# zju3dv/LoG

Hardware: NVIDIA H100
Metric: gaussians_per_s_fwd_bwd (higher is better)
Workload: dtype f32

## Files before the change

include/log_b200_raster.h:

```cpp
#ifndef LOG_B200_RASTER_H
#define LOG_B200_RASTER_H

#include <stdint.h>

#ifdef __cplusplus
extern "C" {
#endif

#define LGR_ABI_VERSION 19
#define LGR_TILE 16

#define LGR_FILTER_ADD 0
#define LGR_FILTER_MAX 1
#define LGR_FILTER_NONE 2

#define LGR_E_BADARG (-1)
#define LGR_E_CAPACITY (-2)
#define LGR_E_UNSUPPORTED (-3)

typedef struct lgr_view {
  int32_t image_height, image_width;
  float tanfovx, tanfovy;
  float scale_modifier;
  int32_t sh_degree;
  int32_t sh_coeffs;
  int32_t filter_mode;
  int32_t want_aux;
  int32_t tile_row_begin, tile_row_end;
  int32_t num_owners;
  int32_t raw_params;
  int32_t* band_ids_d;
  int32_t* band_blk_d;
  int32_t* band_count_d;
  int32_t* band_rows_d;
  float* band_dsplat_d;
  int32_t* tile_rank_d;
  const int64_t* gather_index_d;
  const int32_t* pid_map_d;
  int32_t* contrib_id_d;
  uint32_t* contrib_entry_d;
  int32_t* contrib_count_d;
  const int32_t* last_contrib_d;
  const int32_t* region_count_d;
  int64_t region_cap;
  int32_t num_regions;
  int32_t num_channels;
  int32_t log_depth;
  float* splat_ext_d;
  const float* cov3D_precomp_d;
  float* dcov3D_d;
  const float* viewmatrix_d;
  const float* projmatrix_d;
  const float* campos_d;
  const float* bg_d;
} lgr_view;

#define LGR_SPLAT_FLOATS 12
#define LGR_GRAD_FLOATS 12
#define LGR_TILE_SCRATCH_INTS 33
#define LGR_CONTRIB_MAX_LIST (1 << 24)
#define LGR_META_INTS 8

int lgr_abi_version(void);

int lgr_compute_radius(int64_t n, const float* means3D_d, const float* scales_d, const float* rotations_d,
                       const float* projmatrix_d, const float* viewmatrix_d, float focal_x, float focal_y,
                       float tan_fovx, float tan_fovy, float* radii_d, void* stream);

int lgr_mark_visible(int64_t n, const float* means3D_d, const float* viewmatrix_d, uint8_t* visible_d, void* stream);

int lgr_forward_project(const lgr_view* view, int64_t n, const float* means3D_d, const float* opacities_d,
                        const float* scales_d, const float* rotations_d, const float* colors_precomp_d,
                        const float* shs_d, float* splat_d, int32_t* radii_d, uint8_t* clamped_d,
                        int32_t* tile_start_d, int32_t* tile_cursor_d, int32_t* meta_d, void* stream);

int lgr_forward_render(const lgr_view* view, int64_t n, int64_t num_instances, int32_t max_tile_len,
                       int32_t num_long_tiles, const float* splat_d, const int32_t* radii_d, const int32_t* tile_start_d,
                       int32_t* tile_cursor_d, uint32_t* inst_key_d, uint32_t* inst_val_d, uint32_t* inst_tmp_d,
                       int32_t* sorted_ids_d, float* image_d, float* final_T_d, int32_t* n_contrib_d,
                       int32_t* point_id_pixel_d, float* point_weight_pixel_d, float* point_weight_d,
                       int32_t* point_count_d, void* stream);
int32_t lgr_sort_smem_capacity(void);

int lgr_forward_render_device_sized(const lgr_view* view, int64_t n, int64_t instance_capacity, int32_t* meta_d,
                                    const float* splat_d, const int32_t* radii_d, int32_t* tile_start_d,
                                    int32_t* tile_cursor_d, uint32_t* inst_key_d, uint32_t* inst_val_d,
                                    int32_t* sorted_ids_d, float* image_d, float* final_T_d, int32_t* n_contrib_d,
                                    int32_t* point_id_pixel_d, float* point_weight_pixel_d, float* point_weight_d,
                                    int32_t* point_count_d, void* stream);

int lgr_backward(const lgr_view* view, int64_t n, int64_t num_instances, const float* means3D_d,
                 const float* opacities_d, const float* scales_d, const float* rotations_d,
                 const float* colors_precomp_d, const float* shs_d, const float* splat_d, const int32_t* radii_d,
                 const uint8_t* clamped_d, const int32_t* tile_start_d, const int32_t* sorted_ids_d,
                 const float* image_d, const float* dL_dimage_d, float* dsplat_d,
                 float* dmeans3D_d, float* dmeans2D_d, float* dopacities_d, float* dscales_d, float* drotations_d,
                 float* dcolors_d, float* dshs_d, float* grad_rows_d, void* const* peer_stage_d, int32_t my_rank,
                 int64_t num_rows, void* stream);

#define LGR_STAGE_HEADER_FLOATS 64
#define LGR_ROW_FLOATS 20
#define LGR_OWNER_CHUNK(n, r) ((((n) + (r) - 1) / (r) + 255) / 256 * 256)
int lgr_grad_scatter_add(int64_t num_rows, const float* rows_d, int64_t lo, int64_t hi, float* shard_d, void* stream);
int lgr_grad_scatter_add_staged(const float* stage_d, int32_t num_sources, int64_t owner_chunk, int64_t lo, int64_t hi,
                                float* shard_d, void* stream);

typedef struct lgr_shard_layout {
  int32_t num_ranks, my_rank;
  int64_t cap;
  int64_t off_count, off_splat, off_radii, off_gid, off_dsplat, off_weight, off_pcount;
} lgr_shard_layout;
#define LGR_SHARD_MAX_RANKS 32
#define LGR_SHARD_SEND_INTS(n_local, r) (2 * (int64_t)(r) * ((((n_local) > 0 ? (n_local) : 1) + 255) / 256) + (r))

int lgr_shard_send(const lgr_view* view, const lgr_shard_layout* layout, int64_t n_local, int64_t gid_base,
                   const float* splat_d, const int32_t* radii_d, int32_t* send_scratch_d, void* const* peer_base_d,
                   void* stream);

int lgr_shard_recv_bin(const lgr_view* view, const lgr_shard_layout* layout, float* exchange_d, float* dsplat_d,
                       int32_t* tile_start_d, int32_t* tile_cursor_d, int32_t* meta_d, void* stream);

int lgr_blend_backward(const lgr_view* view, int64_t n, int64_t num_instances, const float* splat_d,
                       const int32_t* tile_start_d, const int32_t* sorted_ids_d, const float* image_d,
                       const float* dL_dimage_d, float* dsplat_d, void* stream);

int lgr_shard_return_rows(const lgr_shard_layout* layout, const float* exchange_d, int64_t total_rows, const void* rows_d,
                          int32_t row_floats, int64_t dst_offset_floats, void* const* peer_base_d, void* stream);

int lgr_shard_gather(const lgr_view* view, const lgr_shard_layout* layout, int64_t n_local, const float* splat_d,
                     const int32_t* radii_d, const int32_t* send_scratch_d, const float* exchange_d,
                     float* dsplat_local_d, float* point_weight_d, int32_t* point_count_d, void* stream);

int lgr_shard_recv_bin_aux(const lgr_view* view, const lgr_shard_layout* layout, float* exchange_d, float* dsplat_d,
                           int32_t* tile_start_d, int32_t* tile_cursor_d, int32_t* meta_d, float* point_weight_rows_d,
                           int32_t* point_count_rows_d, void* stream);
int lgr_shard_return_packed(const lgr_shard_layout* layout, const float* exchange_d, const float* dsplat_rows_d,
                            const float* point_weight_rows_d, const int32_t* point_count_rows_d, void* const* peer_base_d,
                            void* stream);
int lgr_shard_gather_packed(const lgr_view* view, const lgr_shard_layout* layout, int64_t n_local, const float* splat_d,
                            const int32_t* radii_d, const int32_t* send_scratch_d, const float* exchange_d,
                            float* dsplat_local_d, float* point_weight_d, int32_t* point_count_d, void* stream);

typedef struct lgr_tree {
  int64_t num_points, num_nodes;
  int32_t max_child, max_level;
  const int32_t* node_index_d;
  const int32_t* tree_d;
} lgr_tree;
#define LGR_TREE_SCRATCH_INTS(p, s) (8 + 2 * (int64_t)(p) + (int64_t)(s) + 2 * (((int64_t)(s) + 255) / 256) + 2 + ((int64_t)(s) + 3) / 4)
int lgr_tree_traverse(const lgr_tree* tree, const float* xyz_d, const float* scaling_raw_d, const float* rotation_raw_d,
                      const float* projmatrix_d, const float* viewmatrix_d, float focal_x, float focal_y, float tan_fovx,
                      float tan_fovy, const int64_t* root_index_d, int64_t num_roots, float min_resolution_pixel,
                      int32_t max_depth, int32_t* scratch_d, int64_t* index_out_d, int64_t* count_out_d, void* stream);

int lgr_point_compact(int64_t n, const int32_t* point_count_d, int32_t* scratch_d, int32_t* ids_out_d,
                      int32_t* counts_out_d, int32_t* num_out_d, void* stream);

int lgr_sparse_adam(int64_t rows, int32_t row_floats, const int64_t* index_d, const float* grad_d, float* param_d,
                    float* exp_avg_d, float* exp_avg_sq_d, float* max_exp_avg_sq_d, int64_t step, double lr, double beta1,
                    double beta2, double eps, void* stream);

#define LGR_PROFILE_KERNELS 12
int lgr_profile_enable(int on);
int lgr_profile_collect(double* ms_out, int32_t* launches_out, int32_t capacity);
const char* lgr_profile_kernel_name(int kernel_id);


#ifdef __cplusplus
}
#endif
#endif
```

log_b200/_capi.py:

```python
import ctypes
import os

from .build import LIB_PATH

_i32, _i64, _f32, _vp = ctypes.c_int32, ctypes.c_int64, ctypes.c_float, ctypes.c_void_p

LGR_FILTER_ADD, LGR_FILTER_MAX, LGR_FILTER_NONE = 0, 1, 2
LGR_SPLAT_FLOATS = 12
LGR_GRAD_FLOATS = 12
LGR_META_INTS = 8
LGR_TILE_SCRATCH_INTS = 33
LGR_ABI_VERSION = 19
LGR_CONTRIB_MAX_LIST = 1 << 24
LGR_STAGE_HEADER_FLOATS = 64
LGR_ROW_FLOATS = 20

EXPORTS = ('lgr_abi_version', 'lgr_sort_smem_capacity', 'lgr_compute_radius', 'lgr_forward_project',
           'lgr_forward_render', 'lgr_forward_render_device_sized', 'lgr_backward', 'lgr_grad_scatter_add', 'lgr_grad_scatter_add_staged', 'lgr_point_compact', 'lgr_sparse_adam', 'lgr_profile_enable', 'lgr_profile_collect',
           'lgr_profile_kernel_name', 'lgr_shard_send', 'lgr_shard_recv_bin', 'lgr_blend_backward', 'lgr_shard_return_rows',
           'lgr_shard_gather', 'lgr_shard_recv_bin_aux', 'lgr_shard_return_packed', 'lgr_shard_gather_packed', 'lgr_tree_traverse', 'lgr_mark_visible')
LGR_SHARD_MAX_RANKS = 32
LGR_PROFILE_KERNELS = 12


class LgrView(ctypes.Structure):
    _fields_ = [('image_height', _i32), ('image_width', _i32), ('tanfovx', _f32), ('tanfovy', _f32),
                ('scale_modifier', _f32), ('sh_degree', _i32), ('sh_coeffs', _i32), ('filter_mode', _i32),
                ('want_aux', _i32), ('tile_row_begin', _i32), ('tile_row_end', _i32),
                ('num_owners', _i32), ('raw_params', _i32), ('band_ids_d', _vp), ('band_blk_d', _vp), ('band_count_d', _vp), ('band_rows_d', _vp), ('band_dsplat_d', _vp), ('tile_rank_d', _vp), ('gather_index_d', _vp), ('pid_map_d', _vp), ('contrib_id_d', _vp), ('contrib_entry_d', _vp), ('contrib_count_d', _vp), ('last_contrib_d', _vp),
                ('region_count_d', _vp), ('region_cap', _i64), ('num_regions', _i32), ('num_channels', _i32), ('log_depth', _i32), ('splat_ext_d', _vp), ('cov3D_precomp_d', _vp), ('dcov3D_d', _vp),
                ('viewmatrix_d', _vp), ('projmatrix_d', _vp), ('campos_d', _vp), ('bg_d', _vp)]


class LgrShardLayout(ctypes.Structure):
    _fields_ = [('num_ranks', _i32), ('my_rank', _i32), ('cap', _i64), ('off_count', _i64), ('off_splat', _i64),
                ('off_radii', _i64), ('off_gid', _i64), ('off_dsplat', _i64), ('off_weight', _i64), ('off_pcount', _i64)]


class LgrTree(ctypes.Structure):
    _fields_ = [('num_points', _i64), ('num_nodes', _i64), ('max_child', _i32), ('max_level', _i32),
                ('node_index_d', _vp), ('tree_d', _vp)]


def tree_scratch_ints(num_points, slots):
    return 8 + 2 * num_points + slots + 2 * ((slots + 255) // 256) + 2 + (slots + 3) // 4


def shard_send_ints(n_local, r):
    return 2 * r * ((max(n_local, 1) + 255) // 256) + r


class LgrError(RuntimeError):
    pass


_lib = None


def bind(lib):
    lib.lgr_abi_version.restype = ctypes.c_int
    lib.lgr_sort_smem_capacity.restype = _i32
    lib.lgr_mark_visible.restype = ctypes.c_int
    lib.lgr_mark_visible.argtypes = [_i64, _vp, _vp, _vp, _vp]
    lib.lgr_compute_radius.restype = ctypes.c_int
    lib.lgr_compute_radius.argtypes = [_i64, _vp, _vp, _vp, _vp, _vp, _f32, _f32, _f32, _f32, _vp, _vp]
    lib.lgr_forward_project.restype = ctypes.c_int
    lib.lgr_forward_project.argtypes = [ctypes.POINTER(LgrView), _i64] + [_vp] * 13
    lib.lgr_forward_render.restype = ctypes.c_int
    lib.lgr_forward_render.argtypes = [ctypes.POINTER(LgrView), _i64, _i64, _i32, _i32] + [_vp] * 16
    lib.lgr_forward_render_device_sized.restype = ctypes.c_int
    lib.lgr_forward_render_device_sized.argtypes = [ctypes.POINTER(LgrView), _i64, _i64] + [_vp] * 16
    lib.lgr_sparse_adam.restype = ctypes.c_int
    lib.lgr_sparse_adam.argtypes = [_i64, _i32, _vp, _vp, _vp, _vp, _vp, _vp, _i64, ctypes.c_double, ctypes.c_double,
                                    ctypes.c_double, ctypes.c_double, _vp]
    lib.lgr_point_compact.restype = ctypes.c_int
    lib.lgr_point_compact.argtypes = [_i64, _vp, _vp, _vp, _vp, _vp, _vp]
    lib.lgr_backward.restype = ctypes.c_int
    lib.lgr_backward.argtypes = [ctypes.POINTER(LgrView), _i64, _i64] + [_vp] * 23 + [_i32, _i64, _vp]
    lib.lgr_grad_scatter_add_staged.restype = ctypes.c_int
    lib.lgr_grad_scatter_add_staged.argtypes = [_vp, _i32, _i64, _i64, _i64, _vp, _vp]
    lib.lgr_grad_scatter_add.restype = ctypes.c_int
    lib.lgr_grad_scatter_add.argtypes = [_i64, _vp, _i64, _i64, _vp, _vp]
    lay = ctypes.POINTER(LgrShardLayout)
    lib.lgr_shard_send.restype = ctypes.c_int
    lib.lgr_shard_send.argtypes = [ctypes.POINTER(LgrView), lay, _i64, _i64, _vp, _vp, _vp, _vp, _vp]
    lib.lgr_shard_recv_bin.restype = ctypes.c_int
    lib.lgr_shard_recv_bin.argtypes = [ctypes.POINTER(LgrView), lay, _vp, _vp, _vp, _vp, _vp, _vp]
    lib.lgr_blend_backward.restype = ctypes.c_int
    lib.lgr_blend_backward.argtypes = [ctypes.POINTER(LgrView), _i64, _i64, _vp, _vp, _vp, _vp, _vp, _vp, _vp]
    lib.lgr_shard_return_rows.restype = ctypes.c_int
    lib.lgr_shard_return_rows.argtypes = [lay, _vp, _i64, _vp, _i32, _i64, _vp, _vp]
    lib.lgr_shard_gather.restype = ctypes.c_int
    lib.lgr_shard_gather.argtypes = [ctypes.POINTER(LgrView), lay, _i64, _vp, _vp, _vp, _vp, _vp, _vp, _vp, _vp]
    lib.lgr_shard_recv_bin_aux.restype = ctypes.c_int
    lib.lgr_shard_recv_bin_aux.argtypes = [ctypes.POINTER(LgrView), lay, _vp, _vp, _vp, _vp, _vp, _vp, _vp, _vp]
    lib.lgr_shard_return_packed.restype = ctypes.c_int
    lib.lgr_shard_return_packed.argtypes = [lay, _vp, _vp, _vp, _vp, _vp, _vp]
    lib.lgr_shard_gather_packed.restype = ctypes.c_int
    lib.lgr_shard_gather_packed.argtypes = [ctypes.POINTER(LgrView), lay, _i64, _vp, _vp, _vp, _vp, _vp, _vp, _vp, _vp]
    lib.lgr_tree_traverse.restype = ctypes.c_int
    lib.lgr_tree_traverse.argtypes = [ctypes.POINTER(LgrTree), _vp, _vp, _vp, _vp, _vp, _f32, _f32, _f32, _f32, _vp, _i64, _f32,
                                      _i32, _vp, _vp, _vp, _vp]
    lib.lgr_profile_enable.restype = ctypes.c_int
    lib.lgr_profile_enable.argtypes = [ctypes.c_int]
    lib.lgr_profile_collect.restype = ctypes.c_int
    lib.lgr_profile_collect.argtypes = [_vp, _vp, _i32]
    lib.lgr_profile_kernel_name.restype = ctypes.c_char_p
    lib.lgr_profile_kernel_name.argtypes = [ctypes.c_int]
    return lib


def load():
    global _lib
    if _lib is not None:
        return _lib
    if not os.path.exists(LIB_PATH):
        raise LgrError(f'{LIB_PATH} not found: run `python -m log_b200.build` (or __graft_entry__.build()). '
                       'log_b200 has no CPU fallback.')
    lib = bind(ctypes.CDLL(LIB_PATH))
    if lib.lgr_abi_version() != LGR_ABI_VERSION:
        raise LgrError('liblog_b200_raster.so ABI version mismatch: rebuild with `python -m log_b200.build --force`')
    _lib = lib
    return lib


def current_stream(device=None):
    import torch
    return ctypes.c_void_p(torch.cuda.current_stream(device).cuda_stream)


def require_cuda(t, name):
    if not t.is_cuda:
        raise LgrError(f'{name} is on {t.device}: log_b200 rasterises on CUDA only (no CPU fallback)')


def check(rc, what):
    if rc == 0:
        return
    if rc > 0:
        raise LgrError(f'{what}: CUDA error {rc}')
    names = {-1: 'bad argument', -2: 'instance buffer capacity', -3: 'unsupported'}
    raise LgrError(f'{what}: {names.get(rc, rc)}')


def profile_enable(on=True):
    check(load().lgr_profile_enable(1 if on else 0), 'lgr_profile_enable')


def profile_collect():
    lib = load()
    ms = (ctypes.c_double * LGR_PROFILE_KERNELS)()
    cnt = (_i32 * LGR_PROFILE_KERNELS)()
    check(lib.lgr_profile_collect(ms, cnt, LGR_PROFILE_KERNELS), 'lgr_profile_collect')
    return {lib.lgr_profile_kernel_name(k).decode(): (ms[k], cnt[k]) for k in range(LGR_PROFILE_KERNELS)}


def owner_chunk(n, r):
    return ((n + r - 1) // r + 255) // 256 * 256
```

log_b200/csrc/lgr_bin.cu:

```cuda
#include "lgr_common.cuh"
#include "lgr_prof.cuh"

namespace lgr {

constexpr int SCAN_THREADS = 1024;
constexpr int SORT_CAP_SMALL_FWD = 4096;

__global__ void __launch_bounds__(SCAN_THREADS)
tile_scan_kernel(int ntiles, int32_t* __restrict__ tile_start ,
                 int32_t* __restrict__ cursor ,
                 int32_t* __restrict__ meta, int small_cap, int ranked) {
  __shared__ int warp_sum[SCAN_THREADS / 32];
  __shared__ int carry_s, maxl_s, nbig_s;
  const int tid = threadIdx.x, lane = tid & 31, wid = tid >> 5;
  if (tid == 0) { carry_s = 0; maxl_s = 0; nbig_s = 0; }
  __syncthreads();
  int local_max = 0;
  for (int base = 0; base < ntiles; base += SCAN_THREADS) {
    const int i = base + tid;
    const int c = (i < ntiles) ? cursor[i * CSTRIDE] + cursor[i * CSTRIDE + 1] : 0;
    local_max = max(local_max, c);
    int x = c;
#pragma unroll
    for (int o = 1; o < 32; o <<= 1) { const int y = __shfl_up_sync(0xffffffffu, x, o); if (lane >= o) x += y; }
    if (lane == 31) warp_sum[wid] = x;
    __syncthreads();
    if (wid == 0) {
      int w = warp_sum[lane];
#pragma unroll
      for (int o = 1; o < 32; o <<= 1) { const int y = __shfl_up_sync(0xffffffffu, w, o); if (lane >= o) w += y; }
      warp_sum[lane] = w;
    }
    __syncthreads();
    const int carry = carry_s;
    const int excl = carry + (wid ? warp_sum[wid - 1] : 0) + x - c;
    if (i < ntiles) {
      tile_start[i] = excl; cursor[i * CSTRIDE + ranked] = 0;
      if (c > small_cap) cursor[CSTRIDE * ntiles + atomicAdd(&nbig_s, 1)] = i;
    }
    __syncthreads();
    if (tid == SCAN_THREADS - 1) carry_s = carry + warp_sum[31];
    __syncthreads();
  }
#pragma unroll
  for (int o = 16; o > 0; o >>= 1) local_max = max(local_max, __shfl_xor_sync(0xffffffffu, local_max, o));
  if (lane == 0) atomicMax(&maxl_s, local_max);
  __syncthreads();
  if (tid == 0) { tile_start[ntiles] = carry_s; meta[0] = carry_s; meta[1] = maxl_s; meta[5] = nbig_s; }
}

constexpr int SCATTER_THREADS = 256;

__global__ void __launch_bounds__(SCATTER_THREADS)
bin_scatter_kernel(View v, int64_t n, const float* __restrict__ splat, const int32_t* __restrict__ radii,
                   const int32_t* __restrict__ tile_start, int32_t* __restrict__ cursor, uint32_t* __restrict__ inst_key,
                   uint32_t* __restrict__ inst_val, int64_t capacity ) {
  __shared__ int64_t s_first[LGR_SHARD_MAX_RANKS + 1];
  const int64_t total = v.region_count ? region_setup(v, s_first) : n;
  for (int64_t base = (int64_t)blockIdx.x * SCATTER_THREADS; base < total; base += (int64_t)gridDim.x * SCATTER_THREADS) {
  int64_t i = base + threadIdx.x;
  bool live = i < total;
  if (live && v.region_count) i = region_row(v, s_first, i);
  if (live && v.num_owners > 0) {
    const int b = (int)(i / 256), sl = (int)(i % 256);
    if (sl >= v.band_blk[b]) live = false;
    else {
      const int id = v.band_ids[i];
      v.band_rows[v.band_blk[v.band_blocks + b] + sl] = id;
      if (v.band_dsplat) {
        float4* z = reinterpret_cast<float4*>(v.band_dsplat + (int64_t)id * LGR_GRAD_FLOATS);
        z[0] = z[1] = z[2] = make_float4(0.f, 0.f, 0.f, 0.f);
      }
      i = id;
    }
  }
  int rad = 0;
  float4 r0 = make_float4(0.f, 0.f, 0.f, 0.f), r1 = r0;
  float depth = 0.f;
  int4 rk = make_int4(-1, -1, -1, -1);
  if (live) {
    rad = radii[i];
    r0 = ldg4(splat + i * LGR_SPLAT_FLOATS);
    r1 = ldg4(splat + i * LGR_SPLAT_FLOATS + 4);
    depth = __ldg(splat + i * LGR_SPLAT_FLOATS + 11);
    if (v.tile_rank) rk = __ldg(reinterpret_cast<const int4*>(v.tile_rank + 4 * i));
    live = rad > 0;
  }
  if (live && v.num_owners == 0 && v.band_dsplat) {
    float4* z = reinterpret_cast<float4*>(v.band_dsplat + i * LGR_GRAD_FLOATS);
    z[0] = z[1] = z[2] = make_float4(0.f, 0.f, 0.f, 0.f);
  }
  int x0 = 0, y0 = 0, x1 = 0, y1 = 0;
  uint32_t key = 0;
  if (live) {
    live = r1.z > 0.f;
    if (live) {
      key = __float_as_uint(depth);
      tile_rect_tight(r0.x, r0.y, rad, r1.z, r1.w, v.gx, v.gy, v.row0, v.row1, x0, y0, x1, y1);
    }
  }
  const int w = x1 - x0, cnt = live ? w * (y1 - y0) : 0;
  if (cnt > 0 && cnt <= 4) {
    int t[4], slot[4];
#pragma unroll
    for (int k = 0; k < 4; k++) {
      const int ty = y0 + k / max(w, 1), tx = x0 + k % max(w, 1);
      t[k] = k < cnt ? (ty - v.row0) * v.gx + tx : -1;
    }
    if (v.tile_rank) {
      slot[0] = rk.x; slot[1] = rk.y; slot[2] = rk.z; slot[3] = rk.w;
    } else {
#pragma unroll
      for (int k = 0; k < 4; k++) slot[k] = t[k] >= 0 ? atomicAdd(cursor + t[k] * CSTRIDE, 1) : 0;
    }
#pragma unroll
    for (int k = 0; k < 4; k++)
      if (t[k] >= 0) {
        const int pos = __ldg(tile_start + t[k]) + slot[k];
        if (pos < capacity) { inst_key[pos] = key; inst_val[pos] = (uint32_t)i; }
      }
  }
  const int lane = threadIdx.x & 31, big = v.tile_rank ? 1 : 0;
  unsigned todo = __ballot_sync(0xffffffffu, cnt > 4);
  while (todo) {
    const int src = __ffs(todo) - 1;
    todo &= todo - 1;
    const int bx0 = __shfl_sync(0xffffffffu, x0, src), by0 = __shfl_sync(0xffffffffu, y0, src);
    const int bw = __shfl_sync(0xffffffffu, w, src), bcnt = __shfl_sync(0xffffffffu, cnt, src);
    const uint32_t bkey = __shfl_sync(0xffffffffu, key, src);
    const uint32_t bid = (uint32_t)__shfl_sync(0xffffffffu, (int)i, src);
    for (int k = lane; k < bcnt; k += 32) {
      const int t = (by0 + k / bw - v.row0) * v.gx + bx0 + k % bw;
      const int pos = tile_start[t] + (big ? cursor[t * CSTRIDE] : 0) + atomicAdd(cursor + t * CSTRIDE + big, 1);
      if (pos < capacity) { inst_key[pos] = bkey; inst_val[pos] = bid; }
    }
  }
  }
}

constexpr int SORT_THREADS = 256;
constexpr int SORT_WARPS = SORT_THREADS / 32;
constexpr int RADIX_BITS = 8;
constexpr int RADIX = 1 << RADIX_BITS;
constexpr int SORT_CAP_SMALL = SORT_CAP_SMALL_FWD;
constexpr int SORT_CAP_LARGE = 13312;

__device__ __forceinline__ bool radix_pass(const uint32_t* __restrict__ kin, const uint32_t* __restrict__ vin,
                                           uint32_t* __restrict__ kout, uint32_t* __restrict__ vout, int len, int shift,
                                           bool on_val, int* __restrict__ whist) {
  const int tid = threadIdx.x, lane = tid & 31, wid = tid >> 5;
  const int seg = ((len + SORT_WARPS * 32 - 1) / (SORT_WARPS * 32)) * 32;
  const int beg = min(len, wid * seg), end = min(len, beg + seg);
  for (int j = tid; j < SORT_WARPS * RADIX; j += SORT_THREADS) whist[j] = 0;
  __syncthreads();
  int* myh = whist + wid * RADIX;
  for (int i = beg + lane; i < end; i += 32) {
    const uint32_t d = ((on_val ? vin[i] : kin[i]) >> shift) & (RADIX - 1);
    atomicAdd(myh + d, 1);
  }
  __syncthreads();
  {
    const int d = tid;
    int tot = 0;
#pragma unroll
    for (int w = 0; w < SORT_WARPS; w++) tot += whist[w * RADIX + d];
    int x = tot;
#pragma unroll
    for (int o = 1; o < 32; o <<= 1) { const int y = __shfl_up_sync(0xffffffffu, x, o); if (lane >= o) x += y; }
    __shared__ int wsum[SORT_WARPS];
    if (lane == 31) wsum[wid] = x;
    __syncthreads();
    int base = x - tot;
#pragma unroll
    for (int w = 0; w < SORT_WARPS; w++) if (w < wid) base += wsum[w];
#pragma unroll
    for (int w = 0; w < SORT_WARPS; w++) { const int c = whist[w * RADIX + d]; whist[w * RADIX + d] = base; base += c; }
    if (__syncthreads_or(tot == len)) return true;
  }
  for (int i0 = beg; i0 < end; i0 += 32) {
    const int i = i0 + lane;
    const bool ok = i < end;
    uint32_t k = 0, val = 0;
    if (ok) { k = kin[i]; val = vin[i]; }
    const uint32_t d = ok ? (((on_val ? val : k) >> shift) & (RADIX - 1)) : (RADIX + lane);
    const uint32_t peers = __match_any_sync(0xffffffffu, d);
    const int rank = __popc(peers & ((1u << lane) - 1u));
    int base = 0;
    if (ok) base = myh[d];
    __syncwarp();
    if (ok && rank == 0) myh[d] = base + __popc(peers);
    __syncwarp();
    if (ok) { kout[base + rank] = k; vout[base + rank] = val; }
  }
  __syncthreads();
  return false;
}

__device__ __forceinline__ void sort_tile(uint32_t* kA, uint32_t* vA, uint32_t* kB, uint32_t* vB, int len, int id_bits,
                                          int* whist) {
  uint32_t *ki = kA, *vi = vA, *ko = kB, *vo = vB;
  auto run = [&](int shift, bool on_val) {
    const bool ident = radix_pass(ki, vi, ko, vo, len, shift, on_val, whist);
    if (!ident) { uint32_t* t = ki; ki = ko; ko = t; t = vi; vi = vo; vo = t; }
  };
  for (int s = 0; s < 32; s += RADIX_BITS) run(s, false);
  int my_tie = 0;
  for (int i = threadIdx.x + 1; i < len; i += SORT_THREADS) if (ki[i] == ki[i - 1]) my_tie = 1;
  if (__syncthreads_or(my_tie)) {
    for (int s = 0; s < id_bits; s += RADIX_BITS) run(s, true);
    for (int s = 0; s < 32; s += RADIX_BITS) run(s, false);
  }
  if (ki != kA) {
    for (int i = threadIdx.x; i < len; i += SORT_THREADS) { kA[i] = ki[i]; vA[i] = vi[i]; }
    __syncthreads();
  }
}

constexpr int MSD_SMALL = 96;
constexpr int MSD_STACK = 512;

struct MsdShared {
  int hist[RADIX];
  int bstart[RADIX + 1];
  alignas(16) int wsum[SORT_WARPS];
  unsigned long long wmin[SORT_WARPS], wmax[SORT_WARPS];
  int stack_beg[MSD_STACK], stack_len[MSD_STACK];
  int top, shift, overflow;
};

__device__ __forceinline__ unsigned long long composite(uint32_t k, uint32_t v) { return ((unsigned long long)k << 32) | v; }

__device__ __forceinline__ bool sort_tile_msd(uint32_t* kA, uint32_t* vA, uint32_t* kB, uint32_t* vB, int len, MsdShared& sh) {
  const int tid = threadIdx.x, lane = tid & 31, wid = tid >> 5;
  if (tid == 0) { sh.stack_beg[0] = 0; sh.stack_len[0] = len; sh.top = 1; sh.overflow = 0; }
  __syncthreads();
  while (true) {
    const int top = sh.top;
    if (top == 0 || sh.overflow) break;
    const int beg = sh.stack_beg[top - 1], n = sh.stack_len[top - 1];
    __syncthreads();
    if (tid == 0) sh.top = top - 1;
    unsigned long long mn = ~0ull, mx = 0ull;
    for (int i = tid; i < n; i += SORT_THREADS) {
      const unsigned long long c = composite(kA[beg + i], vA[beg + i]);
      mn = min(mn, c); mx = max(mx, c);
    }
#pragma unroll
    for (int o = 16; o > 0; o >>= 1) {
      mn = min(mn, __shfl_xor_sync(0xffffffffu, mn, o));
      mx = max(mx, __shfl_xor_sync(0xffffffffu, mx, o));
    }
    if (lane == 0) { sh.wmin[wid] = mn; sh.wmax[wid] = mx; }
    sh.hist[tid] = 0;
    __syncthreads();
    if (tid == 0) {
      unsigned long long a = sh.wmin[0], b = sh.wmax[0];
#pragma unroll
      for (int w = 1; w < SORT_WARPS; w++) { a = min(a, sh.wmin[w]); b = max(b, sh.wmax[w]); }
      const int hb = 63 - __clzll((long long)(a ^ b));
      sh.shift = max(0, hb - (RADIX_BITS - 1));
    }
    __syncthreads();
    const int shift = sh.shift;
    for (int i = tid; i < n; i += SORT_THREADS)
      atomicAdd(&sh.hist[(int)((composite(kA[beg + i], vA[beg + i]) >> shift) & (RADIX - 1))], 1);
    __syncthreads();
    {
      const int c = sh.hist[tid];
      int x = c;
#pragma unroll
      for (int o = 1; o < 32; o <<= 1) { const int y = __shfl_up_sync(0xffffffffu, x, o); if (lane >= o) x += y; }
      if (lane == 31) sh.wsum[wid] = x;
      __syncthreads();
      int base = x - c;
#pragma unroll
      for (int w = 0; w < SORT_WARPS; w++) if (w < wid) base += sh.wsum[w];
      sh.bstart[tid] = base;
      sh.hist[tid] = base;
      if (tid == RADIX - 1) sh.bstart[RADIX] = base + c;
    }
    __syncthreads();
    for (int i = tid; i < n; i += SORT_THREADS) {
      const uint32_t k = kA[beg + i], v = vA[beg + i];
      const int slot = atomicAdd(&sh.hist[(int)((composite(k, v) >> shift) & (RADIX - 1))], 1);
      kB[beg + slot] = k; vB[beg + slot] = v;
    }
    __syncthreads();
    for (int i = tid; i < n; i += SORT_THREADS) {
      const uint32_t k = kB[beg + i], v = vB[beg + i];
      const int d = (int)((composite(k, v) >> shift) & (RADIX - 1));
      const int b0 = sh.bstart[d], bn = sh.bstart[d + 1] - b0;
      int dst = i;
      if (bn <= MSD_SMALL) {
        const uint32_t* kb = kB + beg + b0;
        const uint32_t* vb = vB + beg + b0;
        int rank = 0, eq = 0;
#pragma unroll 8
        for (int j = 0; j < bn; j++) {
          const uint32_t kj = kb[j];
          rank += (kj < k) ? 1 : 0;
          eq += (kj == k) ? 1 : 0;
        }
        if (eq > 1)
          for (int j = 0; j < bn; j++) rank += (kb[j] == k && vb[j] < v) ? 1 : 0;
        dst = b0 + rank;
      }
      kA[beg + dst] = k; vA[beg + dst] = v;
    }
    {
      const int b0 = sh.bstart[tid], bn = sh.bstart[tid + 1] - b0;
      if (bn > MSD_SMALL) {
        const int slot = atomicAdd(&sh.top, 1);
        if (slot < MSD_STACK) { sh.stack_beg[slot] = beg + b0; sh.stack_len[slot] = bn; }
        else sh.overflow = 1;
      }
    }
    __syncthreads();
  }
  const bool ok = sh.overflow == 0;
  __syncthreads();
  return ok;
}

template <int MODE>
__global__ void __launch_bounds__(SORT_THREADS)
tile_sort_kernel(const int32_t* __restrict__ tile_list ,
                 const int32_t* __restrict__ tile_start, uint32_t* __restrict__ inst_key,
                 uint32_t* __restrict__ inst_val, uint32_t* __restrict__ tmp, int32_t* __restrict__ sorted_ids, int lo,
                 int cap, int id_bits, const int32_t* __restrict__ count_ptr, int32_t* __restrict__ flags) {
  extern __shared__ uint32_t smem_u32[];
  __shared__ int whist[MODE == 1 ? SORT_WARPS * RADIX : 1];
  __shared__ MsdShared msd;
  const int count = count_ptr ? *count_ptr : (int)gridDim.x;
  for (int b = blockIdx.x; b < count; b += gridDim.x) {
    const int t = tile_list ? tile_list[b] : b;
    const int beg = tile_start[t], len = tile_start[t + 1] - beg;
    if (len <= lo) continue;
    if (MODE == 0 && len > cap) {
      if (flags && lo > 0 && threadIdx.x == 0) atomicOr(flags, 2);
      continue;
    }
    if (MODE == 0) {
      uint32_t* kA = smem_u32; uint32_t* vA = kA + cap; uint32_t* kB = vA + cap; uint32_t* vB = kB + cap;
      for (int i = threadIdx.x; i < len; i += SORT_THREADS) { kA[i] = inst_key[beg + i]; vA[i] = inst_val[beg + i]; }
      __syncthreads();
      if (len > 1 && !sort_tile_msd(kA, vA, kB, vB, len, msd)) __trap();
      for (int i = threadIdx.x; i < len; i += SORT_THREADS) sorted_ids[beg + i] = (int32_t)vA[i];
    } else {
      uint32_t* kA = inst_key + beg; uint32_t* vA = inst_val + beg;
      uint32_t* kB = tmp + 2 * (int64_t)beg; uint32_t* vB = kB + len;
      __syncthreads();
      if (!sort_tile_msd(kA, vA, kB, vB, len, msd)) sort_tile(kA, vA, kB, vB, len, id_bits, whist);
      for (int i = threadIdx.x; i < len; i += SORT_THREADS) sorted_ids[beg + i] = (int32_t)vA[i];
    }
    __syncthreads();
  }
}

__global__ void __launch_bounds__(256)
clamp_lists_kernel(int ntiles, int64_t capacity, int32_t* __restrict__ tile_start, int32_t* __restrict__ meta) {
  if ((int64_t)meta[0] <= capacity) return;
  for (int i = blockIdx.x * 256 + threadIdx.x; i <= ntiles; i += gridDim.x * 256) tile_start[i] = 0;
  if (blockIdx.x == 0 && threadIdx.x == 0) atomicOr(meta + 6, 1);
}


int sort_smem_capacity() { return SORT_CAP_LARGE; }

constexpr int PC_THREADS = 1024;

__global__ void __launch_bounds__(PC_THREADS)
pc_block_count_kernel(int64_t n, const int32_t* __restrict__ count, int32_t* __restrict__ blk) {
  const int64_t i = (int64_t)blockIdx.x * PC_THREADS + threadIdx.x;
  const int c = __syncthreads_count(i < n && count[i] > 0);
  if (threadIdx.x == 0) blk[blockIdx.x] = c;
}

__global__ void __launch_bounds__(1024)
pc_scan_kernel(int nb, int32_t* __restrict__ blk , int32_t* __restrict__ num_out) {
  __shared__ int warp_sum[32];
  __shared__ int carry_s;
  const int tid = threadIdx.x, lane = tid & 31, wid = tid >> 5;
  if (tid == 0) carry_s = 0;
  __syncthreads();
  for (int base = 0; base < nb; base += 1024) {
    const int b = base + tid;
    const int c = b < nb ? blk[b] : 0;
    int x = c;
#pragma unroll
    for (int o = 1; o < 32; o <<= 1) { const int y = __shfl_up_sync(0xffffffffu, x, o); if (lane >= o) x += y; }
    if (lane == 31) warp_sum[wid] = x;
    __syncthreads();
    if (wid == 0) {
      int w = warp_sum[lane];
#pragma unroll
      for (int o = 1; o < 32; o <<= 1) { const int y = __shfl_up_sync(0xffffffffu, w, o); if (lane >= o) w += y; }
      warp_sum[lane] = w;
    }
    __syncthreads();
    const int carry = carry_s;
    if (b < nb) blk[nb + b] = carry + (wid ? warp_sum[wid - 1] : 0) + x - c;
    __syncthreads();
    if (tid == 1023) carry_s = carry + warp_sum[31];
    __syncthreads();
  }
  if (tid == 0) { blk[2 * nb] = carry_s; *num_out = carry_s; }
}

__global__ void __launch_bounds__(PC_THREADS)
pc_compact_kernel(int64_t n, const int32_t* __restrict__ count, const int32_t* __restrict__ blk, int nb,
                  int32_t* __restrict__ ids_out, int32_t* __restrict__ counts_out) {
  __shared__ int wsum[PC_THREADS / 32];
  const int64_t i = (int64_t)blockIdx.x * PC_THREADS + threadIdx.x;
  const int lane = threadIdx.x & 31, wid = threadIdx.x >> 5;
  const int c = i < n ? count[i] : 0;
  const unsigned bal = __ballot_sync(0xffffffffu, c > 0);
  if (lane == 0) wsum[wid] = __popc(bal);
  __syncthreads();
  int base = blk[nb + blockIdx.x];
  for (int w = 0; w < wid; w++) base += wsum[w];
  if (c > 0) {
    const int pos = base + __popc(bal & ((1u << lane) - 1u));
    ids_out[pos] = (int32_t)i;
    counts_out[pos] = c;
  }
}

int launch_point_compact(int64_t n, const int32_t* count, int32_t* blk, int32_t* ids_out, int32_t* counts_out, int32_t* num_out,
                         cudaStream_t st) {
  const int nb = (int)((n + PC_THREADS - 1) / PC_THREADS);
  if (nb == 0) {
    cudaError_t e = cudaMemsetAsync(num_out, 0, sizeof(int32_t), st);
    return e == cudaSuccess ? 0 : (int)e;
  }
  pc_block_count_kernel<<<nb, PC_THREADS, 0, st>>>(n, count, blk);
  LGR_CHECK_LAUNCH();
  pc_scan_kernel<<<1, 1024, 0, st>>>(nb, blk, num_out);
  LGR_CHECK_LAUNCH();
  pc_compact_kernel<<<nb, PC_THREADS, 0, st>>>(n, count, blk, nb, ids_out, counts_out);
  LGR_CHECK_LAUNCH();
  return 0;
}

int launch_tile_scan(int ntiles, int32_t* tile_start, int32_t* cursor, int32_t* meta, bool ranked, cudaStream_t st) {
  ProfScope ps(K_TILE_SCAN, st);
  tile_scan_kernel<<<1, SCAN_THREADS, 0, st>>>(ntiles, tile_start, cursor, meta, SORT_CAP_SMALL_FWD, ranked ? 1 : 0);
  LGR_CHECK_LAUNCH();
  return 0;
}

constexpr int LONG_SORT_GRID = 132;

int launch_bin_and_sort(const View& v, int64_t n, int64_t num_inst, int max_len, int num_long, const float* splat,
                        const int32_t* radii, int32_t* tile_start, int32_t* cursor, uint32_t* inst_key,
                        uint32_t* inst_val, uint32_t* inst_tmp, int32_t* sorted_ids, int32_t* meta_dev, cudaStream_t st) {
  if (n == 0) return 0;
  if (meta_dev) {
    const int nt = v.gx * (v.row1 - v.row0);
    clamp_lists_kernel<<<(nt + 256) / 256, 256, 0, st>>>(nt, num_inst, tile_start, meta_dev);
    LGR_CHECK_LAUNCH();
  }
  if (num_inst == 0 && v.num_owners == 0 && v.band_dsplat == nullptr) return 0;
  const int ntiles = v.gx * (v.row1 - v.row0);
  unsigned blocks = (unsigned)((n + SCATTER_THREADS - 1) / SCATTER_THREADS);
  if (v.region_count && blocks > (unsigned)LGR_REGION_GRID) blocks = (unsigned)LGR_REGION_GRID;
  {
    ProfScope ps(K_BIN_SCATTER, st);
    bin_scatter_kernel<<<blocks, SCATTER_THREADS, 0, st>>>(v, n, splat, radii, tile_start, cursor, inst_key, inst_val,
                                                           meta_dev ? num_inst : (int64_t)0x7fffffffffffffffLL);
  }
  LGR_CHECK_LAUNCH();
  if (num_inst == 0) return 0;
  int id_bits = 8;
  while (id_bits < 32 && (n - 1) >> id_bits) id_bits += 8;
  {
    cudaError_t e = cudaFuncSetAttribute(tile_sort_kernel<0>, cudaFuncAttributeMaxDynamicSharedMemorySize, 16 * SORT_CAP_LARGE);
    if (e != cudaSuccess) return (int)e;
  }
  if (meta_dev) {
    ProfScope ps(K_TILE_SORT, st, 2);
    tile_sort_kernel<0><<<ntiles, SORT_THREADS, 16 * SORT_CAP_SMALL, st>>>(nullptr, tile_start, inst_key, inst_val, inst_tmp, sorted_ids, 0, SORT_CAP_SMALL, id_bits, nullptr, nullptr);
    LGR_CHECK_LAUNCH();
    const int32_t* long_list = cursor + CSTRIDE * ntiles;
    tile_sort_kernel<0><<<LONG_SORT_GRID, SORT_THREADS, 16 * SORT_CAP_LARGE, st>>>(long_list, tile_start, inst_key, inst_val, inst_tmp, sorted_ids, SORT_CAP_SMALL, SORT_CAP_LARGE, id_bits, meta_dev + 5, meta_dev + 6);
    LGR_CHECK_LAUNCH();
    return 0;
  }
  ProfScope ps(K_TILE_SORT, st, 1 + (num_long > 0) + (max_len > SORT_CAP_LARGE));
  const int cap_main = max(256, min(max_len, SORT_CAP_SMALL));
  tile_sort_kernel<0><<<ntiles, SORT_THREADS, 16 * cap_main, st>>>(nullptr, tile_start, inst_key, inst_val, inst_tmp, sorted_ids, 0, cap_main, id_bits, nullptr, nullptr);
  LGR_CHECK_LAUNCH();
  if (num_long > 0) {
    const int32_t* long_list = cursor + CSTRIDE * ntiles;
    const int cap = min(max_len, SORT_CAP_LARGE);
    tile_sort_kernel<0><<<num_long, SORT_THREADS, 16 * cap, st>>>(long_list, tile_start, inst_key, inst_val, inst_tmp, sorted_ids, SORT_CAP_SMALL, cap, id_bits, nullptr, nullptr);
    LGR_CHECK_LAUNCH();
    if (max_len > SORT_CAP_LARGE) {
      if (!inst_tmp) return LGR_E_CAPACITY;
      tile_sort_kernel<1><<<num_long, SORT_THREADS, 0, st>>>(long_list, tile_start, inst_key, inst_val, inst_tmp, sorted_ids, SORT_CAP_LARGE, 0, id_bits, nullptr, nullptr);
      LGR_CHECK_LAUNCH();
    }
  }
  return 0;
}

}
```

log_b200/csrc/lgr_capi.cu:

```cuda
#include "lgr_common.cuh"
#include "lgr_prof.cuh"
#include <math.h>

namespace lgr {
int launch_mark_visible(int64_t, const float*, const float*, uint8_t*, cudaStream_t);
int launch_compute_radius(int64_t, const float*, const float*, const float*, const float*, const float*, float, float,
                          float, float, float*, cudaStream_t);
int launch_project_fwd(const View&, int64_t, const float*, const float*, const float*, const float*, const float*,
                       const float*, float*, int32_t*, uint8_t*, int32_t*, int32_t*, cudaStream_t);
int launch_project_bwd(const View&, int64_t, const float*, const float*, const float*, const float*, const float*, bool,
                       const int32_t*, const uint8_t*, const float*, float*, float*, float*, float*, float*, float*,
                       float*, float*, void* const*, int, cudaStream_t);
int launch_grad_scatter_add(int64_t, const float*, int64_t, int64_t, float*, cudaStream_t);
int launch_grad_scatter_add_staged(const float*, int, int64_t, int64_t, int64_t, float*, cudaStream_t);
int launch_band_scan(const View&, cudaStream_t);
int launch_tile_scan(int, int32_t*, int32_t*, int32_t*, bool, cudaStream_t);
int launch_bin_and_sort(const View&, int64_t, int64_t, int, int, const float*, const int32_t*, int32_t*, int32_t*,
                        uint32_t*, uint32_t*, uint32_t*, int32_t*, int32_t*, cudaStream_t);
int sort_smem_capacity();
int launch_blend_fwd(const View&, const int32_t*, const int32_t*, const float*, float*, float*, int32_t*, int32_t*,
                     float*, float*, int32_t*, cudaStream_t);
int launch_sparse_adam(int64_t, int, const int64_t*, const float*, float*, float*, float*, float*, float, float, float, float,
                       float, float, float, cudaStream_t);
int launch_point_compact(int64_t, const int32_t*, int32_t*, int32_t*, int32_t*, int32_t*, cudaStream_t);
int launch_blend_bwd(const View&, const int32_t*, const int32_t*, const float*, const float*, const float*, float*,
                     cudaStream_t);
int launch_shard_send(const View&, const ShardLayout&, int64_t, int64_t, const float*, const int32_t*, int32_t*, void* const*,
                      cudaStream_t);
int launch_shard_recv_count(const View&, const ShardLayout&, float*, float*, int32_t*, int32_t*, float*, int32_t*, cudaStream_t);
int launch_shard_return_packed(const ShardLayout&, const float*, const float*, const float*, const int32_t*, void* const*, cudaStream_t);
int launch_shard_return(const ShardLayout&, const float*, int64_t, const void*, int, int64_t, void* const*, cudaStream_t);
int launch_shard_gather(const View&, const ShardLayout&, int64_t, const float*, const int32_t*, const int32_t*, const float*,
                        float*, float*, int32_t*, int, cudaStream_t);
int launch_tree_traverse(const TreeArgs&, int64_t, int64_t, const int64_t*, int64_t, int, int32_t*, int64_t*, int64_t*, cudaStream_t);
}

using namespace lgr;

static bool view_ok(const lgr_view* v) {
  if (!v || v->image_height <= 0 || v->image_width <= 0) return false;
  if (!v->viewmatrix_d || !v->projmatrix_d || !v->bg_d) return false;
  if (v->filter_mode < 0 || v->filter_mode > 2) return false;
  if (v->tile_row_begin < 0 || v->tile_row_end < v->tile_row_begin) return false;
  const int gy = (v->image_height + TILE - 1) / TILE;
  if (v->tile_row_end > gy) return false;
  if (v->num_owners < 0 || (v->num_owners > 0 && (!v->band_ids_d || !v->band_count_d || !v->band_blk_d || !v->band_rows_d))) return false;
  if (v->gather_index_d && v->num_owners > 0) return false;
  if (v->region_count_d && (v->num_regions <= 0 || v->num_regions > LGR_SHARD_MAX_RANKS || v->region_cap <= 0 || v->num_owners > 0 ||
                            v->gather_index_d))
    return false;
  const int lists = (v->contrib_id_d != nullptr) + (v->contrib_entry_d != nullptr) + (v->contrib_count_d != nullptr);
  if (lists != 0 && lists != 3) return false;
  if (v->num_channels != 0 && v->num_channels != 3 && v->num_channels != 6) return false;
  if (v->num_channels == 6 && !v->splat_ext_d) return false;
  if (v->log_depth != 0 && (v->log_depth != 1 || v->num_channels != 6)) return false;
  return true;
}

static int six_channels_check(const lgr_view* v) {
  if (v->num_channels != 6) return 0;
  if (v->num_owners > 0 || v->region_count_d || v->pid_map_d) return LGR_E_UNSUPPORTED;
  if (!v->log_depth && (v->raw_params || v->gather_index_d)) return LGR_E_UNSUPPORTED;
  return 0;
}

extern "C" {

int lgr_abi_version(void) { return LGR_ABI_VERSION; }

int32_t lgr_sort_smem_capacity(void) { return sort_smem_capacity(); }

int lgr_compute_radius(int64_t n, const float* means3D_d, const float* scales_d, const float* rotations_d,
                       const float* projmatrix_d, const float* viewmatrix_d, float focal_x, float focal_y,
                       float tan_fovx, float tan_fovy, float* radii_d, void* stream) {
  if (n < 0 || (n > 0 && (!means3D_d || !scales_d || !rotations_d || !radii_d)) || !projmatrix_d || !viewmatrix_d)
    return LGR_E_BADARG;
  return launch_compute_radius(n, means3D_d, scales_d, rotations_d, projmatrix_d, viewmatrix_d, focal_x, focal_y,
                               tan_fovx, tan_fovy, radii_d, (cudaStream_t)stream);
}

int lgr_mark_visible(int64_t n, const float* means3D_d, const float* viewmatrix_d, uint8_t* visible_d, void* stream) {
  if (n < 0 || !viewmatrix_d || (n > 0 && (!means3D_d || !visible_d))) return LGR_E_BADARG;
  return launch_mark_visible(n, means3D_d, viewmatrix_d, visible_d, (cudaStream_t)stream);
}

int lgr_forward_project(const lgr_view* view, int64_t n, const float* means3D_d, const float* opacities_d,
                        const float* scales_d, const float* rotations_d, const float* colors_precomp_d,
                        const float* shs_d, float* splat_d, int32_t* radii_d, uint8_t* clamped_d,
                        int32_t* tile_start_d, int32_t* tile_cursor_d, int32_t* meta_d, void* stream) {
  if (!view_ok(view) || n < 0 || !tile_start_d || !tile_cursor_d || !meta_d) return LGR_E_BADARG;
  if (const int rc6 = six_channels_check(view)) return rc6;
  const bool six_precomp = view->num_channels == 6 && !view->log_depth;
  if (six_precomp && shs_d) return LGR_E_UNSUPPORTED;
  if (six_precomp && n > 0 && !colors_precomp_d) return LGR_E_BADARG;
  const bool log_sh = view->raw_params && colors_precomp_d && shs_d;
  if (!log_sh && (colors_precomp_d != nullptr) == (shs_d != nullptr) && n > 0) return LGR_E_BADARG;
  if (view->raw_params && shs_d && !colors_precomp_d) return LGR_E_UNSUPPORTED;
  if (log_sh) {
    if (!view->campos_d) return LGR_E_BADARG;
    if (view->sh_degree < 0 || view->sh_degree > 3) return LGR_E_UNSUPPORTED;
    if (view->sh_coeffs < (view->sh_degree + 1) * (view->sh_degree + 1) - 1) return LGR_E_BADARG;
    if (view->num_owners > 0) return LGR_E_UNSUPPORTED;
  } else if (shs_d) {
    if (!view->campos_d || !clamped_d) return LGR_E_BADARG;
    if (view->sh_degree < 0 || view->sh_degree > 3) return LGR_E_UNSUPPORTED;
    if (view->sh_coeffs < (view->sh_degree + 1) * (view->sh_degree + 1)) return LGR_E_BADARG;
  }
  const bool cov3d = view->cov3D_precomp_d != nullptr;
  if (n > 0 && (!means3D_d || !opacities_d || (!cov3d && (!scales_d || !rotations_d)) || !splat_d || !radii_d)) return LGR_E_BADARG;
  if (cov3d && (view->raw_params || view->num_owners > 0)) return LGR_E_UNSUPPORTED;
  if (n > 0x7fffffffLL) return LGR_E_UNSUPPORTED;
  cudaStream_t st = (cudaStream_t)stream;
  const View v = make_view(view, n);
  const int ntiles = v.gx * (v.row1 - v.row0);
  if (v.num_owners > 0) {
    if (shs_d) return LGR_E_UNSUPPORTED;
  }
  if (log_sh && view->sh_degree == 0) shs_d = nullptr;
  cudaError_t e = cudaMemsetAsync(tile_cursor_d, 0, sizeof(int32_t) * (size_t)ntiles * CSTRIDE, st);
  if (e != cudaSuccess) return (int)e;
  e = cudaMemsetAsync(meta_d, 0, sizeof(int32_t) * LGR_META_INTS, st);
  if (e != cudaSuccess) return (int)e;
  int rc = launch_project_fwd(v, n, means3D_d, opacities_d, scales_d, rotations_d, colors_precomp_d, shs_d, splat_d,
                              radii_d, clamped_d, tile_cursor_d, meta_d, st);
  if (rc) return rc;
  rc = launch_band_scan(v, st);
  if (rc) return rc;
  return launch_tile_scan(ntiles, tile_start_d, tile_cursor_d, meta_d, view->tile_rank_d != nullptr, st);
}

int lgr_forward_render(const lgr_view* view, int64_t n, int64_t num_instances, int32_t max_tile_len,
                       int32_t num_long_tiles, const float* splat_d, const int32_t* radii_d, const int32_t* tile_start_d,
                       int32_t* tile_cursor_d, uint32_t* inst_key_d, uint32_t* inst_val_d, uint32_t* inst_tmp_d,
                       int32_t* sorted_ids_d, float* image_d, float* final_T_d, int32_t* n_contrib_d,
                       int32_t* point_id_pixel_d, float* point_weight_pixel_d, float* point_weight_d,
                       int32_t* point_count_d, void* stream) {
  if (!view_ok(view) || n < 0 || num_instances < 0 || num_long_tiles < 0 || !tile_start_d || !tile_cursor_d || !image_d || !final_T_d ||
      !n_contrib_d)
    return LGR_E_BADARG;
  if (num_instances > 0 && (!inst_key_d || !inst_val_d || !sorted_ids_d || !splat_d || !radii_d)) return LGR_E_BADARG;
  if (const int rc6 = six_channels_check(view)) return rc6;
  if (view->want_aux && (!point_id_pixel_d || !point_weight_pixel_d || (n > 0 && !point_weight_d))) return LGR_E_BADARG;
  if (num_instances > 0x7fffffffLL) return LGR_E_UNSUPPORTED;
  if (view->contrib_id_d && max_tile_len > LGR_CONTRIB_MAX_LIST) return LGR_E_UNSUPPORTED;
  cudaStream_t st = (cudaStream_t)stream;
  const View v = make_view(view, n);
  int rc = launch_bin_and_sort(v, n, num_instances, max_tile_len, num_long_tiles, splat_d, radii_d, const_cast<int32_t*>(tile_start_d), tile_cursor_d,
                               inst_key_d, inst_val_d, inst_tmp_d, sorted_ids_d, nullptr, st);
  if (rc) return rc;
  return launch_blend_fwd(v, tile_start_d, sorted_ids_d, splat_d, image_d, final_T_d, n_contrib_d, point_id_pixel_d,
                          point_weight_pixel_d, point_weight_d, view->want_aux ? point_count_d : nullptr, st);
}

int lgr_forward_render_device_sized(const lgr_view* view, int64_t n, int64_t instance_capacity, int32_t* meta_d,
                                    const float* splat_d, const int32_t* radii_d, int32_t* tile_start_d,
                                    int32_t* tile_cursor_d, uint32_t* inst_key_d, uint32_t* inst_val_d,
                                    int32_t* sorted_ids_d, float* image_d, float* final_T_d, int32_t* n_contrib_d,
                                    int32_t* point_id_pixel_d, float* point_weight_pixel_d, float* point_weight_d,
                                    int32_t* point_count_d, void* stream) {
  if (!view_ok(view) || n < 0 || instance_capacity <= 0 || !meta_d || !tile_start_d || !tile_cursor_d || !image_d || !final_T_d ||
      !n_contrib_d || !inst_key_d || !inst_val_d || !sorted_ids_d)
    return LGR_E_BADARG;
  if (n > 0 && (!splat_d || !radii_d)) return LGR_E_BADARG;
  if (const int rc6 = six_channels_check(view)) return rc6;
  if (view->want_aux && (!point_id_pixel_d || !point_weight_pixel_d || (n > 0 && !point_weight_d))) return LGR_E_BADARG;
  if (instance_capacity > 0x7fffffffLL) return LGR_E_UNSUPPORTED;
  cudaStream_t st = (cudaStream_t)stream;
  const View v = make_view(view, n);
  int rc = launch_bin_and_sort(v, n, instance_capacity, 0, 0, splat_d, radii_d, tile_start_d, tile_cursor_d, inst_key_d, inst_val_d,
                               nullptr, sorted_ids_d, meta_d, st);
  if (rc) return rc;
  return launch_blend_fwd(v, tile_start_d, sorted_ids_d, splat_d, image_d, final_T_d, n_contrib_d, point_id_pixel_d,
                          point_weight_pixel_d, point_weight_d, view->want_aux ? point_count_d : nullptr, st);
}

int lgr_backward(const lgr_view* view, int64_t n, int64_t num_instances, const float* means3D_d,
                 const float* opacities_d, const float* scales_d, const float* rotations_d,
                 const float* colors_precomp_d, const float* shs_d, const float* splat_d, const int32_t* radii_d,
                 const uint8_t* clamped_d, const int32_t* tile_start_d, const int32_t* sorted_ids_d,
                 const float* image_d, const float* dL_dimage_d, float* dsplat_d,
                 float* dmeans3D_d, float* dmeans2D_d, float* dopacities_d, float* dscales_d, float* drotations_d,
                 float* dcolors_d, float* dshs_d, float* grad_rows_d, void* const* peer_stage_d, int32_t my_rank,
                 int64_t num_rows, void* stream) {
  if (!view_ok(view) || n < 0 || !tile_start_d || !image_d || !dL_dimage_d) return LGR_E_BADARG;
  if (const int rc6 = six_channels_check(view)) return rc6;
  if (view->num_channels == 6 && ((shs_d && !view->log_depth) || grad_rows_d || peer_stage_d)) return LGR_E_UNSUPPORTED;
  if (n == 0) return 0;
  const bool log_sh = view->raw_params && colors_precomp_d && shs_d;
  const bool use_sh = shs_d != nullptr && !log_sh;
  if (!log_sh && use_sh == (colors_precomp_d != nullptr)) return LGR_E_BADARG;
  if (log_sh && (!dshs_d || !view->campos_d || view->num_owners > 0)) return LGR_E_BADARG;
  const bool cov3d = view->cov3D_precomp_d != nullptr;
  if (!means3D_d || (!cov3d && (!scales_d || !rotations_d)) || !splat_d || !radii_d || !dsplat_d) return LGR_E_BADARG;
  if (cov3d && (!view->dcov3D_d || view->raw_params || view->num_owners > 0 || grad_rows_d || peer_stage_d)) return LGR_E_BADARG;
  if (view->raw_params && (!opacities_d || use_sh)) return LGR_E_BADARG;
  if (grad_rows_d || peer_stage_d) {
    if (view->num_owners <= 0 || use_sh) return LGR_E_BADARG;
    if (peer_stage_d && (my_rank < 0 || my_rank >= view->num_owners)) return LGR_E_BADARG;
    if (num_rows < 0 || num_rows > n) return LGR_E_BADARG;
  } else {
    if (view->num_owners > 0) return LGR_E_BADARG;
    if (!dmeans3D_d || !dmeans2D_d || !dopacities_d || (!cov3d && (!dscales_d || !drotations_d))) return LGR_E_BADARG;
    if (use_sh ? (!dshs_d || !clamped_d || !view->campos_d) : !dcolors_d) return LGR_E_BADARG;
  }
  if (num_instances > 0 && !sorted_ids_d) return LGR_E_BADARG;
  cudaStream_t st = (cudaStream_t)stream;
  const View v = make_view(view, n);
  int rc = 0;
  if (num_instances > 0) rc = launch_blend_bwd(v, tile_start_d, sorted_ids_d, splat_d, image_d, dL_dimage_d, dsplat_d, st);
  if (rc) return rc;
  const bool rows_mode = grad_rows_d || peer_stage_d;
  return launch_project_bwd(v, rows_mode ? num_rows : n, means3D_d, opacities_d, scales_d, rotations_d, (use_sh || log_sh) ? shs_d : nullptr, use_sh, radii_d, clamped_d, dsplat_d,
                            dmeans3D_d, dmeans2D_d, dopacities_d, dscales_d, drotations_d, dcolors_d, dshs_d, grad_rows_d, peer_stage_d, my_rank, st);
}

int lgr_sparse_adam(int64_t rows, int32_t row_floats, const int64_t* index_d, const float* grad_d, float* param_d,
                    float* exp_avg_d, float* exp_avg_sq_d, float* max_exp_avg_sq_d, int64_t step, double lr, double beta1,
                    double beta2, double eps, void* stream) {
  if (rows < 0 || row_floats <= 0 || step < 1) return LGR_E_BADARG;
  if (rows > 0 && (!index_d || !grad_d || !param_d || !exp_avg_d || !exp_avg_sq_d)) return LGR_E_BADARG;
  const double bc1 = 1.0 - pow(beta1, (double)step), bc2 = 1.0 - pow(beta2, (double)step);
  const double step_size = lr / bc1;
  return launch_sparse_adam(rows, row_floats, index_d, grad_d, param_d, exp_avg_d, exp_avg_sq_d, max_exp_avg_sq_d,
                            (float)beta1, (float)beta2, (float)(1.0 - beta1), (float)(1.0 - beta2), (float)sqrt(bc2),
                            (float)(-step_size), (float)eps, (cudaStream_t)stream);
}

int lgr_point_compact(int64_t n, const int32_t* point_count_d, int32_t* scratch_d, int32_t* ids_out_d,
                      int32_t* counts_out_d, int32_t* num_out_d, void* stream) {
  if (n < 0 || !num_out_d || (n > 0 && (!point_count_d || !scratch_d || !ids_out_d || !counts_out_d))) return LGR_E_BADARG;
  return launch_point_compact(n, point_count_d, scratch_d, ids_out_d, counts_out_d, num_out_d, (cudaStream_t)stream);
}

int lgr_grad_scatter_add_staged(const float* stage_d, int32_t num_sources, int64_t owner_chunk, int64_t lo, int64_t hi,
                                float* shard_d, void* stream) {
  if (!stage_d || !shard_d || num_sources <= 0 || owner_chunk <= 0 || hi < lo) return LGR_E_BADARG;
  return launch_grad_scatter_add_staged(stage_d, num_sources, owner_chunk, lo, hi, shard_d, (cudaStream_t)stream);
}

int lgr_grad_scatter_add(int64_t num_rows, const float* rows_d, int64_t lo, int64_t hi, float* shard_d, void* stream) {
  if (num_rows < 0 || hi < lo || (num_rows > 0 && (!rows_d || !shard_d))) return LGR_E_BADARG;
  return launch_grad_scatter_add(num_rows, rows_d, lo, hi, shard_d, (cudaStream_t)stream);
}

static bool layout_ok(const lgr_shard_layout* l) {
  if (!l || l->num_ranks <= 0 || l->num_ranks > LGR_SHARD_MAX_RANKS || l->my_rank < 0 || l->my_rank >= l->num_ranks) return false;
  if (l->cap <= 0 || l->cap % 256) return false;
  const int64_t offs[7] = {l->off_count, l->off_splat, l->off_radii, l->off_gid, l->off_dsplat, l->off_weight, l->off_pcount};
  for (int k = 0; k < 7; k++) if (offs[k] < 0 || offs[k] % 4) return false;
  return true;
}

static ShardLayout make_layout(const lgr_shard_layout* l) {
  ShardLayout o;
  o.R = l->num_ranks; o.me = l->my_rank; o.cap = l->cap;
  o.off_count = l->off_count; o.off_splat = l->off_splat; o.off_radii = l->off_radii; o.off_gid = l->off_gid;
  o.off_dsplat = l->off_dsplat; o.off_weight = l->off_weight; o.off_pcount = l->off_pcount;
  return o;
}

int lgr_shard_send(const lgr_view* view, const lgr_shard_layout* layout, int64_t n_local, int64_t gid_base,
                   const float* splat_d, const int32_t* radii_d, int32_t* send_scratch_d, void* const* peer_base_d,
                   void* stream) {
  if (!view_ok(view) || !layout_ok(layout) || n_local < 0 || gid_base < 0 || !send_scratch_d || !peer_base_d) return LGR_E_BADARG;
  if (view->num_channels == 6) return LGR_E_UNSUPPORTED;
  if (n_local > layout->cap || (n_local > 0 && (!splat_d || !radii_d))) return LGR_E_BADARG;
  if (view->num_owners != 0 || view->tile_row_begin != 0 || (view->tile_row_end != 0 && view->tile_row_end != (view->image_height + TILE - 1) / TILE))
    return LGR_E_BADARG;
  if (gid_base + n_local > 0x7fffffffLL) return LGR_E_UNSUPPORTED;
  return launch_shard_send(make_view(view, n_local), make_layout(layout), n_local, gid_base, splat_d, radii_d, send_scratch_d,
                           peer_base_d, (cudaStream_t)stream);
}

int lgr_shard_recv_bin(const lgr_view* view, const lgr_shard_layout* layout, float* exchange_d, float* dsplat_d,
                       int32_t* tile_start_d, int32_t* tile_cursor_d, int32_t* meta_d, void* stream) {
  return lgr_shard_recv_bin_aux(view, layout, exchange_d, dsplat_d, tile_start_d, tile_cursor_d, meta_d, nullptr, nullptr, stream);
}

int lgr_shard_recv_bin_aux(const lgr_view* view, const lgr_shard_layout* layout, float* exchange_d, float* dsplat_d,
                           int32_t* tile_start_d, int32_t* tile_cursor_d, int32_t* meta_d, float* point_weight_rows_d,
                           int32_t* point_count_rows_d, void* stream) {
  if (!view_ok(view) || !layout_ok(layout) || !exchange_d || !dsplat_d || !tile_start_d || !tile_cursor_d || !meta_d) return LGR_E_BADARG;
  if (view->num_channels == 6) return LGR_E_UNSUPPORTED;
  if (view->num_owners != 0) return LGR_E_BADARG;
  if (view->region_count_d != reinterpret_cast<const int32_t*>(exchange_d + layout->off_count) || view->region_cap != layout->cap ||
      view->num_regions != layout->num_ranks)
    return LGR_E_BADARG;
  if ((int64_t)layout->num_ranks * layout->cap > 0x7fffffffLL) return LGR_E_UNSUPPORTED;
  cudaStream_t st = (cudaStream_t)stream;
  const View v = make_view(view, (int64_t)layout->num_ranks * layout->cap);
  const int ntiles = v.gx * (v.row1 - v.row0);
  cudaError_t e = cudaMemsetAsync(tile_cursor_d, 0, sizeof(int32_t) * (size_t)(ntiles > 0 ? ntiles : 1) * CSTRIDE, st);
  if (e != cudaSuccess) return (int)e;
  e = cudaMemsetAsync(meta_d, 0, sizeof(int32_t) * LGR_META_INTS, st);
  if (e != cudaSuccess) return (int)e;
  int rc = launch_shard_recv_count(v, make_layout(layout), exchange_d, dsplat_d, tile_cursor_d, meta_d, point_weight_rows_d,
                                   point_count_rows_d, st);
  if (rc) return rc;
  return launch_tile_scan(ntiles, tile_start_d, tile_cursor_d, meta_d, view->tile_rank_d != nullptr, st);
}

int lgr_blend_backward(const lgr_view* view, int64_t n, int64_t num_instances, const float* splat_d,
                       const int32_t* tile_start_d, const int32_t* sorted_ids_d, const float* image_d,
                       const float* dL_dimage_d, float* dsplat_d, void* stream) {
  if (!view_ok(view) || n < 0 || num_instances < 0 || !tile_start_d || !image_d || !dL_dimage_d) return LGR_E_BADARG;
  if (const int rc6 = six_channels_check(view)) return rc6;
  if (num_instances == 0 || n == 0) return 0;
  if (!splat_d || !sorted_ids_d || !dsplat_d) return LGR_E_BADARG;
  return launch_blend_bwd(make_view(view, n), tile_start_d, sorted_ids_d, splat_d, image_d, dL_dimage_d, dsplat_d,
                          (cudaStream_t)stream);
}

int lgr_shard_return_rows(const lgr_shard_layout* layout, const float* exchange_d, int64_t total_rows, const void* rows_d,
                          int32_t row_floats, int64_t dst_offset_floats, void* const* peer_base_d, void* stream) {
  if (!layout_ok(layout) || !exchange_d || !peer_base_d || total_rows < 0 || row_floats <= 0) return LGR_E_BADARG;
  if (dst_offset_floats < 0 || dst_offset_floats % 4 || (total_rows > 0 && !rows_d)) return LGR_E_BADARG;
  return launch_shard_return(make_layout(layout), exchange_d, total_rows, rows_d, row_floats, dst_offset_floats, peer_base_d,
                             (cudaStream_t)stream);
}

int lgr_shard_gather(const lgr_view* view, const lgr_shard_layout* layout, int64_t n_local, const float* splat_d,
                     const int32_t* radii_d, const int32_t* send_scratch_d, const float* exchange_d,
                     float* dsplat_local_d, float* point_weight_d, int32_t* point_count_d, void* stream) {
  if (!view_ok(view) || !layout_ok(layout) || n_local < 0 || n_local > layout->cap) return LGR_E_BADARG;
  if (view->num_channels == 6) return LGR_E_UNSUPPORTED;
  if (n_local == 0) return 0;
  if (!splat_d || !radii_d || !send_scratch_d || !exchange_d || !dsplat_local_d) return LGR_E_BADARG;
  return launch_shard_gather(make_view(view, n_local), make_layout(layout), n_local, splat_d, radii_d, send_scratch_d, exchange_d,
                             dsplat_local_d, point_weight_d, point_count_d, 0, (cudaStream_t)stream);
}

int lgr_shard_gather_packed(const lgr_view* view, const lgr_shard_layout* layout, int64_t n_local, const float* splat_d,
                            const int32_t* radii_d, const int32_t* send_scratch_d, const float* exchange_d,
                            float* dsplat_local_d, float* point_weight_d, int32_t* point_count_d, void* stream) {
  if (!view_ok(view) || !layout_ok(layout) || n_local < 0 || n_local > layout->cap) return LGR_E_BADARG;
  if (view->num_channels == 6) return LGR_E_UNSUPPORTED;
  if (n_local == 0) return 0;
  if (!splat_d || !radii_d || !send_scratch_d || !exchange_d || !dsplat_local_d) return LGR_E_BADARG;
  return launch_shard_gather(make_view(view, n_local), make_layout(layout), n_local, splat_d, radii_d, send_scratch_d, exchange_d,
                             dsplat_local_d, point_weight_d, point_count_d, 1, (cudaStream_t)stream);
}

int lgr_shard_return_packed(const lgr_shard_layout* layout, const float* exchange_d, const float* dsplat_rows_d,
                            const float* point_weight_rows_d, const int32_t* point_count_rows_d, void* const* peer_base_d,
                            void* stream) {
  if (!layout_ok(layout) || !exchange_d || !dsplat_rows_d || !peer_base_d) return LGR_E_BADARG;
  return launch_shard_return_packed(make_layout(layout), exchange_d, dsplat_rows_d, point_weight_rows_d, point_count_rows_d,
                                    peer_base_d, (cudaStream_t)stream);
}

int lgr_tree_traverse(const lgr_tree* tree, const float* xyz_d, const float* scaling_raw_d, const float* rotation_raw_d,
                      const float* projmatrix_d, const float* viewmatrix_d, float focal_x, float focal_y, float tan_fovx,
                      float tan_fovy, const int64_t* root_index_d, int64_t num_roots, float min_resolution_pixel,
                      int32_t max_depth, int32_t* scratch_d, int64_t* index_out_d, int64_t* count_out_d, void* stream) {
  if (!tree || tree->num_points < 0 || tree->num_nodes < 0 || tree->max_child <= 0 || tree->max_level < 0) return LGR_E_BADARG;
  if (num_roots < 0 || num_roots > tree->num_points || max_depth < 0 || !scratch_d || !count_out_d) return LGR_E_BADARG;
  if (!projmatrix_d || !viewmatrix_d) return LGR_E_BADARG;
  if (tree->num_points > 0 && (!tree->node_index_d || !xyz_d || !scaling_raw_d || !rotation_raw_d || !index_out_d)) return LGR_E_BADARG;
  if (tree->num_nodes > 0 && !tree->tree_d) return LGR_E_BADARG;
  if (num_roots > 0 && !root_index_d) return LGR_E_BADARG;
  if (tree->num_points > 0x7fffffffLL || tree->num_nodes * tree->max_child > 0x7fffffffLL) return LGR_E_UNSUPPORTED;
  TreeArgs a;
  a.node_index = tree->node_index_d; a.tree = tree->tree_d; a.C = tree->max_child;
  a.xyz = xyz_d; a.scaling_raw = scaling_raw_d; a.rotation_raw = rotation_raw_d; a.view = viewmatrix_d; a.proj = projmatrix_d;
  a.fx = focal_x; a.fy = focal_y; a.tanfovx = tan_fovx; a.tanfovy = tan_fovy; a.min_px = min_resolution_pixel;
  const int levels = tree->max_level < max_depth ? tree->max_level : max_depth;
  return launch_tree_traverse(a, tree->num_points, tree->num_nodes, root_index_d, num_roots, levels, scratch_d, index_out_d,
                              count_out_d, (cudaStream_t)stream);
}

int lgr_profile_enable(int on) {
  Profiler& p = Profiler::get();
  p.enabled = on != 0;
  p.used = 0;
  for (int k = 0; k < K_COUNT; k++) p.launches[k] = 0;
  return 0;
}

int lgr_profile_collect(double* ms_out, int32_t* launches_out, int32_t capacity) {
  Profiler& p = Profiler::get();
  if (!ms_out || !launches_out || capacity < K_COUNT) return LGR_E_BADARG;
  for (int k = 0; k < K_COUNT; k++) { ms_out[k] = 0.0; launches_out[k] = p.launches[k]; }
  for (int i = 0; i < p.used; i++) {
    cudaError_t e = cudaEventSynchronize(p.stop[i]);
    if (e != cudaSuccess) return (int)e;
    float ms = 0.f;
    e = cudaEventElapsedTime(&ms, p.start[i], p.stop[i]);
    if (e != cudaSuccess) return (int)e;
    ms_out[p.kid[i]] += ms;
  }
  p.used = 0;
  for (int k = 0; k < K_COUNT; k++) p.launches[k] = 0;
  return 0;
}

const char* lgr_profile_kernel_name(int k) {
  static const char* names[K_COUNT] = {"project_fwd", "tile_scan", "bin_scatter", "tile_sort", "blend_fwd", "blend_bwd",
                                       "project_bwd", "compute_radius", "shard_send", "shard_recv", "shard_return", "shard_gather"};
  return (k >= 0 && k < K_COUNT) ? names[k] : "";
}

}
```

log_b200/csrc/lgr_common.cuh:

```cuda
#pragma once
#include <cuda_runtime.h>
#include <stdint.h>

#include "../../include/log_b200_raster.h"

namespace lgr {

constexpr int TILE = LGR_TILE;
constexpr int TILE_PIX = TILE * TILE;
constexpr float NEAR_Z = 0.2f;
constexpr float ALPHA_MAX = 0.99f;
constexpr float ALPHA_MIN = 1.0f / 255.0f;
constexpr float T_STOP = 1e-4f;
constexpr float FILTER_VAR = 0.3f;
constexpr float CLAMP_FOV = 1.3f;
constexpr int CSTRIDE = 32;
constexpr float LOG2E = 1.4426950408889634f;
constexpr float LN2 = 0.6931471805599453f;

struct View {
  int H, W, gx, gy;
  int row0, row1;
  float tanfovx, tanfovy, fx, fy, scale_mod;
  int sh_degree, sh_K, filter_mode, want_aux;
  int raw_params;
  int num_owners, owner_chunk;
  int32_t* band_ids;
  int32_t* band_blk;
  int32_t* band_count;
  int32_t* band_rows;
  float* band_dsplat;
  int32_t* tile_rank;
  const int64_t* gather;
  const int32_t* pid_map;
  int32_t* contrib_id;
  uint32_t* contrib_entry;
  int32_t* contrib_count;
  const int32_t* last_contrib;
  const int32_t* region_count;
  int64_t region_cap;
  int regions;
  const float* cov3d;
  float* dcov3d;
  int band_blocks;
  const float* view;
  const float* proj;
  const float* campos;
  const float* bg;
  int num_channels;
  int log_depth;
  float* splat_ext;
};

inline View make_view(const lgr_view* v, int64_t n = 0) {
  View o;
  o.num_owners = v->num_owners; o.band_ids = v->band_ids_d; o.band_blk = v->band_blk_d; o.band_count = v->band_count_d; o.band_rows = v->band_rows_d; o.band_dsplat = v->band_dsplat_d; o.tile_rank = v->tile_rank_d; o.gather = v->gather_index_d; o.pid_map = v->pid_map_d; o.contrib_id = v->contrib_id_d; o.contrib_entry = v->contrib_entry_d; o.contrib_count = v->contrib_count_d; o.last_contrib = v->last_contrib_d;
  o.region_count = v->region_count_d; o.region_cap = v->region_cap; o.regions = v->region_count_d ? v->num_regions : 0;
  o.cov3d = v->cov3D_precomp_d; o.dcov3d = v->dcov3D_d;
  o.owner_chunk = o.num_owners > 0 ? (int)LGR_OWNER_CHUNK(n, (int64_t)o.num_owners) : 256;
  if (o.owner_chunk < 256) o.owner_chunk = 256;
  o.band_blocks = (int)((n + 255) / 256);
  o.H = v->image_height; o.W = v->image_width;
  o.gx = (o.W + TILE - 1) / TILE; o.gy = (o.H + TILE - 1) / TILE;
  o.row0 = v->tile_row_begin; o.row1 = v->tile_row_end;
  if (o.row0 == 0 && o.row1 == 0) o.row1 = o.gy;
  o.tanfovx = v->tanfovx; o.tanfovy = v->tanfovy;
  o.fx = o.W / (2.0f * v->tanfovx); o.fy = o.H / (2.0f * v->tanfovy);
  o.scale_mod = v->scale_modifier;
  o.sh_degree = v->sh_degree; o.sh_K = v->sh_coeffs; o.filter_mode = v->filter_mode; o.want_aux = v->want_aux;
  o.raw_params = v->raw_params;
  o.view = v->viewmatrix_d; o.proj = v->projmatrix_d; o.campos = v->campos_d; o.bg = v->bg_d;
  o.num_channels = v->num_channels == 6 ? 6 : 3; o.splat_ext = v->splat_ext_d; o.log_depth = v->log_depth ? 1 : 0;
  return o;
}

struct ShardLayout {
  int R, me;
  int64_t cap;
  int64_t off_count, off_splat, off_radii, off_gid, off_dsplat, off_weight, off_pcount;
};

struct TreeArgs {
  const int32_t* node_index;
  const int32_t* tree;
  int C;
  const float* xyz;
  const float* scaling_raw;
  const float* rotation_raw;
  const float* view;
  const float* proj;
  float fx, fy, tanfovx, tanfovy, min_px;
};


__device__ __forceinline__ float4 ldg4(const float* p) { return __ldg(reinterpret_cast<const float4*>(p)); }

struct Cov2D {
  float a, b, c;
  float a_raw, c_raw;
  float t[3];
  float T[6];
  bool inx, iny;
};

__device__ __forceinline__ void quat_to_R(const float4 q, float R[9]) {
  const float r = q.x, x = q.y, y = q.z, z = q.w;
  R[0] = 1.f - 2.f * (y * y + z * z); R[1] = 2.f * (x * y - r * z); R[2] = 2.f * (x * z + r * y);
  R[3] = 2.f * (x * y + r * z); R[4] = 1.f - 2.f * (x * x + z * z); R[5] = 2.f * (y * z - r * x);
  R[6] = 2.f * (x * z - r * y); R[7] = 2.f * (y * z + r * x); R[8] = 1.f - 2.f * (x * x + y * y);
}

__device__ __forceinline__ void cov3d(const float s[3], const float R[9], float Sg[9]) {
  float M[9];
#pragma unroll
  for (int i = 0; i < 3; i++)
#pragma unroll
    for (int k = 0; k < 3; k++) M[i * 3 + k] = R[i * 3 + k] * s[k];
#pragma unroll
  for (int i = 0; i < 3; i++)
#pragma unroll
    for (int j = 0; j < 3; j++) Sg[i * 3 + j] = M[i * 3] * M[j * 3] + M[i * 3 + 1] * M[j * 3 + 1] + M[i * 3 + 2] * M[j * 3 + 2];
}

__device__ __forceinline__ void cov2d(const float* __restrict__ V, const float p[3], const float Sg[9], float fx, float fy,
                                      float tanfovx, float tanfovy, int filter_mode, Cov2D& o) {
#pragma unroll
  for (int j = 0; j < 3; j++) o.t[j] = p[0] * V[j] + p[1] * V[4 + j] + p[2] * V[8 + j] + V[12 + j];
  const float limx = CLAMP_FOV * tanfovx, limy = CLAMP_FOV * tanfovy;
  const float itz = 1.0f / o.t[2];
  const float txtz = o.t[0] * itz, tytz = o.t[1] * itz;
  o.inx = (txtz >= -limx) && (txtz <= limx);
  o.iny = (tytz >= -limy) && (tytz <= limy);
  const float txc = fminf(limx, fmaxf(-limx, txtz)) * o.t[2];
  const float tyc = fminf(limy, fmaxf(-limy, tytz)) * o.t[2];
  const float J00 = fx * itz, J02 = -(fx * txc) * itz * itz, J11 = fy * itz, J12 = -(fy * tyc) * itz * itz;
#pragma unroll
  for (int j = 0; j < 3; j++) {
    o.T[j] = J00 * V[j * 4 + 0] + J02 * V[j * 4 + 2];
    o.T[3 + j] = J11 * V[j * 4 + 1] + J12 * V[j * 4 + 2];
  }
  float TS[6];
#pragma unroll
  for (int r = 0; r < 2; r++)
#pragma unroll
    for (int j = 0; j < 3; j++) TS[r * 3 + j] = o.T[r * 3] * Sg[j] + o.T[r * 3 + 1] * Sg[3 + j] + o.T[r * 3 + 2] * Sg[6 + j];
  o.a_raw = TS[0] * o.T[0] + TS[1] * o.T[1] + TS[2] * o.T[2];
  o.b = TS[0] * o.T[3] + TS[1] * o.T[4] + TS[2] * o.T[5];
  o.c_raw = TS[3] * o.T[3] + TS[4] * o.T[4] + TS[5] * o.T[5];
  o.a = o.a_raw; o.c = o.c_raw;
  if (filter_mode == LGR_FILTER_ADD) { o.a += FILTER_VAR; o.c += FILTER_VAR; }
  else if (filter_mode == LGR_FILTER_MAX) { o.a = fmaxf(o.a, FILTER_VAR); o.c = fmaxf(o.c, FILTER_VAR); }
}

__device__ __forceinline__ float act_sigmoid(float x) { return 1.0f / (1.0f + expf(-x)); }
__device__ __forceinline__ float4 act_normalize(float4 q, float& inv_norm) {
  inv_norm = 1.0f / fmaxf(sqrtf(q.x * q.x + q.y * q.y + q.z * q.z + q.w * q.w), 1e-12f);
  return make_float4(q.x * inv_norm, q.y * inv_norm, q.z * inv_norm, q.w * inv_norm);
}

__device__ __forceinline__ float radius_from_cov(float a, float b, float c, float& det) {
  det = a * c - b * b;
  const float mid = 0.5f * (a + c);
  const float root = sqrtf(fmaxf(0.1f, mid * mid - det));
  return 3.0f * sqrtf(fmaxf(mid + root, mid - root));
}

__device__ __forceinline__ bool ndc_inside(const float p[3], const float* __restrict__ P) {
  float hom[4];
#pragma unroll
  for (int k = 0; k < 4; k++) hom[k] = p[0] * P[k] + p[1] * P[4 + k] + p[2] * P[8 + k] + P[12 + k];
  const float pw = 1.0f / (hom[3] + 0.0000001f);
  const float nx = hom[0] * pw, ny = hom[1] * pw;
  return !(nx < -1.3f || nx > 1.3f || ny < -1.3f || ny > 1.3f);
}
__device__ __forceinline__ float projected_radius(const float p[3], const float s[3], const float4 q, const float* __restrict__ V,
                                                  float fx, float fy, float tanfovx, float tanfovy) {
  float R[9], Sg[9];
  quat_to_R(q, R);
  cov3d(s, R, Sg);
  Cov2D cv;
  cov2d(V, p, Sg, fx, fy, tanfovx, tanfovy, LGR_FILTER_MAX, cv);
  float det;
  const float rad = radius_from_cov(cv.a, cv.b, cv.c, det);
  return det != 0.0f ? rad : 0.0f;
}

__device__ __forceinline__ void tile_rect(float px, float py, int rad, int gx, int gy, int& x0, int& y0, int& x1, int& y1) {
  x0 = min(gx, max(0, (int)((px - rad) / TILE)));
  x1 = min(gx, max(0, (int)((px + rad + TILE - 1) / TILE)));
  y0 = min(gy, max(0, (int)((py - rad) / TILE)));
  y1 = min(gy, max(0, (int)((py + rad + TILE - 1) / TILE)));
}

__device__ __forceinline__ void tile_rect_tight(float px, float py, int rad, float hx, float hy, int gx, int gy, int row0,
                                                int row1, int& x0, int& y0, int& x1, int& y1) {
  tile_rect(px, py, rad, gx, gy, x0, y0, x1, y1);
  const int tx0 = (int)ceilf((px - hx - (TILE - 1)) * (1.0f / TILE));
  const int tx1 = (int)floorf((px + hx) * (1.0f / TILE)) + 1;
  const int ty0 = (int)ceilf((py - hy - (TILE - 1)) * (1.0f / TILE));
  const int ty1 = (int)floorf((py + hy) * (1.0f / TILE)) + 1;
  x0 = max(x0, tx0); x1 = min(x1, tx1);
  y0 = max(max(y0, ty0), row0); y1 = min(min(y1, ty1), row1);
  if (x1 < x0) x1 = x0;
  if (y1 < y0) y1 = y0;
}

#ifndef LGR_REGION_GRID
#define LGR_REGION_GRID (132 * 16)
#endif

__device__ __forceinline__ int64_t region_setup(const View& v, int64_t* first) {
  if (threadIdx.x == 0) {
    int64_t acc = 0;
    for (int s = 0; s < v.regions; s++) {
      first[s] = acc;
      const int64_t c = v.region_count[s];
      acc += c < 0 ? 0 : (c > v.region_cap ? v.region_cap : c);
    }
    first[v.regions] = acc;
  }
  __syncthreads();
  return first[v.regions];
}
__device__ __forceinline__ int64_t region_row(const View& v, const int64_t* first, int64_t t) {
  int s = 0;
  while (s + 1 < v.regions && t >= first[s + 1]) s++;
  return (int64_t)s * v.region_cap + (t - first[s]);
}

__device__ __forceinline__ bool count_small_tiles(const View& v, int32_t* __restrict__ tile_count, int64_t row, int x0, int y0, int x1,
                                                  int y1) {
  const int w = x1 - x0, cnt = w * (y1 - y0);
  if (cnt > 4) return true;
  if (v.tile_rank == nullptr) {
    for (int k = 0; k < cnt; k++) atomicAdd(tile_count + ((y0 + k / w - v.row0) * v.gx + x0 + k % w) * CSTRIDE, 1);
    return false;
  }
  int r[4];
#pragma unroll
  for (int k = 0; k < 4; k++) {
    r[k] = -1;
    if (k < cnt) r[k] = atomicAdd(tile_count + ((y0 + k / max(w, 1) - v.row0) * v.gx + x0 + k % max(w, 1)) * CSTRIDE, 1);
  }
  *reinterpret_cast<int4*>(v.tile_rank + 4 * row) = make_int4(r[0], r[1], r[2], r[3]);
  return false;
}

__device__ __forceinline__ void warp_count_big_tiles(const View& v, int32_t* __restrict__ tile_count, bool big, int x0, int y0, int x1,
                                                     int y1) {
  const int lane = threadIdx.x & 31;
  const int slot = v.tile_rank ? 1 : 0;
  unsigned todo = __ballot_sync(0xffffffffu, big);
  while (todo) {
    const int src = __ffs(todo) - 1;
    todo &= todo - 1;
    const int bx0 = __shfl_sync(0xffffffffu, x0, src), by0 = __shfl_sync(0xffffffffu, y0, src);
    const int bx1 = __shfl_sync(0xffffffffu, x1, src), by1 = __shfl_sync(0xffffffffu, y1, src);
    const int w = bx1 - bx0, cnt = w * (by1 - by0);
    for (int k = lane; k < cnt; k += 32) atomicAdd(tile_count + ((by0 + k / w - v.row0) * v.gx + bx0 + k % w) * CSTRIDE + slot, 1);
  }
}

constexpr float SH_C0 = 0.28209479177387814f;
constexpr float SH_C1 = 0.4886025119029199f;
__device__ __constant__ const float SH_C2[5] = {1.0925484305920792f, -1.0925484305920792f, 0.31539156525252005f,
                                                 -1.0925484305920792f, 0.5462742152960396f};
__device__ __constant__ const float SH_C3[7] = {-0.5900435899266435f, 2.890611442640554f, -0.4570457994644658f,
                                                 0.3731763325901154f, -0.4570457994644658f, 1.445305721320277f,
                                                 -0.5900435899266435f};

__device__ __forceinline__ void sh_basis(int deg, float x, float y, float z, float B[16]) {
  B[0] = SH_C0;
  if (deg > 0) {
    B[1] = -SH_C1 * y; B[2] = SH_C1 * z; B[3] = -SH_C1 * x;
    if (deg > 1) {
      const float xx = x * x, yy = y * y, zz = z * z, xy = x * y, yz = y * z, xz = x * z;
      B[4] = SH_C2[0] * xy; B[5] = SH_C2[1] * yz; B[6] = SH_C2[2] * (2.f * zz - xx - yy);
      B[7] = SH_C2[3] * xz; B[8] = SH_C2[4] * (xx - yy);
      if (deg > 2) {
        B[9] = SH_C3[0] * y * (3.f * xx - yy); B[10] = SH_C3[1] * xy * z; B[11] = SH_C3[2] * y * (4.f * zz - xx - yy);
        B[12] = SH_C3[3] * z * (2.f * zz - 3.f * xx - 3.f * yy); B[13] = SH_C3[4] * x * (4.f * zz - xx - yy);
        B[14] = SH_C3[5] * z * (xx - yy); B[15] = SH_C3[6] * x * (xx - 3.f * yy);
      }
    }
  }
}

}

#define LGR_CHECK_LAUNCH()                     \
  do {                                         \
    cudaError_t e__ = cudaGetLastError();      \
    if (e__ != cudaSuccess) return (int)e__;   \
  } while (0)
```

log_b200/csrc/lgr_project.cu:

```cuda
#include "lgr_common.cuh"
#include "lgr_prof.cuh"

namespace lgr {

constexpr int PROJ_THREADS = 256;

__device__ __forceinline__ void load3(const float* __restrict__ p, int64_t i, float o[3]) {
  o[0] = __ldg(p + 3 * i); o[1] = __ldg(p + 3 * i + 1); o[2] = __ldg(p + 3 * i + 2);
}

__global__ void __launch_bounds__(PROJ_THREADS)
mark_visible_kernel(int64_t n, const float* __restrict__ means, const float* __restrict__ view, uint8_t* __restrict__ visible) {
  const int64_t i = (int64_t)blockIdx.x * PROJ_THREADS + threadIdx.x;
  if (i >= n) return;
  float p[3];
  load3(means, i, p);
  const float z = p[0] * __ldg(view + 2) + p[1] * __ldg(view + 6) + p[2] * __ldg(view + 10) + __ldg(view + 14);
  visible[i] = z > NEAR_Z ? 1 : 0;
}

__global__ void __launch_bounds__(PROJ_THREADS)
compute_radius_kernel(int64_t n, const float* __restrict__ means, const float* __restrict__ scales,
                      const float* __restrict__ rots, const float* __restrict__ proj, const float* __restrict__ view,
                      float fx, float fy, float tanfovx, float tanfovy, float* __restrict__ radii) {
  __shared__ float sV[16], sP[16];
  if (threadIdx.x < 16) { sV[threadIdx.x] = view[threadIdx.x]; sP[threadIdx.x] = proj[threadIdx.x]; }
  __syncthreads();
  const int64_t i = (int64_t)blockIdx.x * PROJ_THREADS + threadIdx.x;
  if (i >= n) return;
  float p[3];
  load3(means, i, p);
  float out = 0.0f;
  if (ndc_inside(p, sP)) {
    float s[3];
    load3(scales, i, s);
    out = projected_radius(p, s, ldg4(rots + 4 * i), sV, fx, fy, tanfovx, tanfovy);
  }
  radii[i] = out;
}

template <bool USE_SH, bool LOG_SH = false, bool COV3D = false, bool SIX = false, bool DEPTH = false>
__global__ void __launch_bounds__(PROJ_THREADS)
project_fwd_kernel(View v, int64_t n, const float* __restrict__ means, const float* __restrict__ opac,
                   const float* __restrict__ scales, const float* __restrict__ rots,
                   const float* __restrict__ colors, const float* __restrict__ shs, float* __restrict__ splat,
                   int32_t* __restrict__ radii, uint8_t* __restrict__ clamped, int32_t* __restrict__ tile_count,
                   int32_t* __restrict__ meta) {
  __shared__ float sV[16], sP[16], sCam[3];
  __shared__ float sWf;
  __shared__ unsigned sStock[PROJ_THREADS / 32];
  __shared__ int sVis[PROJ_THREADS / 32];
  if (threadIdx.x < 16) { sV[threadIdx.x] = v.view[threadIdx.x]; sP[threadIdx.x] = v.proj[threadIdx.x]; }
  if (threadIdx.x == 32) {
    float a = 0.f;
    for (int r = 0; r < 3; r++) for (int c = 0; c < 3; c++) { const float w = v.view[r * 4 + c]; a += w * w; }
    sWf = a;
  }
  if ((USE_SH || LOG_SH) && threadIdx.x < 3) sCam[threadIdx.x] = v.campos[threadIdx.x];
  __syncthreads();
  int64_t i = (int64_t)blockIdx.x * PROJ_THREADS + threadIdx.x;
  int rad_out = 0;
  unsigned long long stock_tiles = 0;
  bool in_band = false;
  bool work = i < n;
  if (work && v.num_owners > 0) {
    float p[3], s[3];
    load3(means, i, p);
    load3(scales, i, s);
    const float4 q = ldg4(rots + 4 * i);
    float qn = q.x * q.x + q.y * q.y + q.z * q.z + q.w * q.w;
    if (v.raw_params) {
#pragma unroll
      for (int k = 0; k < 3; k++) s[k] = expf(s[k]);
      qn = qn > 1e-24f ? 1.0f : qn;
    }
    const float tz = p[0] * sV[2] + p[1] * sV[6] + p[2] * sV[10] + sV[14];
    if (!(tz > NEAR_Z)) work = false;
    else if (fabsf(qn - 1.0f) < 1e-3f) {
      const float ty = p[0] * sV[1] + p[1] * sV[5] + p[2] * sV[9] + sV[13];
      const float tx = p[0] * sV[0] + p[1] * sV[4] + p[2] * sV[8] + sV[12];
      const float itz = __fdividef(1.0f, tz);
      const float lx = fminf(CLAMP_FOV * v.tanfovx, fabsf(tx * itz)), ly = fminf(CLAMP_FOV * v.tanfovy, fabsf(ty * itz));
      const float jn = (v.fx * itz) * (v.fx * itz) * (1.0f + lx * lx) + (v.fy * itz) * (v.fy * itz) * (1.0f + ly * ly);
      const float sm = fmaxf(fabsf(s[0]), fmaxf(fabsf(s[1]), fabsf(s[2]))) * v.scale_mod;
      const float rb2 = 9.0f * (sWf * jn * sm * sm * 1.03f + 0.7f);
      const float hw = p[0] * sP[3] + p[1] * sP[7] + p[2] * sP[11] + sP[15];
      const float hy_ = p[0] * sP[1] + p[1] * sP[5] + p[2] * sP[9] + sP[13];
      const float py = (__fdividef(hy_, hw + 0.0000001f) * 1.00001f + 1.0f) * (0.5f * v.H) - 0.5f;
      const float lo = (float)(v.row0 * TILE) - (float)(TILE + 2), hi = (float)(v.row1 * TILE) + 3.0f;
      const float dist = fmaxf(fmaxf(lo - py, py - hi), 0.0f);
      if (dist * dist > rb2 * 1.02f + 4.0f * dist) work = false;
    }
  }
  if (v.num_owners > 0) {
    __shared__ int sSurv[PROJ_THREADS];
    __shared__ int sWcnt[PROJ_THREADS / 32];
    const int lane = threadIdx.x & 31, wid = threadIdx.x >> 5;
    if (!work && i < n) radii[i] = 0;
    const unsigned bal = __ballot_sync(0xffffffffu, work);
    if (lane == 0) sWcnt[wid] = __popc(bal);
    __syncthreads();
    int base = 0, total = 0;
#pragma unroll
    for (int w = 0; w < PROJ_THREADS / 32; w++) { const int c = sWcnt[w]; if (w < wid) base += c; total += c; }
    if (work) sSurv[base + __popc(bal & ((1u << lane) - 1u))] = threadIdx.x;
    __syncthreads();
    work = threadIdx.x < total;
    i = work ? (int64_t)blockIdx.x * PROJ_THREADS + sSurv[threadIdx.x] : n;
  }
  bool big_splat = false;
  int bx0 = 0, by0 = 0, bx1 = 0, by1 = 0;
  const int64_t src = (v.gather && work) ? v.gather[i] : i;
  if (work) {
    float p[3], Sg[9];
    load3(means, src, p);
    if (COV3D) {
      const float* c6 = v.cov3d + 6 * src;
      const float cxx = __ldg(c6), cxy = __ldg(c6 + 1), cxz = __ldg(c6 + 2), cyy = __ldg(c6 + 3), cyz = __ldg(c6 + 4), czz = __ldg(c6 + 5);
      Sg[0] = cxx; Sg[1] = cxy; Sg[2] = cxz; Sg[3] = cxy; Sg[4] = cyy; Sg[5] = cyz; Sg[6] = cxz; Sg[7] = cyz; Sg[8] = czz;
    } else {
      float s[3], R[9];
      load3(scales, src, s);
      float4 q = ldg4(rots + 4 * src);
      if (v.raw_params) {
        float inv;
#pragma unroll
        for (int k = 0; k < 3; k++) s[k] = expf(s[k]);
        q = act_normalize(q, inv);
      }
#pragma unroll
      for (int k = 0; k < 3; k++) s[k] *= v.scale_mod;
      quat_to_R(q, R);
      cov3d(s, R, Sg);
    }
    Cov2D cv;
    cov2d(sV, p, Sg, v.fx, v.fy, v.tanfovx, v.tanfovy, v.filter_mode, cv);
    float det;
    const float radf = radius_from_cov(cv.a, cv.b, cv.c, det);
    float4 r0 = make_float4(0.f, 0.f, 0.f, 0.f), r1 = r0, r2 = r0, r3 = r0;
    if (cv.t[2] > NEAR_Z && det > 0.0f) {
      float hom[4];
#pragma unroll
      for (int k = 0; k < 4; k++) hom[k] = p[0] * sP[k] + p[1] * sP[4 + k] + p[2] * sP[8 + k] + sP[12 + k];
      const float pw = 1.0f / (hom[3] + 0.0000001f);
      const float px = ((hom[0] * pw + 1.0f) * v.W - 1.0f) * 0.5f;
      const float py = ((hom[1] * pw + 1.0f) * v.H - 1.0f) * 0.5f;
      const int rad = (int)ceilf(radf);
      int x0, y0, x1, y1;
      tile_rect(px, py, rad, v.gx, v.gy, x0, y0, x1, y1);
      if ((x1 - x0) * (y1 - y0) > 0) {
        rad_out = rad;
        stock_tiles = (unsigned long long)((x1 - x0) * (max(0, min(y1, v.row1) - max(y0, v.row0))));
        in_band = stock_tiles > 0;
        const float idet = 1.0f / det;
        const float o = v.raw_params ? act_sigmoid(__ldg(opac + src)) : __ldg(opac + src);
        float hx = 0.f, hy = 0.f;
        bool reach = o * 255.0f >= 1.0f;
        if (reach) {
          const float q = 2.0f * logf(o * 255.0f) * 1.004f + 1e-3f;
          hx = sqrtf(q * cv.a) * 1.001f + 1e-3f;
          hy = sqrtf(q * cv.c) * 1.001f + 1e-3f;
        }
        float rgb[3];
        if (USE_SH) {
          float d[3] = {p[0] - sCam[0], p[1] - sCam[1], p[2] - sCam[2]};
          const float inv = 1.0f / sqrtf(d[0] * d[0] + d[1] * d[1] + d[2] * d[2]);
          float B[16];
          sh_basis(v.sh_degree, d[0] * inv, d[1] * inv, d[2] * inv, B);
          const int nb = (v.sh_degree + 1) * (v.sh_degree + 1);
          const float* sh = shs + src * v.sh_K * 3;
          rgb[0] = rgb[1] = rgb[2] = 0.5f;
          for (int k = 0; k < nb; k++) {
            rgb[0] += B[k] * __ldg(sh + 3 * k); rgb[1] += B[k] * __ldg(sh + 3 * k + 1); rgb[2] += B[k] * __ldg(sh + 3 * k + 2);
          }
          uint8_t cl = 0;
#pragma unroll
          for (int ch = 0; ch < 3; ch++) if (rgb[ch] < 0.0f) { cl |= (uint8_t)(1u << ch); rgb[ch] = 0.0f; }
          clamped[i] = cl;
        } else if (SIX) {
          const float* c6 = colors + 6 * src;
          rgb[0] = __ldg(c6); rgb[1] = __ldg(c6 + 1); rgb[2] = __ldg(c6 + 2);
          r3 = make_float4(__ldg(c6 + 3), __ldg(c6 + 4), __ldg(c6 + 5), 0.f);
        } else {
          load3(colors, src, rgb);
          if (v.raw_params) {
#pragma unroll
            for (int ch = 0; ch < 3; ch++) rgb[ch] = fmaf(SH_C0, rgb[ch], 0.5f);
          }
          if (LOG_SH && v.sh_degree > 0) {
            float d[3] = {p[0] - sCam[0], p[1] - sCam[1], p[2] - sCam[2]};
            const float inv = 1.0f / sqrtf(d[0] * d[0] + d[1] * d[1] + d[2] * d[2]);
            float B[16];
            sh_basis(v.sh_degree, d[0] * inv, d[1] * inv, d[2] * inv, B);
            const int nb = (v.sh_degree + 1) * (v.sh_degree + 1);
            const float* sh = shs + src * v.sh_K * 3;
            for (int k = 1; k < nb; k++) {
              rgb[0] += B[k] * __ldg(sh + 3 * (k - 1)); rgb[1] += B[k] * __ldg(sh + 3 * (k - 1) + 1);
              rgb[2] += B[k] * __ldg(sh + 3 * (k - 1) + 2);
            }
          }
        }
        const float kdet = LOG2E * idet;
        r0 = make_float4(px, py, cv.c * kdet, -cv.b * kdet);
        r1 = make_float4(cv.a * kdet, o, hx, hy);
        r2 = make_float4(rgb[0], rgb[1], rgb[2], cv.t[2]);
        if (DEPTH) r3 = make_float4(cv.t[2], p[2], 1.0f, 0.f);
        if (reach) {
          tile_rect_tight(px, py, rad, hx, hy, v.gx, v.gy, v.row0, v.row1, x0, y0, x1, y1);
          big_splat = count_small_tiles(v, tile_count, i, x0, y0, x1, y1);
          bx0 = x0; by0 = y0; bx1 = x1; by1 = y1;
        }
      }
    }
    if (v.num_owners == 0 || in_band) {
      float4* dst = reinterpret_cast<float4*>(splat + i * LGR_SPLAT_FLOATS);
      dst[0] = r0; dst[1] = r1; dst[2] = r2;
      if (SIX || DEPTH) reinterpret_cast<float4*>(v.splat_ext)[i] = r3;
    }
    radii[i] = rad_out;
    if (USE_SH && rad_out == 0) clamped[i] = 0;
  } else if (i < n) {
    radii[i] = 0;
  }
  warp_count_big_tiles(v, tile_count, big_splat, bx0, by0, bx1, by1);
  if (v.num_owners > 0) {
    __shared__ int sCnt[PROJ_THREADS / 32];
    const int lane = threadIdx.x & 31, wid = threadIdx.x >> 5;
    const unsigned bal = __ballot_sync(0xffffffffu, in_band);
    if (lane == 0) sCnt[wid] = __popc(bal);
    __syncthreads();
    int base = 0, total = 0;
#pragma unroll
    for (int w = 0; w < PROJ_THREADS / 32; w++) { const int c = sCnt[w]; if (w < wid) base += c; total += c; }
    if (in_band) v.band_ids[(int64_t)blockIdx.x * PROJ_THREADS + base + __popc(bal & ((1u << lane) - 1u))] = (int)i;
    if (threadIdx.x == 0) v.band_blk[blockIdx.x] = total;
    __syncthreads();
  }
  {
    const unsigned st_w = __reduce_add_sync(0xffffffffu, (unsigned)stock_tiles);
    const int vis_w = __popc(__ballot_sync(0xffffffffu, rad_out > 0));
    if ((threadIdx.x & 31) == 0) { sStock[threadIdx.x >> 5] = st_w; sVis[threadIdx.x >> 5] = vis_w; }
    __syncthreads();
    if (threadIdx.x == 0) {
      unsigned long long a = 0; int b = 0;
#pragma unroll
      for (int w = 0; w < PROJ_THREADS / 32; w++) { a += sStock[w]; b += sVis[w]; }
      if (a) atomicAdd(reinterpret_cast<unsigned long long*>(meta + 2), a);
      if (b) atomicAdd(meta + 4, b);
    }
  }
}

template <bool USE_SH, bool ROWS, bool LOG_SH = false, bool COV3D = false, bool SIX = false, bool DEPTH = false>
__global__ void __launch_bounds__(PROJ_THREADS)
project_bwd_kernel(View v, int64_t n, const float* __restrict__ means, const float* __restrict__ opac,
                   const float* __restrict__ scales, const float* __restrict__ rots, const float* __restrict__ shs, const int32_t* __restrict__ radii,
                   const uint8_t* __restrict__ clamped, const float* __restrict__ dsplat, float* __restrict__ dmeans,
                   float* __restrict__ dmeans2D, float* __restrict__ dopac, float* __restrict__ dscales,
                   float* __restrict__ drots, float* __restrict__ dcolors, float* __restrict__ dshs,
                   float* __restrict__ grad_rows, void* const* __restrict__ peer_stage, int my_rank) {
  __shared__ float sV[16], sP[16], sCam[3];
  if (threadIdx.x < 16) { sV[threadIdx.x] = v.view[threadIdx.x]; sP[threadIdx.x] = v.proj[threadIdx.x]; }
  if ((USE_SH || LOG_SH) && threadIdx.x < 3) sCam[threadIdx.x] = v.campos[threadIdx.x];
  __syncthreads();
  int64_t blk = blockIdx.x;
  if (ROWS && peer_stage) {
    int64_t first = 0;
    for (int o = 0; o <= my_rank && o < v.num_owners - 1; o++) first += v.band_count[o];
    if (my_rank == v.num_owners - 1) first = 0;
    blk = (blk + first / PROJ_THREADS) % gridDim.x;
  }
  int64_t i = blk * PROJ_THREADS + threadIdx.x;
  const bool active = i < n;
  if (!ROWS && !active) return;
  int64_t row = 0;
  if (ROWS && active) {
    row = i;
    i = v.band_rows[row];
  }
  float dm[3] = {0.f, 0.f, 0.f}, dm2[2] = {0.f, 0.f}, dop = 0.f, dsc[3] = {0.f, 0.f, 0.f}, dq[4] = {0.f, 0.f, 0.f, 0.f};
  float drgb[3] = {0.f, 0.f, 0.f}, dext[3] = {0.f, 0.f, 0.f};
  const bool live = active && radii[i] > 0;
  const int64_t src = (v.gather && live) ? v.gather[i] : i;
  const int K = v.sh_K;
  if (live) {
    const float4 g0 = ldg4(dsplat + i * LGR_GRAD_FLOATS);
    const float4 g1 = ldg4(dsplat + i * LGR_GRAD_FLOATS + 4);
    const float4 g2 = ldg4(dsplat + i * LGR_GRAD_FLOATS + 8);
    float p[3], s0[3], s[3], R[9], Sg[9];
    load3(means, src, p);
    float4 q = make_float4(1.f, 0.f, 0.f, 0.f);
    float q_inv = 1.0f;
    if (COV3D) {
      const float* c6 = v.cov3d + 6 * src;
      const float cxx = __ldg(c6), cxy = __ldg(c6 + 1), cxz = __ldg(c6 + 2), cyy = __ldg(c6 + 3), cyz = __ldg(c6 + 4), czz = __ldg(c6 + 5);
      Sg[0] = cxx; Sg[1] = cxy; Sg[2] = cxz; Sg[3] = cxy; Sg[4] = cyy; Sg[5] = cyz; Sg[6] = cxz; Sg[7] = cyz; Sg[8] = czz;
    } else {
      load3(scales, src, s0);
      q = ldg4(rots + 4 * src);
      if (v.raw_params) {
#pragma unroll
        for (int k = 0; k < 3; k++) s0[k] = expf(s0[k]);
        q = act_normalize(q, q_inv);
      }
#pragma unroll
      for (int k = 0; k < 3; k++) s[k] = s0[k] * v.scale_mod;
      quat_to_R(q, R);
      cov3d(s, R, Sg);
    }
    Cov2D cv;
    cov2d(sV, p, Sg, v.fx, v.fy, v.tanfovx, v.tanfovy, v.filter_mode, cv);
    dop = g1.y;
    drgb[0] = g1.z; drgb[1] = g1.w; drgb[2] = g2.x;
    if (SIX) { dext[0] = g2.y; dext[1] = g2.z; dext[2] = g2.w; }
    const float a = cv.a, b = cv.b, c = cv.c;
    const float det = a * c - b * b, idet2 = 1.0f / (det * det);
    float da = idet2 * (-c * c * g0.z + b * c * g0.w + (det - a * c) * g1.x);
    float dc = idet2 * (-a * a * g1.x + a * b * g0.w + (det - a * c) * g0.z);
    const float db = idet2 * (2.f * b * c * g0.z - (det + 2.f * b * b) * g0.w + 2.f * a * b * g1.x);
    if (v.filter_mode == LGR_FILTER_MAX) {
      if (!(cv.a_raw >= FILTER_VAR)) da = 0.f;
      if (!(cv.c_raw >= FILTER_VAR)) dc = 0.f;
    }
    const float G00 = da, G01 = 0.5f * db, G11 = dc;
    float GT[6];
#pragma unroll
    for (int j = 0; j < 3; j++) { GT[j] = G00 * cv.T[j] + G01 * cv.T[3 + j]; GT[3 + j] = G01 * cv.T[j] + G11 * cv.T[3 + j]; }
    float dS[9];
#pragma unroll
    for (int r = 0; r < 3; r++)
#pragma unroll
      for (int j = 0; j < 3; j++) dS[r * 3 + j] = cv.T[r] * GT[j] + cv.T[3 + r] * GT[3 + j];
    if (COV3D) {
      float* d6 = v.dcov3d + 6 * i;
      d6[0] = dS[0]; d6[1] = dS[1] + dS[3]; d6[2] = dS[2] + dS[6]; d6[3] = dS[4]; d6[4] = dS[5] + dS[7]; d6[5] = dS[8];
    }
    float dR[9];
    if (!COV3D) {
#pragma unroll
    for (int k = 0; k < 3; k++) {
      float acc = 0.f;
#pragma unroll
      for (int r = 0; r < 3; r++) {
        const float dMrk = 2.f * (dS[r * 3] * R[k] * s[k] + dS[r * 3 + 1] * R[3 + k] * s[k] + dS[r * 3 + 2] * R[6 + k] * s[k]);
        acc += dMrk * R[r * 3 + k];
        dR[r * 3 + k] = dMrk * s[k];
      }
      dsc[k] = acc * v.scale_mod;
    }
    {
      const float r = q.x, x = q.y, y = q.z, z = q.w;
      dq[0] = 2.f * (-z * dR[1] + y * dR[2] + z * dR[3] - x * dR[5] - y * dR[6] + x * dR[7]);
      dq[1] = 2.f * (y * dR[1] + z * dR[2] + y * dR[3] - 2.f * x * dR[4] - r * dR[5] + z * dR[6] + r * dR[7] - 2.f * x * dR[8]);
      dq[2] = 2.f * (-2.f * y * dR[0] + x * dR[1] + r * dR[2] + x * dR[3] + z * dR[5] - r * dR[6] + z * dR[7] - 2.f * y * dR[8]);
      dq[3] = 2.f * (-2.f * z * dR[0] - r * dR[1] + x * dR[2] + r * dR[3] - 2.f * z * dR[4] + y * dR[5] + x * dR[6] + y * dR[7]);
    }
    }
    float TS[6], dT[6];
#pragma unroll
    for (int r = 0; r < 2; r++)
#pragma unroll
      for (int j = 0; j < 3; j++) TS[r * 3 + j] = cv.T[r * 3] * Sg[j] + cv.T[r * 3 + 1] * Sg[3 + j] + cv.T[r * 3 + 2] * Sg[6 + j];
#pragma unroll
    for (int j = 0; j < 3; j++) { dT[j] = 2.f * (G00 * TS[j] + G01 * TS[3 + j]); dT[3 + j] = 2.f * (G01 * TS[j] + G11 * TS[3 + j]); }
    const float dJ00 = dT[0] * sV[0] + dT[1] * sV[4] + dT[2] * sV[8];
    const float dJ02 = dT[0] * sV[2] + dT[1] * sV[6] + dT[2] * sV[10];
    const float dJ11 = dT[3] * sV[1] + dT[4] * sV[5] + dT[5] * sV[9];
    const float dJ12 = dT[3] * sV[2] + dT[4] * sV[6] + dT[5] * sV[10];
    const float tz = cv.t[2], itz = 1.0f / tz, itz2 = itz * itz, itz3 = itz2 * itz;
    const float limx = CLAMP_FOV * v.tanfovx, limy = CLAMP_FOV * v.tanfovy;
    const float txc = fminf(limx, fmaxf(-limx, cv.t[0] * itz)) * tz, tyc = fminf(limy, fmaxf(-limy, cv.t[1] * itz)) * tz;
    float dt[3];
    dt[0] = cv.inx ? -v.fx * itz2 * dJ02 : 0.f;
    dt[1] = cv.iny ? -v.fy * itz2 * dJ12 : 0.f;
    dt[2] = -v.fx * itz2 * dJ00 - v.fy * itz2 * dJ11 + 2.f * v.fx * txc * itz3 * dJ02 + 2.f * v.fy * tyc * itz3 * dJ12;
#pragma unroll
    for (int r = 0; r < 3; r++) dm[r] = sV[r * 4] * dt[0] + sV[r * 4 + 1] * dt[1] + sV[r * 4 + 2] * dt[2];
// ... 341 lines not shown
```

log_b200/csrc/lgr_shard.cu:

```cuda
#include "lgr_common.cuh"
#include "lgr_prof.cuh"

namespace lgr {

constexpr int SHARD_THREADS = 256;
constexpr int SHARD_WARPS = SHARD_THREADS / 32;
constexpr int SHARD_MAX_RANKS = 32;
constexpr unsigned FULLMASK = 0xffffffffu;


__device__ __forceinline__ int owner_of_row(int y, int gy, int R) {
  const int base = gy / R, extra = gy - base * R;
  const int split = extra * (base + 1);
  return y < split ? y / (base + 1) : extra + (y - split) / max(base, 1);
}

__device__ __forceinline__ bool owner_range(const View& v, int R, const float* __restrict__ splat,
                                            const int32_t* __restrict__ radii, int64_t i, int64_t n, int& o0, int& o1) {
  o0 = 0; o1 = -1;
  if (i >= n) return false;
  const int rad = radii[i];
  if (rad <= 0) return false;
  const float4 r0 = ldg4(splat + i * LGR_SPLAT_FLOATS);
  const float4 r1 = ldg4(splat + i * LGR_SPLAT_FLOATS + 4);
  if (!(r1.z > 0.f)) return false;
  int x0, y0, x1, y1;
  tile_rect_tight(r0.x, r0.y, rad, r1.z, r1.w, v.gx, v.gy, 0, v.gy, x0, y0, x1, y1);
  if (x1 <= x0 || y1 <= y0) return false;
  o0 = owner_of_row(y0, v.gy, R);
  o1 = owner_of_row(y1 - 1, v.gy, R);
  return true;
}

__device__ __forceinline__ void count_owner_hits(bool valid, int o0, int o1, int R, int (*sW)[SHARD_WARPS]) {
  const int lane = threadIdx.x & 31, wid = threadIdx.x >> 5;
  for (int o = 0; o < R; o++) {
    const unsigned bal = __ballot_sync(FULLMASK, valid && o0 <= o && o <= o1);
    if (lane == 0) sW[o][wid] = __popc(bal);
  }
  __syncthreads();
}

__global__ void __launch_bounds__(SHARD_THREADS)
shard_count_kernel(View v, int R, int64_t n, const float* __restrict__ splat, const int32_t* __restrict__ radii,
                   int32_t* __restrict__ send_blk, int B) {
  __shared__ __align__(16) int sW[SHARD_MAX_RANKS][SHARD_WARPS];
  const int64_t i = (int64_t)blockIdx.x * SHARD_THREADS + threadIdx.x;
  int o0, o1;
  const bool valid = owner_range(v, R, splat, radii, i, n, o0, o1);
  count_owner_hits(valid, o0, o1, R, sW);
  if (threadIdx.x < R) {
    int t = 0;
#pragma unroll
    for (int w = 0; w < SHARD_WARPS; w++) t += sW[threadIdx.x][w];
    send_blk[(int64_t)threadIdx.x * B + blockIdx.x] = t;
  }
}

__global__ void __launch_bounds__(1024)
shard_scan_kernel(ShardLayout L, int B, int32_t* __restrict__ send_blk, void* const* __restrict__ peer_base) {
  __shared__ int warp_sum[32];
  __shared__ int carry_s;
  const int o = blockIdx.x, tid = threadIdx.x, lane = tid & 31, wid = tid >> 5;
  const int32_t* cnt = send_blk + (int64_t)o * B;
  int32_t* pre = send_blk + (int64_t)(L.R + o) * B;
  if (tid == 0) carry_s = 0;
  __syncthreads();
  for (int base = 0; base < B; base += 1024) {
    const int b = base + tid;
    const int c = b < B ? cnt[b] : 0;
    int x = c;
#pragma unroll
    for (int k = 1; k < 32; k <<= 1) { const int y = __shfl_up_sync(FULLMASK, x, k); if (lane >= k) x += y; }
    if (lane == 31) warp_sum[wid] = x;
    __syncthreads();
    if (wid == 0) {
      int w = warp_sum[lane];
#pragma unroll
      for (int k = 1; k < 32; k <<= 1) { const int y = __shfl_up_sync(FULLMASK, w, k); if (lane >= k) w += y; }
      warp_sum[lane] = w;
    }
    __syncthreads();
    const int carry = carry_s;
    if (b < B) pre[b] = carry + (wid ? warp_sum[wid - 1] : 0) + x - c;
    __syncthreads();
    if (tid == 1023) carry_s = carry + warp_sum[31];
    __syncthreads();
  }
  if (tid == 0) {
    const int total = carry_s;
    send_blk[(int64_t)2 * L.R * B + o] = total;
    reinterpret_cast<int32_t*>(reinterpret_cast<float*>(peer_base[o]) + L.off_count)[L.me] = total;
  }
}

__global__ void __launch_bounds__(SHARD_THREADS)
shard_push_kernel(View v, ShardLayout L, int64_t n, int64_t gid_base, const float* __restrict__ splat,
                  const int32_t* __restrict__ radii, const int32_t* __restrict__ send_blk, int B,
                  void* const* __restrict__ peer_base) {
  __shared__ __align__(16) int sW[SHARD_MAX_RANKS][SHARD_WARPS];
  __shared__ float4 sRows[SHARD_THREADS * 3];
  const int lane = threadIdx.x & 31, wid = threadIdx.x >> 5;
  const int64_t i = (int64_t)blockIdx.x * SHARD_THREADS + threadIdx.x;
  int o0, o1;
  const bool valid = owner_range(v, L.R, splat, radii, i, n, o0, o1);
  count_owner_hits(valid, o0, o1, L.R, sW);
  float4 r0, r1, r2;
  int rad = 0;
  if (valid) {
    r0 = ldg4(splat + i * LGR_SPLAT_FLOATS); r1 = ldg4(splat + i * LGR_SPLAT_FLOATS + 4);
    r2 = ldg4(splat + i * LGR_SPLAT_FLOATS + 8);
    rad = radii[i];
  }
  for (int o = 0; o < L.R; o++) {
    int cnt = 0, before = 0;
#pragma unroll
    for (int w = 0; w < SHARD_WARPS; w++) { const int c = sW[o][w]; if (w < wid) before += c; cnt += c; }
    if (cnt == 0) continue;
    const bool t = valid && o0 <= o && o <= o1;
    const unsigned bal = __ballot_sync(FULLMASK, t);
    const int first = send_blk[(int64_t)(L.R + o) * B + blockIdx.x];
    float* base = reinterpret_cast<float*>(peer_base[o]);
    const int64_t row0 = (int64_t)L.me * L.cap + first;
    if (t) {
      const int r = before + __popc(bal & ((1u << lane) - 1u));
      sRows[3 * r] = r0; sRows[3 * r + 1] = r1; sRows[3 * r + 2] = r2;
      reinterpret_cast<int32_t*>(base + L.off_radii)[row0 + r] = rad;
      reinterpret_cast<int32_t*>(base + L.off_gid)[row0 + r] = (int32_t)(gid_base + i);
    }
    __syncthreads();
    float4* dst = reinterpret_cast<float4*>(base + L.off_splat + row0 * LGR_SPLAT_FLOATS);
    for (int k = threadIdx.x; k < cnt * 3; k += SHARD_THREADS) dst[k] = sRows[k];
    __syncthreads();
  }
}

__global__ void __launch_bounds__(SHARD_THREADS)
shard_recv_count_kernel(View v, ShardLayout L, float* __restrict__ xbuf, float* __restrict__ dsplat,
                        int32_t* __restrict__ tile_count, int32_t* __restrict__ meta, float* __restrict__ pw_rows,
                        int32_t* __restrict__ pc_rows) {
  __shared__ __align__(16) unsigned sStock[SHARD_WARPS];
  __shared__ __align__(16) int sVis[SHARD_WARPS];
  __shared__ int64_t s_first[LGR_SHARD_MAX_RANKS + 1];
  const int64_t total = region_setup(v, s_first);
  const int32_t* radii = reinterpret_cast<const int32_t*>(xbuf + L.off_radii);
  unsigned stock = 0;
  int vis = 0;
  for (int64_t base = (int64_t)blockIdx.x * SHARD_THREADS; base < total; base += (int64_t)gridDim.x * SHARD_THREADS) {
    bool big_splat = false;
    int bx0 = 0, by0 = 0, bx1 = 0, by1 = 0;
    if (base + threadIdx.x < total) {
      const int64_t slot = region_row(v, s_first, base + threadIdx.x);
      const float* rec = xbuf + L.off_splat + slot * LGR_SPLAT_FLOATS;
      const float4 r0 = *reinterpret_cast<const float4*>(rec);
      const float4 r1 = *reinterpret_cast<const float4*>(rec + 4);
      const int rad = radii[slot];
      int x0, y0, x1, y1;
      tile_rect(r0.x, r0.y, rad, v.gx, v.gy, x0, y0, x1, y1);
      stock += (unsigned)((x1 - x0) * max(0, min(y1, v.row1) - max(y0, v.row0)));
      vis += 1;
      tile_rect_tight(r0.x, r0.y, rad, r1.z, r1.w, v.gx, v.gy, v.row0, v.row1, x0, y0, x1, y1);
      big_splat = count_small_tiles(v, tile_count, slot, x0, y0, x1, y1);
      bx0 = x0; by0 = y0; bx1 = x1; by1 = y1;
      float4* z = reinterpret_cast<float4*>(dsplat + slot * LGR_GRAD_FLOATS);
      z[0] = z[1] = z[2] = make_float4(0.f, 0.f, 0.f, 0.f);
      if (pw_rows) pw_rows[slot] = 0.f;
      if (pc_rows) pc_rows[slot] = 0;
    }
    warp_count_big_tiles(v, tile_count, big_splat, bx0, by0, bx1, by1);
  }
  const unsigned st_w = __reduce_add_sync(FULLMASK, stock);
  const int vis_w = __reduce_add_sync(FULLMASK, vis);
  if ((threadIdx.x & 31) == 0) { sStock[threadIdx.x >> 5] = st_w; sVis[threadIdx.x >> 5] = vis_w; }
  __syncthreads();
  if (threadIdx.x == 0) {
    unsigned long long a = 0; int b = 0;
#pragma unroll
    for (int w = 0; w < SHARD_WARPS; w++) { a += sStock[w]; b += sVis[w]; }
    if (a) atomicAdd(reinterpret_cast<unsigned long long*>(meta + 2), a);
    if (b) atomicAdd(meta + 4, b);
  }
}

template <typename T>
__global__ void __launch_bounds__(SHARD_THREADS)
shard_return_kernel(ShardLayout L, const float* __restrict__ xbuf, const T* __restrict__ rows, int items_per_row,
                    int64_t dst_off_floats, void* const* __restrict__ peer_base) {
  const int32_t* count = reinterpret_cast<const int32_t*>(xbuf + L.off_count);
  int64_t total = 0;
  for (int s = 0; s < L.R; s++) total += count[s];
  total *= items_per_row;
  for (int64_t t = (int64_t)blockIdx.x * SHARD_THREADS + threadIdx.x; t < total; t += (int64_t)gridDim.x * SHARD_THREADS) {
    int s = 0;
    int64_t first = 0;
    while (s + 1 < L.R && t >= first + (int64_t)count[s] * items_per_row) { first += (int64_t)count[s] * items_per_row; s++; }
    const int64_t k = t - first;
    T* dst = reinterpret_cast<T*>(reinterpret_cast<float*>(peer_base[s]) + dst_off_floats) +
             (int64_t)L.me * L.cap * items_per_row + k;
    *dst = rows[(int64_t)s * L.cap * items_per_row + k];
  }
}

__global__ void __launch_bounds__(SHARD_THREADS)
shard_return_packed_kernel(ShardLayout L, const float* __restrict__ xbuf, const float* __restrict__ dsplat_rows,
                           const float* __restrict__ pw_rows, const int32_t* __restrict__ pc_rows,
                           void* const* __restrict__ peer_base) {
  __shared__ int64_t first[SHARD_MAX_RANKS + 1];
  if (threadIdx.x == 0) {
    const int32_t* count = reinterpret_cast<const int32_t*>(xbuf + L.off_count);
    int64_t acc = 0;
    for (int s = 0; s < L.R; s++) { first[s] = acc; acc += (int64_t)count[s] * 3; }
    first[L.R] = acc;
  }
  __syncthreads();
  const int64_t total = first[L.R], stride = (int64_t)gridDim.x * SHARD_THREADS;
  constexpr int U = 4;
  for (int64_t t0 = (int64_t)blockIdx.x * SHARD_THREADS + threadIdx.x; t0 < total; t0 += U * stride) {
    float4 val[U];
    float4* dst[U];
#pragma unroll
    for (int u = 0; u < U; u++) {
      const int64_t t = t0 + u * stride;
      dst[u] = nullptr;
      if (t < total) {
        int s = 0;
        while (s + 1 < L.R && t >= first[s + 1]) s++;
        const int64_t k = t - first[s];
        const int64_t row = (int64_t)s * L.cap + k / 3;
        const int part = (int)(k % 3);
        val[u] = reinterpret_cast<const float4*>(dsplat_rows)[row * 3 + part];
        if (part == 2) {
          val[u].y = pw_rows ? pw_rows[row] : 0.f;
          val[u].z = pc_rows ? __int_as_float(pc_rows[row]) : 0.f;
        }
        dst[u] = reinterpret_cast<float4*>(reinterpret_cast<float*>(peer_base[s]) + L.off_dsplat) + (int64_t)L.me * L.cap * 3 + k;
      }
    }
#pragma unroll
    for (int u = 0; u < U; u++)
      if (dst[u]) *dst[u] = val[u];
  }
}

__global__ void __launch_bounds__(SHARD_THREADS)
shard_gather_kernel(View v, ShardLayout L, int64_t n, const float* __restrict__ splat, const int32_t* __restrict__ radii,
                    const int32_t* __restrict__ send_blk, int B, const float* __restrict__ xbuf,
                    float* __restrict__ dsplat_out, float* __restrict__ weight_out, int32_t* __restrict__ pcount_out, int packed) {
  __shared__ __align__(16) int sW[SHARD_MAX_RANKS][SHARD_WARPS];
  const int lane = threadIdx.x & 31, wid = threadIdx.x >> 5;
  const int64_t i = (int64_t)blockIdx.x * SHARD_THREADS + threadIdx.x;
  int o0, o1;
  const bool valid = owner_range(v, L.R, splat, radii, i, n, o0, o1);
  count_owner_hits(valid, o0, o1, L.R, sW);
  float4 a = make_float4(0.f, 0.f, 0.f, 0.f), b = a, c = a;
  unsigned wmax = 0u;
  int pc = 0;
  for (int o = 0; o < L.R; o++) {
    const bool t = valid && o0 <= o && o <= o1;
    const unsigned bal = __ballot_sync(FULLMASK, t);
    if (!t) continue;
    int before = 0;
#pragma unroll
    for (int w = 0; w < SHARD_WARPS; w++) if (w < wid) before += sW[o][w];
    const int64_t row = (int64_t)o * L.cap + send_blk[(int64_t)(L.R + o) * B + blockIdx.x] + before +
                        __popc(bal & ((1u << lane) - 1u));
    const float4* g = reinterpret_cast<const float4*>(xbuf + L.off_dsplat + row * LGR_GRAD_FLOATS);
    const float4 g0 = g[0], g1 = g[1], g2 = g[2];
    a.x += g0.x; a.y += g0.y; a.z += g0.z; a.w += g0.w;
    b.x += g1.x; b.y += g1.y; b.z += g1.z; b.w += g1.w;
    c.x += g2.x;
    if (packed) {
      if (weight_out) wmax = max(wmax, __float_as_uint(g2.y));
      if (pcount_out) pc += __float_as_int(g2.z);
    } else {
      c.y += g2.y; c.z += g2.z; c.w += g2.w;
      if (weight_out) wmax = max(wmax, reinterpret_cast<const unsigned*>(xbuf + L.off_weight)[row]);
      if (pcount_out) pc += reinterpret_cast<const int32_t*>(xbuf + L.off_pcount)[row];
    }
  }
  if (i < n) {
    float4* d = reinterpret_cast<float4*>(dsplat_out + i * LGR_GRAD_FLOATS);
    d[0] = a; d[1] = b; d[2] = c;
    if (weight_out) weight_out[i] = __uint_as_float(wmax);
    if (pcount_out) pcount_out[i] = pc;
  }
}

static inline unsigned blocks_for(int64_t n) { return (unsigned)((n + SHARD_THREADS - 1) / SHARD_THREADS); }

int launch_shard_send(const View& v, const ShardLayout& L, int64_t n, int64_t gid_base, const float* splat,
                      const int32_t* radii, int32_t* send_blk, void* const* peer_base, cudaStream_t st) {
  const int B = (int)blocks_for(n > 0 ? n : 1);
  ProfScope ps(K_SHARD_SEND, st, n > 0 ? 3 : 1);
  if (n > 0) {
    shard_count_kernel<<<B, SHARD_THREADS, 0, st>>>(v, L.R, n, splat, radii, send_blk, B);
    LGR_CHECK_LAUNCH();
  } else {
    cudaError_t e = cudaMemsetAsync(send_blk, 0, sizeof(int32_t) * (size_t)L.R * B, st);
    if (e != cudaSuccess) return (int)e;
  }
  shard_scan_kernel<<<L.R, 1024, 0, st>>>(L, B, send_blk, peer_base);
  LGR_CHECK_LAUNCH();
  if (n > 0) {
    shard_push_kernel<<<B, SHARD_THREADS, 0, st>>>(v, L, n, gid_base, splat, radii, send_blk, B, peer_base);
    LGR_CHECK_LAUNCH();
  }
  return 0;
}

int launch_shard_recv_count(const View& v, const ShardLayout& L, float* xbuf, float* dsplat, int32_t* tile_count, int32_t* meta,
                            float* pw_rows, int32_t* pc_rows, cudaStream_t st) {
  const int64_t total = (int64_t)L.R * L.cap;
  if (total <= 0) return 0;
  if (!v.region_count) return LGR_E_BADARG;
  int64_t blocks = blocks_for(total);
  if (blocks > LGR_REGION_GRID) blocks = LGR_REGION_GRID;
  ProfScope ps(K_SHARD_RECV, st);
  shard_recv_count_kernel<<<(unsigned)blocks, SHARD_THREADS, 0, st>>>(v, L, xbuf, dsplat, tile_count, meta, pw_rows, pc_rows);
  LGR_CHECK_LAUNCH();
  return 0;
}

// ... 41 lines not shown
```

log_b200/rasterizer.py:

```python
import ctypes
from typing import NamedTuple, Optional

import torch
import torch.nn as nn

from . import _capi
from ._capi import LGR_FILTER_ADD, LGR_FILTER_MAX, LGR_FILTER_NONE, LgrView

PREZERO_DSPLAT = bool(int(__import__('os').environ.get('LGR_PREZERO_DSPLAT', '0')))
RANKED_BIN = bool(int(__import__('os').environ.get('LGR_RANKED_BIN', '1')))
CONTRIB_BITS = bool(int(__import__('os').environ.get('LGR_CONTRIB_BITS', '1')))
FLAVOUR_STOCK = 'stock'
FLAVOUR_FORK = 'fork'


class GaussianRasterizationSettings(NamedTuple):
    image_height: int
    image_width: int
    tanfovx: float
    tanfovy: float
    bg: torch.Tensor
    scale_modifier: float
    viewmatrix: torch.Tensor
    projmatrix: torch.Tensor
    sh_degree: int
    campos: torch.Tensor
    prefiltered: bool
    debug: bool


def _ptr(t: Optional[torch.Tensor]):
    return None if t is None or t.numel() == 0 else ctypes.c_void_p(t.data_ptr())


def _f32c(t: Optional[torch.Tensor], name: str, device=None):
    if t is None:
        return None
    _capi.require_cuda(t, name)
    if device is not None and t.device != device:
        raise _capi.LgrError(f'{name} is on {t.device}, expected {device}')
    if t.dtype != torch.float32:
        raise TypeError(f'{name} must be float32, got {t.dtype}')
    t = t.detach()
    if not t.is_contiguous():
        t = t.contiguous()
    if t.data_ptr() % 16:
        t = t.clone()
    return t


def _stream(device=None):
    return _capi.current_stream(device)


def _make_view(s: GaussianRasterizationSettings, filter_mode: int, want_aux: bool, sh_coeffs: int, tile_rows, keep,
               num_owners=0, band_ids=None, band_count=None, band_blk=None, band_rows=None, band_dsplat=None,
               raw_params=False, tile_rank=None, gather_index=None, pid_map=None, cov3D_precomp=None, splat_ext=None,
               log_depth=False):
    dev = s.viewmatrix.device
    vm, pm = _f32c(s.viewmatrix, 'viewmatrix'), _f32c(s.projmatrix, 'projmatrix', dev)
    bg = _f32c(s.bg, 'bg', dev)
    cp = _f32c(s.campos, 'campos', dev) if s.campos is not None else None
    keep.extend([vm, pm, bg, cp])
    v = LgrView()
    v.image_height, v.image_width = int(s.image_height), int(s.image_width)
    v.tanfovx, v.tanfovy = float(s.tanfovx), float(s.tanfovy)
    v.scale_modifier = float(s.scale_modifier)
    v.sh_degree, v.sh_coeffs = int(s.sh_degree), int(sh_coeffs)
    v.filter_mode, v.want_aux = int(filter_mode), int(bool(want_aux))
    v.tile_row_begin, v.tile_row_end = (0, 0) if tile_rows is None else (int(tile_rows[0]), int(tile_rows[1]))
    v.num_owners = int(num_owners)
    v.raw_params = int(bool(raw_params))
    v.band_ids_d = band_ids.data_ptr() if band_ids is not None else None
    v.band_count_d = band_count.data_ptr() if band_count is not None else None
    v.band_blk_d = band_blk.data_ptr() if band_blk is not None else None
    v.band_rows_d = band_rows.data_ptr() if band_rows is not None else None
    v.band_dsplat_d = band_dsplat.data_ptr() if band_dsplat is not None else None
    v.tile_rank_d = tile_rank.data_ptr() if tile_rank is not None else None
    v.gather_index_d = gather_index.data_ptr() if gather_index is not None else None
    v.pid_map_d = pid_map.data_ptr() if pid_map is not None else None
    v.cov3D_precomp_d = cov3D_precomp.data_ptr() if cov3D_precomp is not None else None
    if splat_ext is not None:
        v.num_channels, v.splat_ext_d = 6, splat_ext.data_ptr()
        v.log_depth = int(bool(log_depth))
    v.viewmatrix_d, v.projmatrix_d = vm.data_ptr(), pm.data_ptr()
    v.campos_d = cp.data_ptr() if cp is not None else None
    v.bg_d = bg.data_ptr()
    return v


def set_contrib_lists(view, buf, D, n_contrib):
    if buf is None:
        view.contrib_id_d = view.contrib_entry_d = view.contrib_count_d = view.last_contrib_d = None
        return
    p = buf.data_ptr()
    view.contrib_id_d, view.contrib_entry_d, view.contrib_count_d = p, p + 4 * D, p + 8 * D
    view.last_contrib_d = n_contrib.data_ptr()


def colour_channels(colors_precomp, settings, shs=None, raw_params=False, gather_index=None, num_owners=0, log_depth=False):
    width = None
    if colors_precomp is not None:
        width = int(colors_precomp.shape[-1]) if colors_precomp.dim() > 0 else 0
        if width not in (3, 6):
            raise _capi.LgrError(f'colors_precomp must have 3 or 6 channels per Gaussian, got shape {tuple(colors_precomp.shape)}')
    if log_depth:
        if width == 6:
            raise _capi.LgrError('render_depth generates the depth channels itself: pass three-channel colors_precomp (N,3), '
                                 'not (N,6)')
        if num_owners > 0:
            raise _capi.LgrError('render_depth is not available in band mode (num_owners > 0)')
        return 6
    if width is None or width == 3:
        return 3
    if colors_precomp.dim() != 2:
        raise _capi.LgrError(f'six-channel colors_precomp must be (N,6), got shape {tuple(colors_precomp.shape)}')
    for what, used in (('shs', shs is not None), ('raw_params', raw_params), ('gather_index (render_gathered)', gather_index is not None),
                       ('band mode (num_owners > 0)', num_owners > 0)):
        if used:
            raise _capi.LgrError(f'six colour channels (colors_precomp (N,6)) are not available with {what}')
    if settings.bg.numel() != 6:
        raise _capi.LgrError(f'six colour channels need a background of 6 entries (raster_settings.bg), got {settings.bg.numel()}')
    return 6


def use_contrib_lists(D, max_tile_len):
    return CONTRIB_BITS and D > 0 and (max_tile_len is None or max_tile_len <= _capi.LGR_CONTRIB_MAX_LIST)


class RasterState:
    __slots__ = ('view', 'keep', 'n', 'num_instances', 'max_tile_len', 'stock_instances', 'num_visible', 'splat',
                 'radii', 'clamped', 'tile_start', 'sorted_ids', 'final_T', 'n_contrib', 'image', 'sh', 'num_owners',
                 'band_ids', 'band_count', 'band_counts_host', 'point_count', 'meta', 'cov3D', 'dcov3D', 'contrib',
                 'channels', 'splat_ext', 'log_depth')

    def read_stats(self):
        m = self.meta.tolist()
        return dict(num_instances=int(m[0]), max_tile_len=int(m[1]), stock_instances=(m[2] & 0xffffffff) | ((m[3] & 0xffffffff) << 32),
                    num_visible=int(m[4]), overflow=int(m[6]))

    def contrib_lists(self):
        if self.contrib is None:
            return None
        D = self.num_instances
        return self.contrib[:D], self.contrib[D:2 * D], self.contrib[2 * D:]


def rasterize_forward(settings, means3D, opacities, scales, rotations, colors_precomp, shs, filter_mode, want_aux,
                      tile_rows=None, num_owners=0, raw_params=False, prezero_dsplat=None, gather_index=None,
                      instance_capacity=None, cov3D_precomp=None, log_depth=False):
    channels = colour_channels(colors_precomp, settings, shs, raw_params, gather_index, num_owners, log_depth)
    if log_depth:
        bg3 = settings.bg.reshape(-1)[:3]
        settings = settings._replace(bg=torch.cat([bg3, bg3]))
    lib = _capi.load()
    dev = means3D.device
    if cov3D_precomp is not None and (raw_params or num_owners > 0):
        raise _capi.LgrError('cov3D_precomp is not available with raw_params or in band mode')
    for name, t in (('opacities', opacities), ('scales', scales), ('rotations', rotations), ('colors_precomp', colors_precomp),
                    ('shs', shs), ('cov3D_precomp', cov3D_precomp), ('viewmatrix', settings.viewmatrix), ('projmatrix', settings.projmatrix), ('bg', settings.bg)):
        if t is not None and t.device != dev:
            raise _capi.LgrError(f'{name} is on {t.device}, means3D on {dev}: all inputs of a call must share one device')
    n = int(means3D.shape[0])
    keep = []
    if gather_index is not None:
        if gather_index.dtype != torch.int64 or gather_index.device != dev or gather_index.dim() != 1:
            raise _capi.LgrError('gather_index must be a 1-D int64 tensor on the inputs\' device')
        if num_owners > 0:
            raise _capi.LgrError('gather_index is not available in band mode')
        gather_index = gather_index.contiguous()
        keep.append(gather_index)
        n = int(gather_index.shape[0])
    K = 0 if shs is None else int(shs.shape[1])
    band_ids = band_count = band_blk = band_rows = band_dsplat = None
    if prezero_dsplat is None:
        prezero_dsplat = PREZERO_DSPLAT and torch.is_grad_enabled()
    if num_owners == 0 and prezero_dsplat:
        band_dsplat = torch.empty((max(n, 1), _capi.LGR_GRAD_FLOATS), dtype=torch.float32, device=dev)
    if num_owners > 0:
        band_rows = torch.empty((max(n, 1),), dtype=torch.int32, device=dev)
        band_dsplat = torch.empty((max(n, 1), _capi.LGR_GRAD_FLOATS), dtype=torch.float32, device=dev)
        nb = (n + 255) // 256
        band_ids = torch.empty((max(256 * nb, 1),), dtype=torch.int32, device=dev)
        band_blk = torch.empty((2 * nb + 1,), dtype=torch.int32, device=dev)
        band_count = torch.empty((num_owners,), dtype=torch.int32, device=dev)
    tile_rank = torch.empty((max(n, 1), 4), dtype=torch.int32, device=dev) if RANKED_BIN else None
    keep.append(tile_rank)
    splat_ext = torch.empty((max(n, 1), 4), dtype=torch.float32, device=dev) if channels == 6 else None
    keep.append(splat_ext)
    view = _make_view(settings, filter_mode, want_aux, K, tile_rows, keep, num_owners, band_ids, band_count, band_blk, band_rows, band_dsplat,
                      raw_params, tile_rank, gather_index, cov3D_precomp=cov3D_precomp, splat_ext=splat_ext, log_depth=log_depth)
    H, W = view.image_height, view.image_width
    gx, gy = (W + 15) // 16, (H + 15) // 16
    rows = gy if tile_rows is None else int(tile_rows[1]) - int(tile_rows[0])
    ntiles = gx * rows
    i32 = dict(dtype=torch.int32, device=dev)
    f32 = dict(dtype=torch.float32, device=dev)
    splat = torch.empty((n, _capi.LGR_SPLAT_FLOATS), **f32)
    radii = torch.empty((n,), **i32)
    clamped = torch.empty((n,), dtype=torch.uint8, device=dev) if shs is not None else None
    tile_start = torch.empty((ntiles + 1,), **i32)
    tile_cursor = torch.empty((_capi.LGR_TILE_SCRATCH_INTS * max(ntiles, 1),), **i32)
    meta = torch.empty((_capi.LGR_META_INTS,), **i32)
    st = _stream(dev)
    _capi.check(lib.lgr_forward_project(ctypes.byref(view), n, _ptr(means3D), _ptr(opacities), _ptr(scales),
                                        _ptr(rotations), _ptr(colors_precomp), _ptr(shs), _ptr(splat), _ptr(radii),
                                        _ptr(clamped), _ptr(tile_start), _ptr(tile_cursor), _ptr(meta), st),
                'lgr_forward_project')
    u32 = dict(dtype=torch.int32, device=dev)
    image = torch.empty((channels, H, W), **f32) if tile_rows is None else torch.zeros((channels, H, W), **f32)
    final_T = torch.empty((H, W), **f32) if tile_rows is None else torch.ones((H, W), **f32)
    n_contrib = torch.empty((H, W), **i32) if tile_rows is None else torch.zeros((H, W), **i32)
    pid = pwp = pw = pc = None
    if want_aux:
        pc = torch.zeros((n,), **i32)
        pid = torch.empty((H, W), **i32) if tile_rows is None else torch.full((H, W), -1, **i32)
        pwp = torch.empty((H, W), **f32) if tile_rows is None else torch.zeros((H, W), **f32)
        pw = torch.zeros((n,), **f32)
    if instance_capacity:
        if num_owners > 0:
            raise _capi.LgrError('instance_capacity (device-sized call) is not available in band mode')
        D, max_len, num_long, stock_D, m = int(instance_capacity), None, None, None, None
        inst_key, inst_val = torch.empty((D,), **u32), torch.empty((D,), **u32)
        sorted_ids = torch.empty((D,), **i32)
        contrib = torch.empty((2 * D + ntiles,), **i32) if use_contrib_lists(D, None) else None
        keep.append(contrib)
        set_contrib_lists(view, contrib, D, n_contrib)
        _capi.check(lib.lgr_forward_render_device_sized(ctypes.byref(view), n, D, _ptr(meta), _ptr(splat), _ptr(radii), _ptr(tile_start),
                                                        _ptr(tile_cursor), _ptr(inst_key), _ptr(inst_val), _ptr(sorted_ids), _ptr(image),
                                                        _ptr(final_T), _ptr(n_contrib), _ptr(pid), _ptr(pwp), _ptr(pw), _ptr(pc), st),
                    'lgr_forward_render_device_sized')
    else:
        m = (meta if band_count is None else torch.cat([meta, band_count])).tolist()
        D, max_len, num_long = int(m[0]), int(m[1]), int(m[5])
        stock_D = (m[2] & 0xffffffff) | ((m[3] & 0xffffffff) << 32)
        if D < 0 or stock_D > 0x7fffffff:
            raise _capi.LgrError(f'this view needs {stock_D} (Gaussian, tile) instances by the stock rule (D = {m[0] & 0xffffffff} binned, '
                                 f'{m[4]} of {n} Gaussians visible, longest tile list {max_len}): more than 2^31 - 1 is unsupported')
        inst_key = torch.empty((D,), **u32)
        inst_val = torch.empty((D,), **u32)
        inst_tmp = torch.empty((2 * D,), **u32) if max_len > lib.lgr_sort_smem_capacity() else None
        sorted_ids = torch.empty((D,), **i32)
        contrib = torch.empty((2 * D + ntiles,), **i32) if use_contrib_lists(D, max_len) else None
        keep.append(contrib)
        set_contrib_lists(view, contrib, D, n_contrib)
        _capi.check(lib.lgr_forward_render(ctypes.byref(view), n, D, max_len, num_long, _ptr(splat), _ptr(radii), _ptr(tile_start),
                                           _ptr(tile_cursor), _ptr(inst_key), _ptr(inst_val), _ptr(inst_tmp),
                                           _ptr(sorted_ids), _ptr(image), _ptr(final_T), _ptr(n_contrib), _ptr(pid),
                                           _ptr(pwp), _ptr(pw), _ptr(pc), st), 'lgr_forward_render')
    s = RasterState()
    s.view, s.keep, s.n, s.num_instances, s.max_tile_len = view, keep, n, D, max_len
    s.stock_instances, s.num_visible = stock_D, (int(m[4]) if m is not None else None)
    s.meta = meta
    s.cov3D, s.dcov3D = cov3D_precomp, None
    s.splat, s.radii, s.clamped, s.tile_start, s.sorted_ids = splat, radii, clamped, tile_start, sorted_ids
    s.final_T, s.n_contrib, s.image, s.sh = final_T, n_contrib, image, shs is not None
    s.point_count = pc
    s.contrib = contrib
    s.channels, s.splat_ext, s.log_depth = channels, splat_ext, bool(log_depth)
    s.num_owners, s.band_ids, s.band_count = num_owners, (band_ids, band_blk, band_rows, band_dsplat), band_count
    s.band_counts_host = [int(x) for x in m[_capi.LGR_META_INTS:]] if num_owners > 0 else None
    return image, radii, pid, pwp, pw, s


def rasterize_backward(state: RasterState, grad_image, means3D, opacities, scales, rotations, colors_precomp, shs,
                       peer_stage=None, my_rank=0):
    lib = _capi.load()
    dev = means3D.device
    n = state.n
    f32 = dict(dtype=torch.float32, device=dev)
    g = _f32c(grad_image, 'grad_image', dev)
    if state.band_ids[3] is not None:
        dsplat = state.band_ids[3]
        state.band_ids = state.band_ids[:3] + (None,)
    else:
        dsplat = torch.zeros((n, _capi.LGR_GRAD_FLOATS), **f32)
    if state.num_owners > 0:
        m_rows = sum(state.band_counts_host)
        if peer_stage is not None:
            _capi.check(lib.lgr_backward(ctypes.byref(state.view), n, state.num_instances, _ptr(means3D), _ptr(opacities),
                                         _ptr(scales), _ptr(rotations), _ptr(colors_precomp), None, _ptr(state.splat),
                                         _ptr(state.radii), None, _ptr(state.tile_start), _ptr(state.sorted_ids),
                                         _ptr(state.image), _ptr(g), _ptr(dsplat), None, None, None, None, None, None, None,
                                         None, ctypes.c_void_p(peer_stage.data_ptr()), int(my_rank), m_rows, _stream(dev)), 'lgr_backward')
            return None
        rows = torch.empty((m_rows, _capi.LGR_ROW_FLOATS), **f32)
        _capi.check(lib.lgr_backward(ctypes.byref(state.view), n, state.num_instances, _ptr(means3D), _ptr(opacities),
                                     _ptr(scales), _ptr(rotations), _ptr(colors_precomp), None, _ptr(state.splat),
                                     _ptr(state.radii), None, _ptr(state.tile_start), _ptr(state.sorted_ids),
                                     _ptr(state.image), _ptr(g), _ptr(dsplat), None, None, None, None, None, None, None,
                                     ctypes.c_void_p(rows.data_ptr()) if rows.numel() else _ptr(dsplat), None, 0, m_rows, _stream(dev)),
                    'lgr_backward')
        return rows
    dmeans3D = torch.empty((n, 3), **f32)
    dmeans2D = torch.empty((n, 3), **f32)
    dopac = torch.empty((n,), **f32)
    cov = state.cov3D is not None
    dscales = None if cov else torch.empty((n, 3), **f32)
    drot = None if cov else torch.empty((n, 4), **f32)
    if cov:
        state.dcov3D = torch.empty((n, 6), **f32)
        state.view.dcov3D_d = state.dcov3D.data_ptr()
    dcolors = torch.empty((n, 3 if state.log_depth else state.channels), **f32) if colors_precomp is not None else None
    dshs = torch.empty((n,) + tuple(shs.shape[1:]), **f32) if shs is not None else None
    _capi.check(lib.lgr_backward(ctypes.byref(state.view), n, state.num_instances, _ptr(means3D), _ptr(opacities),
                                 _ptr(scales), _ptr(rotations), _ptr(colors_precomp), _ptr(shs), _ptr(state.splat),
                                 _ptr(state.radii), _ptr(state.clamped), _ptr(state.tile_start), _ptr(state.sorted_ids),
                                 _ptr(state.image), _ptr(g), _ptr(dsplat), _ptr(dmeans3D),
                                 _ptr(dmeans2D), _ptr(dopac), _ptr(dscales), _ptr(drot), _ptr(dcolors), _ptr(dshs), None,
                                 None, 0, 0, _stream(dev)), 'lgr_backward')
    return dmeans3D, dmeans2D, dopac, dscales, drot, dcolors, dshs


def point_id_count(point_count: torch.Tensor):
    lib = _capi.load()
    n = int(point_count.shape[0])
    dev = point_count.device
    i32 = dict(dtype=torch.int32, device=dev)
    scratch = torch.empty((2 * ((n + 1023) // 1024) + 1,), **i32)
    ids = torch.empty((n,), **i32)
    cnt = torch.empty((n,), **i32)
    num = torch.empty((1,), **i32)
    _capi.check(lib.lgr_point_compact(n, _ptr(point_count), _ptr(scratch), _ptr(ids), _ptr(cnt),
                                      ctypes.c_void_p(num.data_ptr()), _stream(dev)), 'lgr_point_compact')
    k = int(num.item())
    return ids[:k], cnt[:k]


class _RasterizeGaussians(torch.autograd.Function):

    @staticmethod
    def forward(ctx, means3D, means2D, opacities, colors_precomp, shs, scales, rotations, settings, filter_mode, want_aux,
                tile_rows, raw_params=False, prezero_dsplat=False, instance_capacity=None, holder=None, cov3D_precomp=None,
                log_depth=False):
        dev = means3D.device
        m = _f32c(means3D, 'means3D')
        o = _f32c(opacities, 'opacities', dev)
        cov = _f32c(cov3D_precomp, 'cov3D_precomp', dev)
        sc = _f32c(scales, 'scales', dev) if cov is None else None
        r = _f32c(rotations, 'rotations', dev) if cov is None else None
        c = _f32c(colors_precomp, 'colors_precomp', dev)
        sh = _f32c(shs, 'shs', dev)
        image, radii, pid, pwp, pw, state = rasterize_forward(settings, m, o, sc, r, c, sh, filter_mode, want_aux, tile_rows,
                                                              raw_params=raw_params, prezero_dsplat=prezero_dsplat,
                                                              instance_capacity=instance_capacity, cov3D_precomp=cov,
                                                              log_depth=log_depth)
        if holder is not None:
            holder['state'] = state
        state.image = None
        ctx.state = state
        ctx.opacity_shape = opacities.shape
        none = torch.empty(0, device=dev)
        ctx.save_for_backward(m, o, sc if sc is not None else none, r if r is not None else none, c if c is not None else none,
                              sh if sh is not None else none, image, cov if cov is not None else none)
        ctx.has_color, ctx.has_sh, ctx.has_cov = c is not None, sh is not None, cov is not None
        ctx.debug = bool(getattr(settings, 'debug', False))
        if want_aux:
            ctx.mark_non_differentiable(radii, pid, pwp, pw, state.point_count)
            return image, radii, pid, pwp, pw, state.point_count
        ctx.mark_non_differentiable(radii)
        return image, radii

    @staticmethod
    def backward(ctx, grad_image, *unused):
        m, o, sc, r, c, sh, image, cov = ctx.saved_tensors
        c = c if ctx.has_color else None
        sh = sh if ctx.has_sh else None
        if ctx.has_cov:
            sc = r = None
            ctx.state.cov3D = cov
        ctx.state.image = image
        dm3, dm2, dop, dsc, drot, dcol, dsh = rasterize_backward(ctx.state, grad_image, m, o, sc, r, c, sh)
        ctx.state.image = None
        if ctx.debug and m.is_cuda:
            torch.cuda.synchronize(m.device)
        return (dm3, dm2, dop.reshape(ctx.opacity_shape), dcol, dsh, dsc, drot, None, None, None, None, None, None, None, None,
                ctx.state.dcov3D, None)


class GaussianRasterizer(nn.Module):
    flavour = FLAVOUR_FORK

    def __init__(self, raster_settings):
        super().__init__()
        self.raster_settings = raster_settings
        self.tile_rows = None
        self.instance_capacity = None
        self.last_state = None

    def markVisible(self, positions):
        lib = _capi.load()
        p = _f32c(positions.detach(), 'positions')
        V = _f32c(self.raster_settings.viewmatrix, 'viewmatrix', p.device)
        out = torch.empty((int(p.shape[0]),), dtype=torch.uint8, device=p.device)
        _capi.check(lib.lgr_mark_visible(int(p.shape[0]), _ptr(p), _ptr(V), _ptr(out), _stream(p.device)), 'lgr_mark_visible')
        return out.bool()

    def compute_radius(self, xyz, scaling, rotation):
        s = self.raster_settings
        return compute_radius(xyz, scaling, rotation, s.projmatrix, s.viewmatrix,
                              s.image_width / (2.0 * s.tanfovx), s.image_height / (2.0 * s.tanfovy), s.tanfovx, s.tanfovy)

# ... 48 lines not shown
```

log_b200/sharded.py:

```python
from typing import List, Tuple

import torch
import torch.distributed as dist

GRAD_FLOATS_PRECOMP = 17


def tile_row_partition(image_height: int, world_size: int) -> List[Tuple[int, int]]:
    gy = (image_height + 15) // 16
    base, extra = divmod(gy, world_size)
    out, start = [], 0
    for r in range(world_size):
        n = base + (1 if r < extra else 0)
        out.append((start, start + n))
        start += n
    return out


def owner_chunk(num_gaussians: int, world_size: int) -> int:
    return ((num_gaussians + world_size - 1) // world_size + 255) // 256 * 256


def owner_partition(num_gaussians: int, world_size: int) -> List[Tuple[int, int]]:
    chunk = owner_chunk(num_gaussians, world_size)
# ... 56 lines not shown

class PeerExchange:

    def __init__(self, num_gaussians: int, group=None):
        import torch.distributed._symmetric_memory as symm
        from . import _capi
        self.group = group if group is not None else dist.group.WORLD
        self.world, self.rank = dist.get_world_size(self.group), dist.get_rank(self.group)
        self.n = int(num_gaussians)
        self.chunk = owner_chunk(self.n, self.world)
        dev = torch.device('cuda', torch.cuda.current_device())
        floats = _capi.LGR_STAGE_HEADER_FLOATS + self.world * self.chunk * _capi.LGR_ROW_FLOATS
        self.stage = symm.empty(floats, dtype=torch.float32, device=dev)
        self.stage[:_capi.LGR_STAGE_HEADER_FLOATS].zero_()
        self.handle = symm.rendezvous(self.stage, self.group)
        self.peer_ptrs = torch.tensor(list(self.handle.buffer_ptrs), dtype=torch.int64, device=dev)
        self.lo, self.hi = owner_partition(self.n, self.world)[self.rank]
        self.handle.barrier()

    def backward(self, state, grad_image, means3D, opacities, scales, rotations, colors_precomp) -> torch.Tensor:
        import ctypes
        from . import _capi
        from .rasterizer import rasterize_backward
        lib = _capi.load()
        self.handle.barrier()
        rasterize_backward(state, grad_image, means3D, opacities, scales, rotations, colors_precomp, None,
                           peer_stage=self.peer_ptrs, my_rank=self.rank)
        self.handle.barrier()
        shard = torch.zeros((self.chunk, _capi.LGR_ROW_FLOATS), dtype=torch.float32, device=self.stage.device)
        _capi.check(lib.lgr_grad_scatter_add_staged(ctypes.c_void_p(self.stage.data_ptr()), self.world, self.chunk, self.lo,
                                                    self.hi, ctypes.c_void_p(shard.data_ptr()),
                                                    _capi.current_stream()),
                    'lgr_grad_scatter_add_staged')
        return shard


def owner_of_row(tile_row: int, image_height: int, world_size: int) -> int:
    gy = (image_height + 15) // 16
    base, extra = divmod(gy, world_size)
    split = extra * (base + 1)
    return tile_row // (base + 1) if tile_row < split else extra + (tile_row - split) // max(base, 1)


def shard_layout(num_gaussians: int, world_size: int, rank: int):
    from . import _capi
    cap = owner_chunk(num_gaussians, world_size)
    rows = world_size * cap
    off = 0

    def take(floats):
        nonlocal off
        o = off
        off += (floats + 63) // 64 * 64
        return o
    lay = _capi.LgrShardLayout()
    lay.num_ranks, lay.my_rank, lay.cap = world_size, rank, cap
    lay.off_count = take(max(world_size, 64))
    lay.off_splat = take(rows * _capi.LGR_SPLAT_FLOATS)
    lay.off_radii = take(rows)
    lay.off_gid = take(rows)
    lay.off_dsplat = take(rows * _capi.LGR_GRAD_FLOATS)
    lay.off_weight = take(rows)
    lay.off_pcount = take(rows)
    return lay, off


class ShardStep:
    pass


class SplatExchange:

    def __init__(self, num_gaussians: int, image_height: int, rank: int, world: int, own_buffer, peer_ptrs, barrier):
        from . import _capi
        self.n, self.rank, self.world = int(num_gaussians), int(rank), int(world)
        if not 0 < self.world <= _capi.LGR_SHARD_MAX_RANKS:
            raise ValueError(f'shard mode supports 1..{_capi.LGR_SHARD_MAX_RANKS} ranks, got {world}')
        self.layout, self.floats = shard_layout(self.n, self.world, self.rank)
        self.cap = int(self.layout.cap)
        self.lo, self.hi = owner_partition(self.n, self.world)[self.rank]
        self.band = tile_row_partition(image_height, self.world)[self.rank]
        self.image_height = int(image_height)
        peer_ptrs = [int(p) for p in peer_ptrs]
        _capi.require_cuda(own_buffer, 'the exchange buffer')
        if own_buffer.dtype != torch.float32 or own_buffer.numel() < self.floats:
            raise ValueError(f'the exchange buffer must be a float32 tensor of >= {self.floats} elements')
        if len(peer_ptrs) != self.world or peer_ptrs[self.rank] != own_buffer.data_ptr():
            raise ValueError('peer_ptrs needs one address per rank, entry `rank` being own_buffer')
        self.buf, self.barrier = own_buffer, barrier
        dev = self.buf.device
        self.peer_ptrs = torch.tensor(peer_ptrs, dtype=torch.int64, device=dev)
        L, rows = self.layout, self.world * self.cap
        self.count = self.buf[L.off_count:L.off_count + self.world].view(torch.int32)
        self.header = self.buf[L.off_count:L.off_count + 40].view(torch.int32)
        self.meta = self.header[32:40]
        self.recv_splat = self.buf[L.off_splat:L.off_splat + rows * 12].view(rows, 12)
        self.recv_radii = self.buf[L.off_radii:L.off_radii + rows].view(torch.int32)
        self.recv_gid = self.buf[L.off_gid:L.off_gid + rows].view(torch.int32)
        self.dsplat_rows = torch.empty((rows, _capi.LGR_GRAD_FLOATS), dtype=torch.float32, device=dev)
        self.count.zero_()
        self.recv_radii.zero_()
        self._cache = {}
        self._in_flight = False
        import os
        self.sync_free = bool(int(os.environ.get('LGR_SYNC_FREE', '0')))
        self._inst_cap = 0

    def _scratch(self, name: str, shape, dtype):
        need = 1
        for d in shape:
            need *= int(d)
        t = self._cache.get(name)
        if t is None or t.numel() < need or t.dtype != dtype:
            t = torch.empty((max(need, 1) * 5 // 4 + 64,), dtype=dtype, device=self.buf.device)
            self._cache[name] = t
        return t[:need].view(*shape)

    @classmethod
    def over_symmetric_memory(cls, num_gaussians: int, image_height: int, group=None):
        import torch.distributed._symmetric_memory as symm
        group = group if group is not None else dist.group.WORLD
        world, rank = dist.get_world_size(group), dist.get_rank(group)
        _, floats = shard_layout(num_gaussians, world, rank)
        dev = torch.device('cuda', torch.cuda.current_device())
        buf = symm.empty(floats, dtype=torch.float32, device=dev)
        handle = symm.rendezvous(buf, group)
        self = cls(num_gaussians, image_height, rank, world, buf, list(handle.buffer_ptrs), handle.barrier)
        self.handle = handle
        handle.barrier()
        return self

    def project_and_send(self, settings, means3D, opacities, scales, rotations, colors_precomp=None, shs=None,
                         filter_mode=None, want_aux=True, raw_params=False, render_depth=False) -> ShardStep:
        import ctypes
        from . import _capi
        from .rasterizer import _f32c, _make_view, _ptr, _stream
        lib = _capi.load()
        if render_depth:
            raise _capi.LgrError('render_depth is not available in shard mode: the exchange moves three-channel records only')
        if colors_precomp is not None and int(colors_precomp.shape[-1]) != 3:
            raise _capi.LgrError(f'shard mode renders three precomputed colour channels, got colors_precomp {tuple(colors_precomp.shape)}')
        filter_mode = _capi.LGR_FILTER_MAX if filter_mode is None else filter_mode
        dev = self.buf.device
        n = int(means3D.shape[0])
        if n != self.hi - self.lo:
            raise ValueError(f'rank {self.rank} owns Gaussians [{self.lo},{self.hi}): expected {self.hi - self.lo} rows, got {n}')
        s = ShardStep()
        s.inputs = tuple(_f32c(t, k, dev) for k, t in (('means3D', means3D), ('opacities', opacities), ('scales', scales),
                                                       ('rotations', rotations), ('colors_precomp', colors_precomp), ('shs', shs)))
        m, o, sc, r, c, sh = s.inputs
        s.keep, s.n, s.want_aux, s.settings = [], n, bool(want_aux), settings
        K = 0 if sh is None else int(sh.shape[1])
        s.view_full = _make_view(settings, filter_mode, want_aux, K, None, s.keep, raw_params=raw_params)
        from .rasterizer import RANKED_BIN
        rank_rows = self._scratch('tile_rank', (self.world * self.cap, 4), torch.int32) if RANKED_BIN else None
        s.view_band = _make_view(settings, filter_mode, want_aux, K, self.band, s.keep, raw_params=raw_params, tile_rank=rank_rows,
                                 pid_map=self.recv_gid)
        s.view_band.region_count_d = self.buf.data_ptr() + 4 * int(self.layout.off_count)
        s.view_band.region_cap, s.view_band.num_regions = self.cap, self.world
        H, W = s.view_full.image_height, s.view_full.image_width
        if H != self.image_height:
            raise ValueError('image height differs from the one the bands were cut for')
        gx, gy = (W + 15) // 16, (H + 15) // 16
        i32 = dict(dtype=torch.int32, device=dev)
        s.splat = self._scratch('splat', (n, _capi.LGR_SPLAT_FLOATS), torch.float32)
        s.radii = torch.empty((n,), **i32)
        s.clamped = self._scratch('clamped', (n,), torch.uint8) if sh is not None else None
        s.tile_start_full = self._scratch('tile_start_full', (gx * gy + 1,), torch.int32)
        cursor = self._scratch('cursor_full', (_capi.LGR_TILE_SCRATCH_INTS * gx * gy,), torch.int32)
        meta = self._scratch('meta_full', (_capi.LGR_META_INTS,), torch.int32)
        st = _stream()
        _capi.check(lib.lgr_forward_project(ctypes.byref(s.view_full), n, _ptr(m), _ptr(o), _ptr(sc), _ptr(r), _ptr(c), _ptr(sh),
                                            _ptr(s.splat), _ptr(s.radii), _ptr(s.clamped), _ptr(s.tile_start_full), _ptr(cursor),
                                            _ptr(meta), st), 'lgr_forward_project')
        s.send_scratch = self._scratch('send', (_capi.shard_send_ints(n, self.world),), torch.int32)
        _capi.check(lib.lgr_shard_send(ctypes.byref(s.view_full), ctypes.byref(self.layout), n, self.lo, _ptr(s.splat),
                                       _ptr(s.radii), _ptr(s.send_scratch), ctypes.c_void_p(self.peer_ptrs.data_ptr()), st),
                    'lgr_shard_send')
        return s

    def receive_and_render(self, s: ShardStep):
        import ctypes
        from . import _capi
        from .rasterizer import _ptr, _stream, set_contrib_lists, use_contrib_lists
        lib = _capi.load()
        dev = self.buf.device
        v = s.view_band
        H, W = v.image_height, v.image_width
        gx = (W + 15) // 16
        ntiles = gx * (self.band[1] - self.band[0])
        rows = self.world * self.cap
        i32, f32 = dict(dtype=torch.int32, device=dev), dict(dtype=torch.float32, device=dev)
        s.tile_start = self._scratch('tile_start', (ntiles + 1,), torch.int32)
        cursor = self._scratch('cursor', (_capi.LGR_TILE_SCRATCH_INTS * max(ntiles, 1),), torch.int32)
        meta = self.meta
        st = _stream()
        s.pw_rows = s.pc_rows = None
        if s.want_aux:
            s.pw_rows = self._scratch('pw_rows', (rows,), torch.float32)
            s.pc_rows = self._scratch('pc_rows', (rows,), torch.int32)
        _capi.check(lib.lgr_shard_recv_bin_aux(ctypes.byref(v), ctypes.byref(self.layout), _ptr(self.buf), _ptr(self.dsplat_rows),
                                               _ptr(s.tile_start), _ptr(cursor), _ptr(meta), _ptr(s.pw_rows), _ptr(s.pc_rows), st),
                    'lgr_shard_recv_bin_aux')
        s.image = torch.zeros((3, H, W), **f32)
        final_T = self._scratch('final_T', (H, W), torch.float32)
        n_contrib = self._scratch('n_contrib', (H, W), torch.int32)
        pid = pwp = None
        if s.want_aux:
            pid = torch.full((H, W), -1, **i32)
            pwp = torch.zeros((H, W), **f32)
        if self.sync_free and self._inst_cap > 0:
            cap = self._inst_cap
            inst_key = self._scratch('inst_key', (cap,), torch.int32)
            inst_val = self._scratch('inst_val', (cap,), torch.int32)
            s.sorted_ids = self._scratch('sorted_ids', (cap,), torch.int32)
            set_contrib_lists(v, self._scratch('contrib', (2 * cap + ntiles,), torch.int32) if use_contrib_lists(cap, None) else None,
                              cap, n_contrib)
            s.num_instances, s.max_tile_len, s.num_rows, s.stock_instances = cap, None, None, None
            _capi.check(lib.lgr_forward_render_device_sized(ctypes.byref(v), rows, cap, _ptr(meta), _ptr(self.recv_splat), _ptr(self.recv_radii),
                                                            _ptr(s.tile_start), _ptr(cursor), _ptr(inst_key), _ptr(inst_val), _ptr(s.sorted_ids),
                                                            _ptr(s.image), _ptr(final_T), _ptr(n_contrib), _ptr(pid), _ptr(pwp),
                                                            _ptr(s.pw_rows), _ptr(s.pc_rows), st), 'lgr_forward_render_device_sized')
            return s.image, s.radii, pid, pwp
        h = self.header.tolist()
        m = h[32:40]
        D, max_len, num_long = int(m[0]), int(m[1]), int(m[5])
        s.num_instances, s.max_tile_len, s.num_rows = D, max_len, int(sum(h[:self.world]))
        s.stock_instances = (m[2] & 0xffffffff) | ((m[3] & 0xffffffff) << 32)
        if max_len <= lib.lgr_sort_smem_capacity():
            self._inst_cap = max(self._inst_cap, D + D // 4 + 4096)
        inst_key = self._scratch('inst_key', (D,), torch.int32)
        inst_val = self._scratch('inst_val', (D,), torch.int32)
        inst_tmp = self._scratch('inst_tmp', (2 * D,), torch.int32) if max_len > lib.lgr_sort_smem_capacity() else None
        s.sorted_ids = self._scratch('sorted_ids', (D,), torch.int32)
        set_contrib_lists(v, self._scratch('contrib', (2 * D + ntiles,), torch.int32) if use_contrib_lists(D, max_len) else None,
                          D, n_contrib)
        _capi.check(lib.lgr_forward_render(ctypes.byref(v), rows, D, max_len, num_long, _ptr(self.recv_splat), _ptr(self.recv_radii),
                                           _ptr(s.tile_start), _ptr(cursor), _ptr(inst_key), _ptr(inst_val), _ptr(inst_tmp),
                                           _ptr(s.sorted_ids), _ptr(s.image), _ptr(final_T), _ptr(n_contrib), _ptr(pid), _ptr(pwp),
                                           _ptr(s.pw_rows), _ptr(s.pc_rows), st), 'lgr_forward_render')
        return s.image, s.radii, pid, pwp

    def stats(self):
        h = self.header.tolist()
        m = h[32:40]
        return dict(num_rows=int(sum(h[:self.world])), num_instances=int(m[0]), max_tile_len=int(m[1]),
                    stock_instances=(m[2] & 0xffffffff) | ((m[3] & 0xffffffff) << 32), overflow=int(m[6]))

    def check_overflow(self):
        st = self.stats()
        if st['overflow']:
            self._inst_cap = 0
            raise RuntimeError(f'shard-mode step outgrew its device-sized buffers (flags {st["overflow"]}, D = {st["num_instances"]}, '
                               f'longest tile list {st["max_tile_len"]}): its outputs are invalid, redo the step')
        return st

    def blend_backward_and_return(self, s: ShardStep, grad_image):
        import ctypes
        from . import _capi
        from .rasterizer import _f32c, _ptr, _stream
        lib = _capi.load()
        s.grad_image = _f32c(grad_image, 'grad_image', self.buf.device)
        st, L, peers = _stream(), self.layout, ctypes.c_void_p(self.peer_ptrs.data_ptr())
        rows = self.world * self.cap
        _capi.check(lib.lgr_blend_backward(ctypes.byref(s.view_band), rows, s.num_instances, _ptr(self.recv_splat),
                                           _ptr(s.tile_start), _ptr(s.sorted_ids), _ptr(s.image), _ptr(s.grad_image),
                                           _ptr(self.dsplat_rows), st), 'lgr_blend_backward')
        _capi.check(lib.lgr_shard_return_packed(ctypes.byref(L), _ptr(self.buf), _ptr(self.dsplat_rows), _ptr(s.pw_rows), _ptr(s.pc_rows),
                                                peers, st), 'lgr_shard_return_packed')

    def gather_and_project_backward(self, s: ShardStep):
        import ctypes
        from . import _capi
        from .rasterizer import _ptr, _stream
        lib = _capi.load()
        dev = self.buf.device
        n = s.n
        m, o, sc, r, c, sh = s.inputs
        f32 = dict(dtype=torch.float32, device=dev)
        dsplat = self._scratch('dsplat_local', (n, _capi.LGR_GRAD_FLOATS), torch.float32)
        pw = torch.empty((n,), **f32) if s.want_aux else None
        pc = torch.empty((n,), dtype=torch.int32, device=dev) if s.want_aux else None
        st = _stream()
        _capi.check(lib.lgr_shard_gather_packed(ctypes.byref(s.view_full), ctypes.byref(self.layout), n, _ptr(s.splat), _ptr(s.radii),
                                                _ptr(s.send_scratch), _ptr(self.buf), _ptr(dsplat), _ptr(pw), _ptr(pc), st),
                    'lgr_shard_gather_packed')
        dmeans3D, dmeans2D = torch.empty((n, 3), **f32), torch.empty((n, 3), **f32)
        dopac, dscales, drot = torch.empty((n,), **f32), torch.empty((n, 3), **f32), torch.empty((n, 4), **f32)
        dcolors = torch.empty((n, 3), **f32) if c is not None else None
        dshs = torch.empty_like(sh) if sh is not None else None
        if n:
            _capi.check(lib.lgr_backward(ctypes.byref(s.view_full), n, 0, _ptr(m), _ptr(o), _ptr(sc), _ptr(r), _ptr(c), _ptr(sh),
                                         _ptr(s.splat), _ptr(s.radii), _ptr(s.clamped), _ptr(s.tile_start_full), None,
                                         _ptr(s.image), _ptr(s.grad_image), _ptr(dsplat), _ptr(dmeans3D), _ptr(dmeans2D),
                                         _ptr(dopac), _ptr(dscales), _ptr(drot), _ptr(dcolors), _ptr(dshs), None, None, 0, 0, st),
                        'lgr_backward')
        return (dmeans3D, dmeans2D, dopac, dscales, drot, dcolors, dshs), pw, pc

    def forward(self, settings, means3D, opacities, scales, rotations, colors_precomp=None, shs=None, **kw):
        if self._in_flight:
            self.barrier()
        self._in_flight = True
        s = self.project_and_send(settings, means3D, opacities, scales, rotations, colors_precomp, shs, **kw)
        self.barrier()
        return self.receive_and_render(s) + (s,)

    def backward(self, s: ShardStep, grad_image):
        self.blend_backward_and_return(s, grad_image)
        self.barrier()
        self._in_flight = False
        return self.gather_and_project_backward(s)


class _ShardRasterize(torch.autograd.Function):

    @staticmethod
    def forward(ctx, xch, settings, kw, means3D, means2D, opacities, scales, rotations, colors_precomp, shs):
        image, radii, pid, pwp, step = xch.forward(settings, means3D, opacities.reshape(-1), scales, rotations, colors_precomp, shs, **kw)
        ctx.xch, ctx.step, ctx.opacity_shape = xch, step, opacities.shape
        outs = (image, radii) if pid is None else (image, radii, pid, pwp)
        ctx.mark_non_differentiable(*outs[1:])
        return outs

    @staticmethod
    def backward(ctx, grad_image, *unused):
        (dm3, dm2, dop, dsc, drot, dcol, dsh), pw, pc = ctx.xch.backward(ctx.step, grad_image)
        ctx.xch.last_point_weight, ctx.xch.last_point_count = pw, pc
        return None, None, None, dm3, dm2, dop.reshape(ctx.opacity_shape), dsc, drot, dcol, dsh


def _rasterize(self, settings, means3D, means2D, opacities, scales, rotations, colors_precomp=None, shs=None, **kw):
    return _ShardRasterize.apply(self, settings, kw, means3D, means2D, opacities, scales, rotations, colors_precomp, shs)


SplatExchange.rasterize = _rasterize
```

Baseline: 1.688 billion.

## Replace ranked binning with per-tile fixed-capacity key/value slabs written during projection

Removes the tile_rank path, which precomputed per-Gaussian tile ranks. In its place, keys and values go into per-tile slabs of fixed capacity, sized to the sort's shared-memory capacity, so the separate bin_scatter pass and the global inst_key/inst_val buffers can be skipped when every tile fits. Tiles that overflow the slab raise an overflow flag. The cost is a large preallocated slab of ntiles times capacity entries, reads from scattered slab memory in the sort, and a fallback when tile lists exceed the slab size.

```diff
diff --git a/include/log_b200_raster.h b/include/log_b200_raster.h
--- a/include/log_b200_raster.h
+++ b/include/log_b200_raster.h
@@ -7,7 +7,7 @@
 extern "C" {
 #endif
 
-#define LGR_ABI_VERSION 19
+#define LGR_ABI_VERSION 20
 #define LGR_TILE 16
 
 #define LGR_FILTER_ADD 0
@@ -34,7 +34,9 @@
   int32_t* band_count_d;
   int32_t* band_rows_d;
   float* band_dsplat_d;
-  int32_t* tile_rank_d;
+  uint32_t* slab_key_d;
+  uint32_t* slab_val_d;
+  int32_t slab_cap;
   const int64_t* gather_index_d;
   const int32_t* pid_map_d;
   int32_t* contrib_id_d;
diff --git a/log_b200/_capi.py b/log_b200/_capi.py
--- a/log_b200/_capi.py
+++ b/log_b200/_capi.py
@@ -10,7 +10,7 @@
 LGR_GRAD_FLOATS = 12
 LGR_META_INTS = 8
 LGR_TILE_SCRATCH_INTS = 33
-LGR_ABI_VERSION = 19
+LGR_ABI_VERSION = 20
 LGR_CONTRIB_MAX_LIST = 1 << 24
 LGR_STAGE_HEADER_FLOATS = 64
 LGR_ROW_FLOATS = 20
@@ -27,7 +27,7 @@
     _fields_ = [('image_height', _i32), ('image_width', _i32), ('tanfovx', _f32), ('tanfovy', _f32),
                 ('scale_modifier', _f32), ('sh_degree', _i32), ('sh_coeffs', _i32), ('filter_mode', _i32),
                 ('want_aux', _i32), ('tile_row_begin', _i32), ('tile_row_end', _i32),
-                ('num_owners', _i32), ('raw_params', _i32), ('band_ids_d', _vp), ('band_blk_d', _vp), ('band_count_d', _vp), ('band_rows_d', _vp), ('band_dsplat_d', _vp), ('tile_rank_d', _vp), ('gather_index_d', _vp), ('pid_map_d', _vp), ('contrib_id_d', _vp), ('contrib_entry_d', _vp), ('contrib_count_d', _vp), ('last_contrib_d', _vp),
+                ('num_owners', _i32), ('raw_params', _i32), ('band_ids_d', _vp), ('band_blk_d', _vp), ('band_count_d', _vp), ('band_rows_d', _vp), ('band_dsplat_d', _vp), ('slab_key_d', _vp), ('slab_val_d', _vp), ('slab_cap', _i32), ('gather_index_d', _vp), ('pid_map_d', _vp), ('contrib_id_d', _vp), ('contrib_entry_d', _vp), ('contrib_count_d', _vp), ('last_contrib_d', _vp),
                 ('region_count_d', _vp), ('region_cap', _i64), ('num_regions', _i32), ('num_channels', _i32), ('log_depth', _i32), ('splat_ext_d', _vp), ('cov3D_precomp_d', _vp), ('dcov3D_d', _vp),
                 ('viewmatrix_d', _vp), ('projmatrix_d', _vp), ('campos_d', _vp), ('bg_d', _vp)]
 
diff --git a/log_b200/csrc/lgr_bin.cu b/log_b200/csrc/lgr_bin.cu
--- a/log_b200/csrc/lgr_bin.cu
+++ b/log_b200/csrc/lgr_bin.cu
@@ -9,7 +9,7 @@
 __global__ void __launch_bounds__(SCAN_THREADS)
 tile_scan_kernel(int ntiles, int32_t* __restrict__ tile_start ,
                  int32_t* __restrict__ cursor ,
-                 int32_t* __restrict__ meta, int small_cap, int ranked) {
+                 int32_t* __restrict__ meta, int small_cap) {
   __shared__ int warp_sum[SCAN_THREADS / 32];
   __shared__ int carry_s, maxl_s, nbig_s;
   const int tid = threadIdx.x, lane = tid & 31, wid = tid >> 5;
@@ -18,7 +18,7 @@
   int local_max = 0;
   for (int base = 0; base < ntiles; base += SCAN_THREADS) {
     const int i = base + tid;
-    const int c = (i < ntiles) ? cursor[i * CSTRIDE] + cursor[i * CSTRIDE + 1] : 0;
+    const int c = (i < ntiles) ? cursor[i * CSTRIDE] : 0;
     local_max = max(local_max, c);
     int x = c;
 #pragma unroll
@@ -35,7 +35,7 @@
     const int carry = carry_s;
     const int excl = carry + (wid ? warp_sum[wid - 1] : 0) + x - c;
     if (i < ntiles) {
-      tile_start[i] = excl; cursor[i * CSTRIDE + ranked] = 0;
+      tile_start[i] = excl; cursor[i * CSTRIDE] = 0;
       if (c > small_cap) cursor[CSTRIDE * ntiles + atomicAdd(&nbig_s, 1)] = i;
     }
     __syncthreads();
@@ -77,13 +77,11 @@
   int rad = 0;
   float4 r0 = make_float4(0.f, 0.f, 0.f, 0.f), r1 = r0;
   float depth = 0.f;
-  int4 rk = make_int4(-1, -1, -1, -1);
   if (live) {
     rad = radii[i];
     r0 = ldg4(splat + i * LGR_SPLAT_FLOATS);
     r1 = ldg4(splat + i * LGR_SPLAT_FLOATS + 4);
     depth = __ldg(splat + i * LGR_SPLAT_FLOATS + 11);
-    if (v.tile_rank) rk = __ldg(reinterpret_cast<const int4*>(v.tile_rank + 4 * i));
     live = rad > 0;
   }
   if (live && v.num_owners == 0 && v.band_dsplat) {
@@ -107,12 +105,8 @@
       const int ty = y0 + k / max(w, 1), tx = x0 + k % max(w, 1);
       t[k] = k < cnt ? (ty - v.row0) * v.gx + tx : -1;
     }
-    if (v.tile_rank) {
-      slot[0] = rk.x; slot[1] = rk.y; slot[2] = rk.z; slot[3] = rk.w;
-    } else {
-#pragma unroll
-      for (int k = 0; k < 4; k++) slot[k] = t[k] >= 0 ? atomicAdd(cursor + t[k] * CSTRIDE, 1) : 0;
-    }
+#pragma unroll
+    for (int k = 0; k < 4; k++) slot[k] = t[k] >= 0 ? atomicAdd(cursor + t[k] * CSTRIDE, 1) : 0;
 #pragma unroll
     for (int k = 0; k < 4; k++)
       if (t[k] >= 0) {
@@ -120,7 +114,7 @@
         if (pos < capacity) { inst_key[pos] = key; inst_val[pos] = (uint32_t)i; }
       }
   }
-  const int lane = threadIdx.x & 31, big = v.tile_rank ? 1 : 0;
+  const int lane = threadIdx.x & 31;
   unsigned todo = __ballot_sync(0xffffffffu, cnt > 4);
   while (todo) {
     const int src = __ffs(todo) - 1;
@@ -131,7 +125,7 @@
     const uint32_t bid = (uint32_t)__shfl_sync(0xffffffffu, (int)i, src);
     for (int k = lane; k < bcnt; k += 32) {
       const int t = (by0 + k / bw - v.row0) * v.gx + bx0 + k % bw;
-      const int pos = tile_start[t] + (big ? cursor[t * CSTRIDE] : 0) + atomicAdd(cursor + t * CSTRIDE + big, 1);
+      const int pos = tile_start[t] + atomicAdd(cursor + t * CSTRIDE, 1);
       if (pos < capacity) { inst_key[pos] = bkey; inst_val[pos] = bid; }
     }
   }
@@ -327,7 +321,8 @@
 tile_sort_kernel(const int32_t* __restrict__ tile_list ,
                  const int32_t* __restrict__ tile_start, uint32_t* __restrict__ inst_key,
                  uint32_t* __restrict__ inst_val, uint32_t* __restrict__ tmp, int32_t* __restrict__ sorted_ids, int lo,
-                 int cap, int id_bits, const int32_t* __restrict__ count_ptr, int32_t* __restrict__ flags) {
+                 int cap, int id_bits, const int32_t* __restrict__ count_ptr, int32_t* __restrict__ flags,
+                 const uint32_t* __restrict__ slab_key, const uint32_t* __restrict__ slab_val, int slab_cap) {
   extern __shared__ uint32_t smem_u32[];
   __shared__ int whist[MODE == 1 ? SORT_WARPS * RADIX : 1];
   __shared__ MsdShared msd;
@@ -336,13 +331,15 @@
     const int t = tile_list ? tile_list[b] : b;
     const int beg = tile_start[t], len = tile_start[t + 1] - beg;
     if (len <= lo) continue;
-    if (MODE == 0 && len > cap) {
-      if (flags && lo > 0 && threadIdx.x == 0) atomicOr(flags, 2);
+    if (MODE == 0 && (len > cap || (slab_cap > 0 && len > slab_cap))) {
+      if (flags && (lo > 0 || (slab_cap > 0 && len > slab_cap)) && threadIdx.x == 0) atomicOr(flags, 2);
       continue;
     }
     if (MODE == 0) {
       uint32_t* kA = smem_u32; uint32_t* vA = kA + cap; uint32_t* kB = vA + cap; uint32_t* vB = kB + cap;
-      for (int i = threadIdx.x; i < len; i += SORT_THREADS) { kA[i] = inst_key[beg + i]; vA[i] = inst_val[beg + i]; }
+      const uint32_t* srck = slab_cap > 0 ? slab_key + (int64_t)t * slab_cap : inst_key + beg;
+      const uint32_t* srcv = slab_cap > 0 ? slab_val + (int64_t)t * slab_cap : inst_val + beg;
+      for (int i = threadIdx.x; i < len; i += SORT_THREADS) { kA[i] = srck[i]; vA[i] = srcv[i]; }
       __syncthreads();
       if (len > 1 && !sort_tile_msd(kA, vA, kB, vB, len, msd)) __trap();
       for (int i = threadIdx.x; i < len; i += SORT_THREADS) sorted_ids[beg + i] = (int32_t)vA[i];
@@ -442,9 +439,9 @@
   return 0;
 }
 
-int launch_tile_scan(int ntiles, int32_t* tile_start, int32_t* cursor, int32_t* meta, bool ranked, cudaStream_t st) {
+int launch_tile_scan(int ntiles, int32_t* tile_start, int32_t* cursor, int32_t* meta, cudaStream_t st) {
   ProfScope ps(K_TILE_SCAN, st);
-  tile_scan_kernel<<<1, SCAN_THREADS, 0, st>>>(ntiles, tile_start, cursor, meta, SORT_CAP_SMALL_FWD, ranked ? 1 : 0);
+  tile_scan_kernel<<<1, SCAN_THREADS, 0, st>>>(ntiles, tile_start, cursor, meta, SORT_CAP_SMALL_FWD);
   LGR_CHECK_LAUNCH();
   return 0;
 }
@@ -460,16 +457,21 @@
     clamp_lists_kernel<<<(nt + 256) / 256, 256, 0, st>>>(nt, num_inst, tile_start, meta_dev);
     LGR_CHECK_LAUNCH();
   }
+  const bool slab = v.slab_cap > 0 && (meta_dev || max_len <= v.slab_cap);
+  const uint32_t* slab_key = slab ? v.slab_key : nullptr;
+  const uint32_t* slab_val = slab ? v.slab_val : nullptr;
+  const int slab_cap = slab ? v.slab_cap : 0;
   if (num_inst == 0 && v.num_owners == 0 && v.band_dsplat == nullptr) return 0;
   const int ntiles = v.gx * (v.row1 - v.row0);
-  unsigned blocks = (unsigned)((n + SCATTER_THREADS - 1) / SCATTER_THREADS);
-  if (v.region_count && blocks > (unsigned)LGR_REGION_GRID) blocks = (unsigned)LGR_REGION_GRID;
-  {
+  if (!slab) {
+    if (num_inst > 0 && (!inst_key || !inst_val)) return LGR_E_BADARG;
+    unsigned blocks = (unsigned)((n + SCATTER_THREADS - 1) / SCATTER_THREADS);
+    if (v.region_count && blocks > (unsigned)LGR_REGION_GRID) blocks = (unsigned)LGR_REGION_GRID;
     ProfScope ps(K_BIN_SCATTER, st);
     bin_scatter_kernel<<<blocks, SCATTER_THREADS, 0, st>>>(v, n, splat, radii, tile_start, cursor, inst_key, inst_val,
                                                            meta_dev ? num_inst : (int64_t)0x7fffffffffffffffLL);
-  }
-  LGR_CHECK_LAUNCH();
+    LGR_CHECK_LAUNCH();
+  }
   if (num_inst == 0) return 0;
   int id_bits = 8;
   while (id_bits < 32 && (n - 1) >> id_bits) id_bits += 8;
@@ -479,25 +481,25 @@
   }
   if (meta_dev) {
     ProfScope ps(K_TILE_SORT, st, 2);
-    tile_sort_kernel<0><<<ntiles, SORT_THREADS, 16 * SORT_CAP_SMALL, st>>>(nullptr, tile_start, inst_key, inst_val, inst_tmp, sorted_ids, 0, SORT_CAP_SMALL, id_bits, nullptr, nullptr);
+    tile_sort_kernel<0><<<ntiles, SORT_THREADS, 16 * SORT_CAP_SMALL, st>>>(nullptr, tile_start, inst_key, inst_val, inst_tmp, sorted_ids, 0, SORT_CAP_SMALL, id_bits, nullptr, meta_dev + 6, slab_key, slab_val, slab_cap);
     LGR_CHECK_LAUNCH();
     const int32_t* long_list = cursor + CSTRIDE * ntiles;
-    tile_sort_kernel<0><<<LONG_SORT_GRID, SORT_THREADS, 16 * SORT_CAP_LARGE, st>>>(long_list, tile_start, inst_key, inst_val, inst_tmp, sorted_ids, SORT_CAP_SMALL, SORT_CAP_LARGE, id_bits, meta_dev + 5, meta_dev + 6);
+    tile_sort_kernel<0><<<LONG_SORT_GRID, SORT_THREADS, 16 * SORT_CAP_LARGE, st>>>(long_list, tile_start, inst_key, inst_val, inst_tmp, sorted_ids, SORT_CAP_SMALL, SORT_CAP_LARGE, id_bits, meta_dev + 5, meta_dev + 6, slab_key, slab_val, slab_cap);
     LGR_CHECK_LAUNCH();
     return 0;
   }
   ProfScope ps(K_TILE_SORT, st, 1 + (num_long > 0) + (max_len > SORT_CAP_LARGE));
   const int cap_main = max(256, min(max_len, SORT_CAP_SMALL));
-  tile_sort_kernel<0><<<ntiles, SORT_THREADS, 16 * cap_main, st>>>(nullptr, tile_start, inst_key, inst_val, inst_tmp, sorted_ids, 0, cap_main, id_bits, nullptr, nullptr);
+  tile_sort_kernel<0><<<ntiles, SORT_THREADS, 16 * cap_main, st>>>(nullptr, tile_start, inst_key, inst_val, inst_tmp, sorted_ids, 0, cap_main, id_bits, nullptr, nullptr, slab_key, slab_val, slab_cap);
   LGR_CHECK_LAUNCH();
   if (num_long > 0) {
     const int32_t* long_list = cursor + CSTRIDE * ntiles;
     const int cap = min(max_len, SORT_CAP_LARGE);
-    tile_sort_kernel<0><<<num_long, SORT_THREADS, 16 * cap, st>>>(long_list, tile_start, inst_key, inst_val, inst_tmp, sorted_ids, SORT_CAP_SMALL, cap, id_bits, nullptr, nullptr);
+    tile_sort_kernel<0><<<num_long, SORT_THREADS, 16 * cap, st>>>(long_list, tile_start, inst_key, inst_val, inst_tmp, sorted_ids, SORT_CAP_SMALL, cap, id_bits, nullptr, nullptr, slab_key, slab_val, slab_cap);
     LGR_CHECK_LAUNCH();
     if (max_len > SORT_CAP_LARGE) {
       if (!inst_tmp) return LGR_E_CAPACITY;
-      tile_sort_kernel<1><<<num_long, SORT_THREADS, 0, st>>>(long_list, tile_start, inst_key, inst_val, inst_tmp, sorted_ids, SORT_CAP_LARGE, 0, id_bits, nullptr, nullptr);
+      tile_sort_kernel<1><<<num_long, SORT_THREADS, 0, st>>>(long_list, tile_start, inst_key, inst_val, inst_tmp, sorted_ids, SORT_CAP_LARGE, 0, id_bits, nullptr, nullptr, nullptr, nullptr, 0);
       LGR_CHECK_LAUNCH();
     }
   }
diff --git a/log_b200/csrc/lgr_capi.cu b/log_b200/csrc/lgr_capi.cu
--- a/log_b200/csrc/lgr_capi.cu
+++ b/log_b200/csrc/lgr_capi.cu
@@ -14,7 +14,7 @@
 int launch_grad_scatter_add(int64_t, const float*, int64_t, int64_t, float*, cudaStream_t);
 int launch_grad_scatter_add_staged(const float*, int, int64_t, int64_t, int64_t, float*, cudaStream_t);
 int launch_band_scan(const View&, cudaStream_t);
-int launch_tile_scan(int, int32_t*, int32_t*, int32_t*, bool, cudaStream_t);
+int launch_tile_scan(int, int32_t*, int32_t*, int32_t*, cudaStream_t);
 int launch_bin_and_sort(const View&, int64_t, int64_t, int, int, const float*, const int32_t*, int32_t*, int32_t*,
                         uint32_t*, uint32_t*, uint32_t*, int32_t*, int32_t*, cudaStream_t);
 int sort_smem_capacity();
@@ -54,6 +54,8 @@
   if (v->num_channels != 0 && v->num_channels != 3 && v->num_channels != 6) return false;
   if (v->num_channels == 6 && !v->splat_ext_d) return false;
   if (v->log_depth != 0 && (v->log_depth != 1 || v->num_channels != 6)) return false;
+  if (v->slab_cap < 0 || v->slab_cap > sort_smem_capacity()) return false;
+  if (v->slab_cap > 0 && (!v->slab_key_d || !v->slab_val_d || v->num_owners > 0 || v->band_dsplat_d)) return false;
   return true;
 }
 
@@ -126,7 +128,7 @@
   if (rc) return rc;
   rc = launch_band_scan(v, st);
   if (rc) return rc;
-  return launch_tile_scan(ntiles, tile_start_d, tile_cursor_d, meta_d, view->tile_rank_d != nullptr, st);
+  return launch_tile_scan(ntiles, tile_start_d, tile_cursor_d, meta_d, st);
 }
 
 int lgr_forward_render(const lgr_view* view, int64_t n, int64_t num_instances, int32_t max_tile_len,
@@ -138,7 +140,8 @@
   if (!view_ok(view) || n < 0 || num_instances < 0 || num_long_tiles < 0 || !tile_start_d || !tile_cursor_d || !image_d || !final_T_d ||
       !n_contrib_d)
     return LGR_E_BADARG;
-  if (num_instances > 0 && (!inst_key_d || !inst_val_d || !sorted_ids_d || !splat_d || !radii_d)) return LGR_E_BADARG;
+  const bool slab = view->slab_cap > 0 && max_tile_len <= view->slab_cap;
+  if (num_instances > 0 && ((!slab && (!inst_key_d || !inst_val_d)) || !sorted_ids_d || !splat_d || !radii_d)) return LGR_E_BADARG;
   if (const int rc6 = six_channels_check(view)) return rc6;
   if (view->want_aux && (!point_id_pixel_d || !point_weight_pixel_d || (n > 0 && !point_weight_d))) return LGR_E_BADARG;
   if (num_instances > 0x7fffffffLL) return LGR_E_UNSUPPORTED;
@@ -159,7 +162,7 @@
                                     int32_t* point_id_pixel_d, float* point_weight_pixel_d, float* point_weight_d,
                                     int32_t* point_count_d, void* stream) {
   if (!view_ok(view) || n < 0 || instance_capacity <= 0 || !meta_d || !tile_start_d || !tile_cursor_d || !image_d || !final_T_d ||
-      !n_contrib_d || !inst_key_d || !inst_val_d || !sorted_ids_d)
+      !n_contrib_d || (view->slab_cap <= 0 && (!inst_key_d || !inst_val_d)) || !sorted_ids_d)
     return LGR_E_BADARG;
   if (n > 0 && (!splat_d || !radii_d)) return LGR_E_BADARG;
   if (const int rc6 = six_channels_check(view)) return rc6;
@@ -297,7 +300,7 @@
   int rc = launch_shard_recv_count(v, make_layout(layout), exchange_d, dsplat_d, tile_cursor_d, meta_d, point_weight_rows_d,
                                    point_count_rows_d, st);
   if (rc) return rc;
-  return launch_tile_scan(ntiles, tile_start_d, tile_cursor_d, meta_d, view->tile_rank_d != nullptr, st);
+  return launch_tile_scan(ntiles, tile_start_d, tile_cursor_d, meta_d, st);
 }
 
 int lgr_blend_backward(const lgr_view* view, int64_t n, int64_t num_instances, const float* splat_d,
diff --git a/log_b200/csrc/lgr_common.cuh b/log_b200/csrc/lgr_common.cuh
--- a/log_b200/csrc/lgr_common.cuh
+++ b/log_b200/csrc/lgr_common.cuh
@@ -30,7 +30,9 @@
   int32_t* band_count;
   int32_t* band_rows;
   float* band_dsplat;
-  int32_t* tile_rank;
+  uint32_t* slab_key;
+  uint32_t* slab_val;
+  int slab_cap;
   const int64_t* gather;
   const int32_t* pid_map;
   int32_t* contrib_id;
@@ -54,7 +56,9 @@
 
 inline View make_view(const lgr_view* v, int64_t n = 0) {
   View o;
-  o.num_owners = v->num_owners; o.band_ids = v->band_ids_d; o.band_blk = v->band_blk_d; o.band_count = v->band_count_d; o.band_rows = v->band_rows_d; o.band_dsplat = v->band_dsplat_d; o.tile_rank = v->tile_rank_d; o.gather = v->gather_index_d; o.pid_map = v->pid_map_d; o.contrib_id = v->contrib_id_d; o.contrib_entry = v->contrib_entry_d; o.contrib_count = v->contrib_count_d; o.last_contrib = v->last_contrib_d;
+  o.num_owners = v->num_owners; o.band_ids = v->band_ids_d; o.band_blk = v->band_blk_d; o.band_count = v->band_count_d; o.band_rows = v->band_rows_d; o.band_dsplat = v->band_dsplat_d; o.gather = v->gather_index_d; o.pid_map = v->pid_map_d; o.contrib_id = v->contrib_id_d; o.contrib_entry = v->contrib_entry_d; o.contrib_count = v->contrib_count_d; o.last_contrib = v->last_contrib_d;
+  o.slab_cap = v->slab_cap > 0 ? v->slab_cap : 0;
+  o.slab_key = o.slab_cap ? v->slab_key_d : nullptr; o.slab_val = o.slab_cap ? v->slab_val_d : nullptr;
   o.region_count = v->region_count_d; o.region_cap = v->region_cap; o.regions = v->region_count_d ? v->num_regions : 0;
   o.cov3d = v->cov3D_precomp_d; o.dcov3d = v->dcov3D_d;
   o.owner_chunk = o.num_owners > 0 ? (int)LGR_OWNER_CHUNK(n, (int64_t)o.num_owners) : 256;
@@ -228,36 +232,49 @@
   return (int64_t)s * v.region_cap + (t - first[s]);
 }
 
-__device__ __forceinline__ bool count_small_tiles(const View& v, int32_t* __restrict__ tile_count, int64_t row, int x0, int y0, int x1,
-                                                  int y1) {
+__device__ __forceinline__ void slab_put(const View& v, int t, int r, uint32_t key, uint32_t row) {
+  if (r < v.slab_cap) {
+    const int64_t p = (int64_t)t * v.slab_cap + r;
+    v.slab_key[p] = key;
+    v.slab_val[p] = row;
+  }
+}
+
+__device__ __forceinline__ bool count_small_tiles(const View& v, int32_t* __restrict__ tile_count, uint32_t key, int64_t row, int x0,
+                                                  int y0, int x1, int y1) {
   const int w = x1 - x0, cnt = w * (y1 - y0);
   if (cnt > 4) return true;
-  if (v.tile_rank == nullptr) {
+  if (v.slab_cap == 0) {
     for (int k = 0; k < cnt; k++) atomicAdd(tile_count + ((y0 + k / w - v.row0) * v.gx + x0 + k % w) * CSTRIDE, 1);
     return false;
   }
-  int r[4];
+  int t[4], r[4];
 #pragma unroll
   for (int k = 0; k < 4; k++) {
-    r[k] = -1;
-    if (k < cnt) r[k] = atomicAdd(tile_count + ((y0 + k / max(w, 1) - v.row0) * v.gx + x0 + k % max(w, 1)) * CSTRIDE, 1);
-  }
-  *reinterpret_cast<int4*>(v.tile_rank + 4 * row) = make_int4(r[0], r[1], r[2], r[3]);
+    t[k] = (y0 + k / max(w, 1) - v.row0) * v.gx + x0 + k % max(w, 1);
+    r[k] = k < cnt ? atomicAdd(tile_count + t[k] * CSTRIDE, 1) : v.slab_cap;
+  }
+#pragma unroll
+  for (int k = 0; k < 4; k++) slab_put(v, t[k], r[k], key, (uint32_t)row);
   return false;
 }
 
-__device__ __forceinline__ void warp_count_big_tiles(const View& v, int32_t* __restrict__ tile_count, bool big, int x0, int y0, int x1,
-                                                     int y1) {
+__device__ __forceinline__ void warp_count_big_tiles(const View& v, int32_t* __restrict__ tile_count, bool big, uint32_t key, int64_t row,
+                                                     int x0, int y0, int x1, int y1) {
   const int lane = threadIdx.x & 31;
-  const int slot = v.tile_rank ? 1 : 0;
   unsigned todo = __ballot_sync(0xffffffffu, big);
   while (todo) {
     const int src = __ffs(todo) - 1;
     todo &= todo - 1;
     const int bx0 = __shfl_sync(0xffffffffu, x0, src), by0 = __shfl_sync(0xffffffffu, y0, src);
     const int bx1 = __shfl_sync(0xffffffffu, x1, src), by1 = __shfl_sync(0xffffffffu, y1, src);
+    const uint32_t bkey = __shfl_sync(0xffffffffu, key, src), brow = (uint32_t)__shfl_sync(0xffffffffu, (int)row, src);
     const int w = bx1 - bx0, cnt = w * (by1 - by0);
-    for (int k = lane; k < cnt; k += 32) atomicAdd(tile_count + ((by0 + k / w - v.row0) * v.gx + bx0 + k % w) * CSTRIDE + slot, 1);
+    for (int k = lane; k < cnt; k += 32) {
+      const int t = (by0 + k / w - v.row0) * v.gx + bx0 + k % w;
+      if (v.slab_cap == 0) atomicAdd(tile_count + t * CSTRIDE, 1);
+      else slab_put(v, t, atomicAdd(tile_count + t * CSTRIDE, 1), bkey, brow);
+    }
   }
 }
 
diff --git a/log_b200/csrc/lgr_project.cu b/log_b200/csrc/lgr_project.cu
--- a/log_b200/csrc/lgr_project.cu
+++ b/log_b200/csrc/lgr_project.cu
@@ -110,6 +110,7 @@
   }
   bool big_splat = false;
   int bx0 = 0, by0 = 0, bx1 = 0, by1 = 0;
+  uint32_t skey = 0;
   const int64_t src = (v.gather && work) ? v.gather[i] : i;
   if (work) {
     float p[3], Sg[9];
@@ -207,7 +208,8 @@
         if (DEPTH) r3 = make_float4(cv.t[2], p[2], 1.0f, 0.f);
         if (reach) {
           tile_rect_tight(px, py, rad, hx, hy, v.gx, v.gy, v.row0, v.row1, x0, y0, x1, y1);
-          big_splat = count_small_tiles(v, tile_count, i, x0, y0, x1, y1);
+          skey = __float_as_uint(cv.t[2]);
+          big_splat = count_small_tiles(v, tile_count, skey, i, x0, y0, x1, y1);
           bx0 = x0; by0 = y0; bx1 = x1; by1 = y1;
         }
       }
@@ -222,7 +224,7 @@
   } else if (i < n) {
     radii[i] = 0;
   }
-  warp_count_big_tiles(v, tile_count, big_splat, bx0, by0, bx1, by1);
+  warp_count_big_tiles(v, tile_count, big_splat, skey, i, bx0, by0, bx1, by1);
   if (v.num_owners > 0) {
     __shared__ int sCnt[PROJ_THREADS / 32];
     const int lane = threadIdx.x & 31, wid = threadIdx.x >> 5;
diff --git a/log_b200/csrc/lgr_shard.cu b/log_b200/csrc/lgr_shard.cu
--- a/log_b200/csrc/lgr_shard.cu
+++ b/log_b200/csrc/lgr_shard.cu
@@ -149,25 +149,28 @@
   for (int64_t base = (int64_t)blockIdx.x * SHARD_THREADS; base < total; base += (int64_t)gridDim.x * SHARD_THREADS) {
     bool big_splat = false;
     int bx0 = 0, by0 = 0, bx1 = 0, by1 = 0;
+    int64_t slot = 0;
+    uint32_t key = 0;
     if (base + threadIdx.x < total) {
-      const int64_t slot = region_row(v, s_first, base + threadIdx.x);
+      slot = region_row(v, s_first, base + threadIdx.x);
       const float* rec = xbuf + L.off_splat + slot * LGR_SPLAT_FLOATS;
       const float4 r0 = *reinterpret_cast<const float4*>(rec);
       const float4 r1 = *reinterpret_cast<const float4*>(rec + 4);
+      key = __float_as_uint(rec[11]);
       const int rad = radii[slot];
       int x0, y0, x1, y1;
       tile_rect(r0.x, r0.y, rad, v.gx, v.gy, x0, y0, x1, y1);
       stock += (unsigned)((x1 - x0) * max(0, min(y1, v.row1) - max(y0, v.row0)));
       vis += 1;
       tile_rect_tight(r0.x, r0.y, rad, r1.z, r1.w, v.gx, v.gy, v.row0, v.row1, x0, y0, x1, y1);
-      big_splat = count_small_tiles(v, tile_count, slot, x0, y0, x1, y1);
+      big_splat = count_small_tiles(v, tile_count, key, slot, x0, y0, x1, y1);
       bx0 = x0; by0 = y0; bx1 = x1; by1 = y1;
       float4* z = reinterpret_cast<float4*>(dsplat + slot * LGR_GRAD_FLOATS);
       z[0] = z[1] = z[2] = make_float4(0.f, 0.f, 0.f, 0.f);
       if (pw_rows) pw_rows[slot] = 0.f;
       if (pc_rows) pc_rows[slot] = 0;
     }
-    warp_count_big_tiles(v, tile_count, big_splat, bx0, by0, bx1, by1);
+    warp_count_big_tiles(v, tile_count, big_splat, key, slot, bx0, by0, bx1, by1);
   }
   const unsigned st_w = __reduce_add_sync(FULLMASK, stock);
   const int vis_w = __reduce_add_sync(FULLMASK, vis);
diff --git a/log_b200/rasterizer.py b/log_b200/rasterizer.py
--- a/log_b200/rasterizer.py
+++ b/log_b200/rasterizer.py
@@ -8,7 +8,6 @@
 from ._capi import LGR_FILTER_ADD, LGR_FILTER_MAX, LGR_FILTER_NONE, LgrView
 
 PREZERO_DSPLAT = bool(int(__import__('os').environ.get('LGR_PREZERO_DSPLAT', '0')))
-RANKED_BIN = bool(int(__import__('os').environ.get('LGR_RANKED_BIN', '1')))
 CONTRIB_BITS = bool(int(__import__('os').environ.get('LGR_CONTRIB_BITS', '1')))
 FLAVOUR_STOCK = 'stock'
 FLAVOUR_FORK = 'fork'
@@ -55,7 +54,7 @@
 
 def _make_view(s: GaussianRasterizationSettings, filter_mode: int, want_aux: bool, sh_coeffs: int, tile_rows, keep,
                num_owners=0, band_ids=None, band_count=None, band_blk=None, band_rows=None, band_dsplat=None,
-               raw_params=False, tile_rank=None, gather_index=None, pid_map=None, cov3D_precomp=None, splat_ext=None,
+               raw_params=False, gather_index=None, pid_map=None, cov3D_precomp=None, splat_ext=None,
                log_depth=False):
     dev = s.viewmatrix.device
     vm, pm = _f32c(s.viewmatrix, 'viewmatrix'), _f32c(s.projmatrix, 'projmatrix', dev)
@@ -76,7 +75,6 @@
     v.band_blk_d = band_blk.data_ptr() if band_blk is not None else None
     v.band_rows_d = band_rows.data_ptr() if band_rows is not None else None
     v.band_dsplat_d = band_dsplat.data_ptr() if band_dsplat is not None else None
-    v.tile_rank_d = tile_rank.data_ptr() if tile_rank is not None else None
     v.gather_index_d = gather_index.data_ptr() if gather_index is not None else None
     v.pid_map_d = pid_map.data_ptr() if pid_map is not None else None
     v.cov3D_precomp_d = cov3D_precomp.data_ptr() if cov3D_precomp is not None else None
@@ -87,6 +85,19 @@
     v.campos_d = cp.data_ptr() if cp is not None else None
     v.bg_d = bg.data_ptr()
     return v
+
+
+def set_slab(view, slab):
+    if slab is None or slab.numel() == 0:
+        view.slab_key_d = view.slab_val_d = None
+        view.slab_cap = 0
+        return
+    view.slab_key_d, view.slab_val_d = slab[0].data_ptr(), slab[1].data_ptr()
+    view.slab_cap = _capi.load().lgr_sort_smem_capacity()
+
+
+def slab_tensor(ntiles, device):
+    return torch.empty((2, ntiles * _capi.load().lgr_sort_smem_capacity()), dtype=torch.int32, device=device)
 
 
 def set_contrib_lists(view, buf, D, n_contrib):
@@ -184,16 +195,17 @@
         band_ids = torch.empty((max(256 * nb, 1),), dtype=torch.int32, device=dev)
         band_blk = torch.empty((2 * nb + 1,), dtype=torch.int32, device=dev)
         band_count = torch.empty((num_owners,), dtype=torch.int32, device=dev)
-    tile_rank = torch.empty((max(n, 1), 4), dtype=torch.int32, device=dev) if RANKED_BIN else None
-    keep.append(tile_rank)
     splat_ext = torch.empty((max(n, 1), 4), dtype=torch.float32, device=dev) if channels == 6 else None
     keep.append(splat_ext)
     view = _make_view(settings, filter_mode, want_aux, K, tile_rows, keep, num_owners, band_ids, band_count, band_blk, band_rows, band_dsplat,
-                      raw_params, tile_rank, gather_index, cov3D_precomp=cov3D_precomp, splat_ext=splat_ext, log_depth=log_depth)
+                      raw_params, gather_index, cov3D_precomp=cov3D_precomp, splat_ext=splat_ext, log_depth=log_depth)
     H, W = view.image_height, view.image_width
     gx, gy = (W + 15) // 16, (H + 15) // 16
     rows = gy if tile_rows is None else int(tile_rows[1]) - int(tile_rows[0])
     ntiles = gx * rows
+    slab = slab_tensor(ntiles, dev) if num_owners == 0 and band_dsplat is None else None
+    set_slab(view, slab)
+    cap = view.slab_cap
     i32 = dict(dtype=torch.int32, device=dev)
     f32 = dict(dtype=torch.float32, device=dev)
     splat = torch.empty((n, _capi.LGR_SPLAT_FLOATS), **f32)
@@ -221,7 +233,9 @@
         if num_owners > 0:
             raise _capi.LgrError('instance_capacity (device-sized call) is not available in band mode')
         D, max_len, num_long, stock_D, m = int(instance_capacity), None, None, None, None
-        inst_key, inst_val = torch.empty((D,), **u32), torch.empty((D,), **u32)
+        inst_key = inst_val = None
+        if not cap:
+            inst_key, inst_val = torch.empty((D,), **u32), torch.empty((D,), **u32)
         sorted_ids = torch.empty((D,), **i32)
         contrib = torch.empty((2 * D + ntiles,), **i32) if use_contrib_lists(D, None) else None
         keep.append(contrib)
@@ -237,8 +251,9 @@
         if D < 0 or stock_D > 0x7fffffff:
             raise _capi.LgrError(f'this view needs {stock_D} (Gaussian, tile) instances by the stock rule (D = {m[0] & 0xffffffff} binned, '
                                  f'{m[4]} of {n} Gaussians visible, longest tile list {max_len}): more than 2^31 - 1 is unsupported')
-        inst_key = torch.empty((D,), **u32)
-        inst_val = torch.empty((D,), **u32)
+        inst_key = inst_val = None
+        if not cap or max_len > cap:
+            inst_key, inst_val = torch.empty((D,), **u32), torch.empty((D,), **u32)
         inst_tmp = torch.empty((2 * D,), **u32) if max_len > lib.lgr_sort_smem_capacity() else None
         sorted_ids = torch.empty((D,), **i32)
         contrib = torch.empty((2 * D + ntiles,), **i32) if use_contrib_lists(D, max_len) else None
@@ -248,6 +263,8 @@
                                            _ptr(tile_cursor), _ptr(inst_key), _ptr(inst_val), _ptr(inst_tmp),
                                            _ptr(sorted_ids), _ptr(image), _ptr(final_T), _ptr(n_contrib), _ptr(pid),
                                            _ptr(pwp), _ptr(pw), _ptr(pc), st), 'lgr_forward_render')
+    set_slab(view, None)
+    del slab
     s = RasterState()
     s.view, s.keep, s.n, s.num_instances, s.max_tile_len = view, keep, n, D, max_len
     s.stock_instances, s.num_visible = stock_D, (int(m[4]) if m is not None else None)
diff --git a/log_b200/sharded.py b/log_b200/sharded.py
--- a/log_b200/sharded.py
+++ b/log_b200/sharded.py
@@ -232,10 +232,11 @@
         s.keep, s.n, s.want_aux, s.settings = [], n, bool(want_aux), settings
         K = 0 if sh is None else int(sh.shape[1])
         s.view_full = _make_view(settings, filter_mode, want_aux, K, None, s.keep, raw_params=raw_params)
-        from .rasterizer import RANKED_BIN
-        rank_rows = self._scratch('tile_rank', (self.world * self.cap, 4), torch.int32) if RANKED_BIN else None
-        s.view_band = _make_view(settings, filter_mode, want_aux, K, self.band, s.keep, raw_params=raw_params, tile_rank=rank_rows,
+        from .rasterizer import set_slab
+        s.view_band = _make_view(settings, filter_mode, want_aux, K, self.band, s.keep, raw_params=raw_params,
                                  pid_map=self.recv_gid)
+        band_tiles = ((settings.image_width + 15) // 16) * (self.band[1] - self.band[0])
+        set_slab(s.view_band, self._scratch('slab', (2, band_tiles * lib.lgr_sort_smem_capacity()), torch.int32))
         s.view_band.region_count_d = self.buf.data_ptr() + 4 * int(self.layout.off_count)
         s.view_band.region_cap, s.view_band.num_regions = self.cap, self.world
         H, W = s.view_full.image_height, s.view_full.image_width
@@ -291,8 +292,10 @@
             pwp = torch.zeros((H, W), **f32)
         if self.sync_free and self._inst_cap > 0:
             cap = self._inst_cap
-            inst_key = self._scratch('inst_key', (cap,), torch.int32)
-            inst_val = self._scratch('inst_val', (cap,), torch.int32)
+            inst_key = inst_val = None
+            if not v.slab_cap:
+                inst_key = self._scratch('inst_key', (cap,), torch.int32)
+                inst_val = self._scratch('inst_val', (cap,), torch.int32)
             s.sorted_ids = self._scratch('sorted_ids', (cap,), torch.int32)
             set_contrib_lists(v, self._scratch('contrib', (2 * cap + ntiles,), torch.int32) if use_contrib_lists(cap, None) else None,
                               cap, n_contrib)
@@ -309,8 +312,10 @@
         s.stock_instances = (m[2] & 0xffffffff) | ((m[3] & 0xffffffff) << 32)
         if max_len <= lib.lgr_sort_smem_capacity():
             self._inst_cap = max(self._inst_cap, D + D // 4 + 4096)
-        inst_key = self._scratch('inst_key', (D,), torch.int32)
-        inst_val = self._scratch('inst_val', (D,), torch.int32)
+        inst_key = inst_val = None
+        if not v.slab_cap or max_len > v.slab_cap:
+            inst_key = self._scratch('inst_key', (D,), torch.int32)
+            inst_val = self._scratch('inst_val', (D,), torch.int32)
         inst_tmp = self._scratch('inst_tmp', (2 * D,), torch.int32) if max_len > lib.lgr_sort_smem_capacity() else None
         s.sorted_ids = self._scratch('sorted_ids', (D,), torch.int32)
         set_contrib_lists(v, self._scratch('contrib', (2 * D + ntiles,), torch.int32) if use_contrib_lists(D, max_len) else None,
```

Result: faster. 1.771 billion, median of 6 (+4.9%).
